# POSTECH-CVLab/PyTorch-StudioGAN

Measured on AMD Instinct MI355X. Metric: images/sec (G+D step) BigGAN ImageNet-128 bs256, higher is better.
Workload: dtype bf16

## Files before the change

### include/sgamd.h

```cpp
#ifndef SGAMD_H
#define SGAMD_H
#include <stdint.h>
#ifdef __cplusplus
extern "C" {
#endif

typedef void* sg_stream_t;

#define SG_DTYPE_F32 0
#define SG_DTYPE_BF16 1
#define SG_DTYPE_F64 2

#define SG_PIX_RELU 1
#define SG_PIX_UPSAMPLE 2
#define SG_PIX_QUAD 4
#define SG_PIX_TRANSPOSED 8
#define SG_EPI_OUT_F32 1
#define SG_EPI_ATOMIC 2
#define SG_EPI_POOL 4
#define SG_EPI_RELU 8
#define SG_EPI_RES_F32 16

const char* sg_last_error(void);
int sg_version(void);
int sg_prof_enable(int on);
int sg_prof_collect(double* out, int nkinds);

typedef struct {
  int dtype;
  int N, Hs, Ws, C, ldx;
  int Ho, Wo, Cout;
  int R, S, stride, pad_h, pad_w;
  int pix_flags, epi_flags;
  float alpha, beta;
  const void* x; const void* w;
  const float* bias; const void* res; const void* mask; void* out; const float* alpha_ptr;
  int ldo, ldr, ldm;
} sg_conv_fwd_desc;
int sg_conv2d_fwd(const sg_conv_fwd_desc* d, sg_stream_t stream);
int sg_set_f32_mode(int mode);
int sg_get_f32_mode(void);

typedef struct {
  sg_conv_fwd_desc main;
  const void* x2; const void* w2; const float* bias2;
  int C2, ldx2, x2_up;
  float* stats;
} sg_conv_skip_desc;
int sg_conv2d_fwd_skip_stat_rows(const sg_conv_skip_desc* d);
int sg_conv2d_fwd_skip(const sg_conv_skip_desc* d, sg_stream_t stream);
int sg_conv2d_fwd_skip_ok(const sg_conv_skip_desc* d);
long long sg_conv_rs_launches(void);

#define SG_Q_POOL 0
#define SG_Q_UP 1
typedef struct {
  int dtype, form;
  int N, Hl, Wl;
  int C, ldx, Cout;
  int pix_flags, epi_flags;
  float alpha, beta;
  const void* x; const void* wq;
  const float* bias; const void* res; const void* mask; void* out; const float* alpha_ptr;
  int ldo, ldr, ldm;
  const void* x2; const void* w2q; const float* bias2;
  int C2, ldx2;
  float* stats;
  int x2_norelu;
} sg_convq_desc;
int sg_conv2d_q_stat_rows(const sg_convq_desc* d);
int sg_conv2d_q(const sg_convq_desc* d, sg_stream_t stream);
int sg_conv2d_q_ok(const sg_convq_desc* d);
int sg_quad_pack(int dtype, int mode, const void* src, void* dst, int M, int Cs, sg_stream_t stream);
typedef struct { const void* src; void* dst; int M, Cs, mode, pad_; } sg_quad_item;
int sg_quad_pack_batch(int dtype, const sg_quad_item* items_dev, const sg_quad_item* items_host, int n, sg_stream_t stream);
typedef struct {
  int dtype, form;
  int N, Hl, Wl;
  int C, ldx, x_flags;
  int Cout, ldg;
  float alpha; const float* alpha_ptr;
  const void* x; const void* dy; float* dw; float* dbias;
  float* work; long long work_floats;
  int splits;
} sg_convq_wgrad_desc;
int sg_conv2d_q_wgrad_plan(const sg_convq_wgrad_desc* d, int* splits, long long* work_floats);
int sg_conv2d_q_wgrad(const sg_convq_wgrad_desc* d, sg_stream_t stream);
int sg_prof_collect_ex(double* out, int nkinds);
int sg_prof_collect_tags(double* out, int ntags);

typedef struct {
  int dtype;
  int N;
  int xHs, xWs, C, ldx, x_flags;
  int gHs, gWs, Cout, ldg, g_flags;
  int Ho, Wo;
  int R, S, stride, pad_h, pad_w;
  float alpha;
  const void* x; const void* dy; float* dw;
  const float* alpha_ptr;
  int splits;
  int no_tr;
  float* work; long long work_floats;
  float* dbias;
} sg_conv_wgrad_desc;
int sg_conv2d_wgrad(const sg_conv_wgrad_desc* d, sg_stream_t stream);
int sg_conv2d_wgrad_fuses_bias(const sg_conv_wgrad_desc* d);
int sg_conv2d_wgrad_plan(const sg_conv_wgrad_desc* d, int* splits, long long* work_floats);

typedef struct {
  int dtype, p_form, q_form;
  int I, J, K, batch;
  const void* p; long long p_bstride; int ldp;
  const void* q; long long q_bstride; int ldq;
  void* out; long long out_bstride; int ldo;
  const float* bias; const void* res; long long res_bstride; int ldr; float beta;
  float alpha; const float* alpha_ptr;
  int epi_flags; int splits; int no_tr;
} sg_gemm_desc;
int sg_gemm(const sg_gemm_desc* d, sg_stream_t stream);
typedef struct { const float* w; const float* y; const float* bias; float* out; int rows, K, ldy, ldo; } sg_linear_item;
int sg_linear_group(const sg_linear_item* items_dev, const sg_linear_item* items_host, int n, int B, sg_stream_t stream);

int sg_nchw_to_nhwc(int dtype, const float* src, void* dst, int N, int C, int H, int W, int ldo, sg_stream_t s);
int sg_nhwc_to_nchw(int dtype, const void* src, float* dst, int N, int C, int H, int W, int lds, int apply_tanh, sg_stream_t s);
int sg_nchw_grad_to_nhwc(int dtype, const float* dy, const float* y, void* dst, int N, int C, int H, int W, int ldo, int apply_tanh, sg_stream_t s);
int sg_avgpool2_fwd(int dtype, const void* x, void* y, int N, int H, int W, int C, sg_stream_t s);
int sg_avgpool2_bwd(int dtype, const void* dy, void* dx, int N, int H, int W, int C, sg_stream_t s);
int sg_maxpool2_fwd(int dtype, const void* x, int ldx, void* y, int ldy, uint8_t* idx, int N, int H, int W, int C, sg_stream_t s);
int sg_maxpool2_bwd(int dtype, const void* dy, int ldy, const uint8_t* idx, void* dx, int ldx, int N, int H, int W, int C, sg_stream_t s);
int sg_softmax_rows(int dtype, const float* s_in, void* p_out, long long rows, int cols, sg_stream_t st);
int sg_softmax_rows_bwd(int dtype, const void* p, const float* dp, void* ds, long long rows, int cols, sg_stream_t st);
int sg_convert(int src_dtype, int dst_dtype, const void* x, void* y, long long n, sg_stream_t s);
int sg_add_relu(int dtype, const void* a, const void* x, void* out, long long n, sg_stream_t s);
int sg_relu_mask(int dtype, const void* dy, const void* x, void* dx, long long n, sg_stream_t s);
int sg_axpby(int dtype, const void* x, void* y, long long n, float a, float b, sg_stream_t s);
int sg_dot(int dtype, const void* x, const void* y, long long n, float* out, float scale, const float* scale_ptr, sg_stream_t s);
int sg_colsum(int dtype, const void* x, int ldx, const void* mask, int ldm, long long rows, int C, float* out, float alpha, sg_stream_t s);

int sg_bn_partial_stats(int dtype, const void* x, int ldx, long long rows, int C, double* partial, sg_stream_t s);
int sg_bn_stats_from_tiles(const float* stats, int nrows, int C, double* partial, sg_stream_t s);
int sg_bn_finalize(const double* partial, double count, int C, float eps, float momentum, float* mean, float* invstd,
                   float* running_mean, float* running_var, sg_stream_t s);
typedef void* sg_comm_t;
int sg_comm_unique_id(void* out128);
int sg_comm_init_rank(const void* id128, int nranks, int rank, sg_comm_t* comm);
int sg_comm_size(sg_comm_t comm, int* nranks);
int sg_comm_destroy(sg_comm_t comm);
int sg_allreduce_flat(sg_comm_t comm, void* buf, long long count, int dtype, sg_stream_t s);
int sg_bn_stats_sync(int dtype, const void* x, int ldx, long long rows, int C, double* partial, sg_comm_t comm, float eps, float momentum,
                     float* mean, float* invstd, float* running_mean, float* running_var, sg_stream_t s);
int sg_reduce_scatter_flat(sg_comm_t comm, float* buf, long long per_rank, sg_stream_t s);
int sg_allgather_flat(sg_comm_t comm, float* buf, long long per_rank, sg_stream_t s);

// ... 194 lines not shown
```

### pytorch-studiogan_amd/_lib.py

```python
import ctypes as C
import os
import subprocess
import sys

import torch

_HERE = os.path.dirname(os.path.abspath(__file__))
LIB_PATH = os.path.join(_HERE, "libsgamd.so")
if os.environ.get("SG_LIBSGAMD"):
    LIB_PATH = os.path.abspath(os.environ["SG_LIBSGAMD"])
CSRC = os.path.join(_HERE, "csrc")

F32, BF16, F64 = 0, 1, 2
PIX_RELU, PIX_UPSAMPLE, PIX_QUAD, PIX_TRANSPOSED = 1, 2, 4, 8
Q_POOL, Q_UP = 0, 1
EPI_OUT_F32, EPI_ATOMIC, EPI_POOL, EPI_RELU, EPI_RES_F32 = 1, 2, 4, 8, 16

_vp, _i, _f, _ll = C.c_void_p, C.c_int, C.c_float, C.c_longlong


class ConvFwdDesc(C.Structure):
    _fields_ = [("dtype", _i), ("N", _i), ("Hs", _i), ("Ws", _i), ("C", _i), ("ldx", _i), ("Ho", _i), ("Wo", _i), ("Cout", _i),
                ("R", _i), ("S", _i), ("stride", _i), ("pad_h", _i), ("pad_w", _i), ("pix_flags", _i), ("epi_flags", _i),
                ("alpha", _f), ("beta", _f), ("x", _vp), ("w", _vp), ("bias", _vp), ("res", _vp), ("mask", _vp), ("out", _vp),
                ("alpha_ptr", _vp), ("ldo", _i), ("ldr", _i), ("ldm", _i)]


class ConvSkipDesc(C.Structure):
    _fields_ = [("main", ConvFwdDesc), ("x2", _vp), ("w2", _vp), ("bias2", _vp), ("C2", _i), ("ldx2", _i), ("x2_up", _i), ("stats", _vp)]


class ConvWgradDesc(C.Structure):
    _fields_ = [("dtype", _i), ("N", _i), ("xHs", _i), ("xWs", _i), ("C", _i), ("ldx", _i), ("x_flags", _i), ("gHs", _i), ("gWs", _i),
                ("Cout", _i), ("ldg", _i), ("g_flags", _i), ("Ho", _i), ("Wo", _i), ("R", _i), ("S", _i), ("stride", _i),
                ("pad_h", _i), ("pad_w", _i), ("alpha", _f), ("x", _vp), ("dy", _vp), ("dw", _vp), ("alpha_ptr", _vp),
                ("splits", _i), ("no_tr", _i), ("work", _vp), ("work_floats", _ll), ("dbias", _vp)]


class ConvQDesc(C.Structure):
    _fields_ = [("dtype", _i), ("form", _i), ("N", _i), ("Hl", _i), ("Wl", _i), ("C", _i), ("ldx", _i), ("Cout", _i),
                ("pix_flags", _i), ("epi_flags", _i), ("alpha", _f), ("beta", _f), ("x", _vp), ("wq", _vp), ("bias", _vp), ("res", _vp),
                ("mask", _vp), ("out", _vp), ("alpha_ptr", _vp), ("ldo", _i), ("ldr", _i), ("ldm", _i),
                ("x2", _vp), ("w2q", _vp), ("bias2", _vp), ("C2", _i), ("ldx2", _i), ("stats", _vp), ("x2_norelu", _i)]


class ConvQWgradDesc(C.Structure):
    _fields_ = [("dtype", _i), ("form", _i), ("N", _i), ("Hl", _i), ("Wl", _i), ("C", _i), ("ldx", _i), ("x_flags", _i), ("Cout", _i),
                ("ldg", _i), ("alpha", _f), ("alpha_ptr", _vp), ("x", _vp), ("dy", _vp), ("dw", _vp), ("dbias", _vp), ("work", _vp),
                ("work_floats", _ll), ("splits", _i)]


class QuadItem(C.Structure):
    _fields_ = [("src", _vp), ("dst", _vp), ("M", _i), ("Cs", _i), ("mode", _i), ("pad_", _i)]


class LinearItem(C.Structure):
    _fields_ = [("w", _vp), ("y", _vp), ("bias", _vp), ("out", _vp), ("rows", _i), ("K", _i), ("ldy", _i), ("ldo", _i)]


class GemmDesc(C.Structure):
    _fields_ = [("dtype", _i), ("p_form", _i), ("q_form", _i), ("I", _i), ("J", _i), ("K", _i), ("batch", _i),
                ("p", _vp), ("p_bstride", _ll), ("ldp", _i), ("q", _vp), ("q_bstride", _ll), ("ldq", _i),
                ("out", _vp), ("out_bstride", _ll), ("ldo", _i), ("bias", _vp), ("res", _vp), ("res_bstride", _ll), ("ldr", _i),
                ("beta", _f), ("alpha", _f), ("alpha_ptr", _vp), ("epi_flags", _i), ("splits", _i), ("no_tr", _i)]


class SnLayer(C.Structure):
    _fields_ = [("w", _vp), ("u", _vp), ("v", _vp), ("sigma", _vp), ("u_snap", _vp), ("v_snap", _vp), ("w_fwd", _vp), ("w_dgrad", _vp),
                ("w_f32", _vp), ("rows", _i), ("cols", _i), ("Cin", _i), ("RS", _i), ("do_power_iter", _i), ("apply_sn", _i),
                ("rows_pad", _i), ("work_off", _ll), ("trans", _i), ("dgrad_noflip", _i), ("Cin_pad", _i)]


class SnBwdLayer(C.Structure):
    _fields_ = [("dwt", _vp), ("w", _vp), ("u", _vp), ("v", _vp), ("sigma", _vp), ("dw", _vp), ("rows", _i), ("cols", _i),
                ("Cin", _i), ("RS", _i), ("natural", _i), ("apply_sn", _i), ("trans", _i), ("Cin_pad", _i)]


class AugDesc(C.Structure):
    _fields_ = [("N", _i), ("C", _i), ("H", _i), ("W", _i), ("ops", _i), ("cut_h", _i), ("cut_w", _i), ("max_t", _i), ("color", _vp), ("geom", _vp)]


AUG_BRIGHTNESS, AUG_SATURATION, AUG_CONTRAST, AUG_FLIP, AUG_TRANSLATE, AUG_TRANSLATE_REFLECT, AUG_CUTOUT = 1, 2, 4, 8, 16, 32, 64

_lib = None


def build(force=False, verbose=False):
    cmd = ["make", "-C", CSRC, "-j", str(max(2, os.cpu_count() or 2))]
    if force:
        subprocess.run(["make", "-C", CSRC, "clean"], check=True, stdout=subprocess.DEVNULL)
    res = subprocess.run(cmd, stdout=subprocess.PIPE, stderr=subprocess.STDOUT, text=True)
    if verbose or res.returncode != 0:
        sys.stderr.write(res.stdout)
    if res.returncode != 0:
        raise RuntimeError("building libsgamd.so failed")
    return LIB_PATH


_PROTOS = {
    "sg_prof_enable": [_i],
    "sg_prof_collect": [C.POINTER(C.c_double), _i],
    "sg_conv2d_fwd": [C.POINTER(ConvFwdDesc), _vp],
    "sg_conv2d_fwd_skip": [C.POINTER(ConvSkipDesc), _vp],
    "sg_conv2d_fwd_skip_ok": [C.POINTER(ConvSkipDesc)],
    "sg_conv_rs_launches": [],
    "sg_conv2d_q": [C.POINTER(ConvQDesc), _vp],
    "sg_conv2d_q_ok": [C.POINTER(ConvQDesc)],
    "sg_conv2d_q_stat_rows": [C.POINTER(ConvQDesc)],
    "sg_conv2d_fwd_skip_stat_rows": [C.POINTER(ConvSkipDesc)],
    "sg_bn_stats_from_tiles": [_vp, _i, _i, _vp, _vp],
    "sg_quad_pack": [_i, _i, _vp, _vp, _i, _i, _vp],
    "sg_quad_pack_batch": [_i, _vp, C.POINTER(QuadItem), _i, _vp],
    "sg_linear_group": [_vp, C.POINTER(LinearItem), _i, _i, _vp],
    "sg_conv2d_q_wgrad_plan": [C.POINTER(ConvQWgradDesc), C.POINTER(_i), C.POINTER(_ll)],
    "sg_conv2d_q_wgrad": [C.POINTER(ConvQWgradDesc), _vp],
    "sg_prof_collect_ex": [C.POINTER(C.c_double), _i],
    "sg_prof_collect_tags": [C.POINTER(C.c_double), _i],
    "sg_conv2d_wgrad": [C.POINTER(ConvWgradDesc), _vp],
    "sg_conv2d_wgrad_plan": [C.POINTER(ConvWgradDesc), C.POINTER(_i), C.POINTER(_ll)],
    "sg_conv2d_wgrad_fuses_bias": [C.POINTER(ConvWgradDesc)],
    "sg_gemm": [C.POINTER(GemmDesc), _vp],
    "sg_nchw_to_nhwc": [_i, _vp, _vp, _i, _i, _i, _i, _i, _vp],
    "sg_nhwc_to_nchw": [_i, _vp, _vp, _i, _i, _i, _i, _i, _i, _vp],
    "sg_nchw_grad_to_nhwc": [_i, _vp, _vp, _vp, _i, _i, _i, _i, _i, _i, _vp],
    "sg_avgpool2_fwd": [_i, _vp, _vp, _i, _i, _i, _i, _vp],
    "sg_avgpool2_bwd": [_i, _vp, _vp, _i, _i, _i, _i, _vp],
    "sg_maxpool2_fwd": [_i, _vp, _i, _vp, _i, _vp, _i, _i, _i, _i, _vp],
    "sg_maxpool2_bwd": [_i, _vp, _i, _vp, _vp, _i, _i, _i, _i, _i, _vp],
    "sg_softmax_rows": [_i, _vp, _vp, _ll, _i, _vp],
    "sg_softmax_rows_bwd": [_i, _vp, _vp, _vp, _ll, _i, _vp],
    "sg_axpby": [_i, _vp, _vp, _ll, _f, _f, _vp],
    "sg_convert": [_i, _i, _vp, _vp, _ll, _vp],
    "sg_add_relu": [_i, _vp, _vp, _vp, _ll, _vp],
    "sg_relu_mask": [_i, _vp, _vp, _vp, _ll, _vp],
    "sg_dot": [_i, _vp, _vp, _ll, _vp, _f, _vp, _vp],
    "sg_colsum": [_i, _vp, _i, _vp, _i, _ll, _i, _vp, _f, _vp],
    "sg_bn_partial_stats": [_i, _vp, _i, _ll, _i, _vp, _vp],
    "sg_bn_finalize": [_vp, C.c_double, _i, _f, _f, _vp, _vp, _vp, _vp, _vp],
    "sg_comm_unique_id": [_vp],
    "sg_comm_init_rank": [_vp, _i, _i, C.POINTER(_vp)],
    "sg_comm_size": [_vp, C.POINTER(_i)],
    "sg_comm_destroy": [_vp],
    "sg_allreduce_flat": [_vp, _vp, _ll, _i, _vp],
    "sg_bn_stats_sync": [_i, _vp, _i, _ll, _i, _vp, _vp, _f, _f, _vp, _vp, _vp, _vp, _vp],
    "sg_set_f32_mode": [_i],
    "sg_get_f32_mode": [],
    "sg_reduce_scatter_flat": [_vp, _vp, _ll, _vp],
    "sg_allgather_flat": [_vp, _vp, _ll, _vp],
    "sg_p2p_create": [_i, _i, _ll, C.POINTER(_vp), _vp],
    "sg_p2p_connect": [_vp, _vp],
    "sg_p2p_destroy": [_vp],
    "sg_p2p_timeouts": [_vp, C.POINTER(_i)],
    "sg_p2p_allreduce_f64": [_vp, _vp, _i, _vp],
    "sg_bn_finalize_p2p": [_vp, _vp, C.c_double, _i, _f, _f, _vp, _vp, _vp, _vp, _vp],
    "sg_bn_stats_sync_p2p": [_i, _vp, _i, _ll, _i, _vp, _vp, _f, _f, _vp, _vp, _vp, _vp, _vp],
    "sg_bn_from_running": [_vp, _vp, _i, _f, _vp, _vp, _vp],
    "sg_bn_apply": [_i, _vp, _vp, _i, _ll, _i, _vp, _vp, _vp, _vp, _i, _i, _vp],
    "sg_bn_bwd_reduce": [_i, _vp, _vp, _i, _ll, _i, _vp, _vp, _vp, _vp, _i, _i, _vp, _vp],
    "sg_bn_bwd_finalize": [_vp, _i, _i, _vp, _i, _vp, _vp, _vp, _vp],
    "sg_bn_bwd_apply": [_i, _vp, _vp, _vp, _i, _ll, _i, _vp, _vp, _vp, _vp, _i, _i, _vp, C.c_double, _i, _vp],
    "sg_bn_bwd_apply_res": [_i, _vp, _vp, _vp, _i, _ll, _i, _vp, _vp, _vp, _vp, _i, _i, _vp, C.c_double, _i, _vp, _vp],
    "sg_bn_bwd2_reduce": [_i, _vp, _vp, _vp, _i, _ll, _i, _vp, _vp, _vp, _vp, _i, _vp, _vp],
    "sg_bn_bwd2_finalize": [_vp, _i, _i, _vp, _vp],
    "sg_bn_bwd2_dgain": [_vp, _vp, C.c_double, _vp, _i, _i, _vp, _vp],
    "sg_bn_bwd2_apply": [_i, _vp, _vp, _vp, _vp, _vp, _i, _ll, _i, _vp, _vp, _vp, _vp, _i, _vp, C.c_double, _i, _vp],
    "sg_attn_fused_ok": [_i, _i, _i, _i, _i],
    "sg_attn_fwd_fused_ok": [_i, _i, _i, _i, _i],
    "sg_attn_fwd_flash_ok": [_i, _i, _i, _i, _i],
    "sg_attn_fwd_fused": [_vp, _vp, _vp, _vp, _vp, _vp, _vp, _i, _i, _i, _i, _i, _vp],
    "sg_attn_bwd_fused_ok": [_i, _i, _i, _i, _i],
    "sg_attn_bwd_fused": [_vp, _vp, _vp, _vp, _vp, _vp, _vp, _vp, _vp, _vp, _i, _i, _i, _i, _i, _vp],
    "sg_attn_probs_fwd": [_vp, _vp, _vp, _vp, _i, _i, _i, _i, _vp],
    "sg_attn_ds_bwd": [_vp, _vp, _vp, _vp, _vp, _vp, _i, _i, _i, _i, _i, _vp],
    "sg_attn_proj_ok": [_i, _i, _i, _i, _i, _i, _i],
    "sg_attn_proj_fwd": [_vp, _i, _vp, _vp, _vp, _vp, _vp, _vp, _vp, _vp, _i, _i, _i, _i, _i, _i, _i, _vp],
    "sg_attn_proj_bwd_data": [_vp, _vp, _vp, _vp, _vp, _vp, _vp, _vp, _vp, _vp, _i, _i, _i, _i, _i, _i, _vp],
    "sg_slice_up_fwd": [_i, _vp, _vp, _i, _i, _i, _i, _i, _i, _vp],
    "sg_slice_up_bwd": [_i, _vp, _vp, _i, _i, _i, _i, _i, _i, _vp],
    "sg_copy_channels": [_i, _vp, _i, _vp, _i, _ll, _i, _vp],
    "sg_interp_rows": [_vp, _vp, _vp, _vp, _i, _ll, _vp],
    "sg_gp_fwd": [_i, _vp, _i, _ll, _vp, _vp, _vp],
    "sg_gp_bwd": [_i, _vp, _vp, _vp, _vp, _i, _ll, _vp],
    "sg_masked_sum_hw": [_i, _vp, _vp, _vp, _i, _i, _i, _vp],
    "sg_sn_forward": [_i, _vp, C.POINTER(SnLayer), _i, _f, _vp, _ll, _vp],
    "sg_sn_backward": [_vp, C.POINTER(SnBwdLayer), _i, _vp, _ll, _vp],
    "sg_embedding_fwd": [_vp, _vp, _vp, _i, _i, _i, _vp],
    "sg_embedding_bwd": [_vp, _vp, _vp, _i, _i, _i, _vp],
# ... 142 lines not shown
```

### pytorch-studiogan_amd/backbones/big_resnet.py

```python
import torch
import torch.nn as nn

from .. import functional as F
from .. import ops
from ..bank import get_bank
from .heads import build_heads, apply_heads


def _dtype(mixed_precision):
    return torch.bfloat16 if mixed_precision else torch.float32


def _need_graph(module, *inputs):
    if not torch.is_grad_enabled():
        return False
    for t in inputs:
        if torch.is_tensor(t) and t.requires_grad:
            return True
    return any(p.requires_grad for p in module.parameters())


class GenBlock(nn.Module):
    def __init__(self, in_channels, out_channels, g_cond_mtd, affine_input_dim, MODULES):
        super().__init__()
# ... 69 lines not shown
        for index in range(self.num_blocks):
            blocks += [[GenBlock(in_channels=self.in_dims[index], out_channels=self.out_dims[index], g_cond_mtd=self.g_cond_mtd,
                                 affine_input_dim=self.affine_input_dim, MODULES=MODULES)]]
            if index + 1 in attn_g_loc and apply_attn:
                blocks += [[ops.SelfAttention(self.out_dims[index], is_generator=True, MODULES=MODULES)]]
        self.blocks = nn.ModuleList([nn.ModuleList(block) for block in blocks])

        self.bn4 = ops.batchnorm_2d(in_features=self.out_dims[-1])
        self.activation = MODULES.g_act_fn
        self.conv2d5 = MODULES.g_conv2d(in_channels=self.out_dims[-1], out_channels=3, kernel_size=3, stride=1, padding=1)
        self.tanh = nn.Tanh()
        self.conv2d5._sg_rows_pad = 8
        ops.init_weights(self.modules, g_init)
        ops.adopt(self, _dtype(mixed_precision))

    def forward(self, z, label, shared_label=None, eval=False):
        dtype = self.compute_dtype
        bank = get_bank(self, dtype)
        slot = bank.begin_forward(_need_graph(self, z, shared_label))
        affine_list = []
        if self.info_type != "N/A":
            if self.g_info_injection == "concat":
                z = self.info_mix_linear.forward_rt(z, slot)
            else:
                z, z_info = z[:, :self.z_dim], z[:, self.z_dim:]
                affine_list.append(self.info_proj_linear.forward_rt(z_info, slot))
        zs = torch.split(z, self.chunk_size, 1)
        z0 = zs[0]
        if self.g_cond_mtd != "W/O":
            if shared_label is None:
                shared_label = self.shared(label)
            affine_list.append(shared_label)
        if len(affine_list) == 0:
            affines = [item for item in zs[1:]]
        else:
            affines = [torch.cat(affine_list + [item], 1) for item in zs[1:]]

        pairs, counter = [], 0
        for blocklist in self.blocks:
            for block in blocklist:
                if not isinstance(block, ops.SelfAttention):
                    if isinstance(block.bn1, ops.ConditionalBatchNorm2d):
                        pairs += [(block.bn1, affines[counter]), (block.bn2, affines[counter])]
                    counter += 1
        F.cbn_prefetch(slot, pairs)

        act = self.linear0.forward_rt(z0, slot)
        act = F.NchwToNhwcFn.apply(act.view(-1, self.in_dims[0], self.bottom, self.bottom), dtype)
        act = ops.block_boundary(self, -1, act)
        counter = 0
        nxt = bank.boundaries(self.blocks) if bank.exchange is not None else None
        with ops.bump_batches_tracked(self):
            for bi, blocklist in enumerate(self.blocks):
                for block in blocklist:
                    if isinstance(block, ops.SelfAttention):
                        act = block.forward_nhwc(act, slot)
                    else:
                        act = block.forward_nhwc(act, affines[counter], slot)
                        counter += 1
                if nxt is not None:
                    act = bank.mark(act, nxt[bi])
                act = ops.block_boundary(self, bi, act)
            act = self.bn4.forward_nhwc(act, relu=True)
        act = self.conv2d5.forward_nhwc(act, slot)
        return F.NhwcToNchwFn.apply(act, True, 3)


class DiscOptBlock(nn.Module):
    def __init__(self, in_channels, out_channels, apply_d_sn, MODULES):
        super().__init__()
        self.apply_d_sn = apply_d_sn
        self.conv2d0 = MODULES.d_conv2d(in_channels=in_channels, out_channels=out_channels, kernel_size=1, stride=1, padding=0)
        self.conv2d1 = MODULES.d_conv2d(in_channels=in_channels, out_channels=out_channels, kernel_size=3, stride=1, padding=1)
        self.conv2d2 = MODULES.d_conv2d(in_channels=out_channels, out_channels=out_channels, kernel_size=3, stride=1, padding=1)
        if not apply_d_sn:
            self.bn0 = MODULES.d_bn(in_features=in_channels)
            self.bn1 = MODULES.d_bn(in_features=out_channels)
        self.activation = MODULES.d_act_fn
        self.average_pooling = nn.AvgPool2d(2)
        self.cpad = 8 if (apply_d_sn and in_channels < 8) else 0
        if self.cpad:
            self.conv2d1._sg_cin_pad = self.conv2d0._sg_cin_pad = self.cpad

    def forward_nhwc(self, x, slot):
        h = self.conv2d1.forward_nhwc(x, slot)
        if not self.apply_d_sn:
            h = self.bn1.forward_nhwc(h, relu=True)
            h = self.conv2d2.forward_nhwc(h, slot, out_pool=True)
        else:
            if self.cpad == 8 and h.dtype == torch.bfloat16 and not x.requires_grad:
                return ops.conv_skip_nhwc(self.conv2d2, self.conv2d0, h, x, slot, in_relu=True, out_pool=True, skip_relu=False)
            h = self.conv2d2.forward_nhwc(h, slot, in_relu=True, out_pool=True)
        x0 = F.AvgPool2Fn.apply(x)
        if not self.apply_d_sn:
            x0 = self.bn0.forward_nhwc(x0)
        return self.conv2d0.forward_nhwc(x0, slot, res=h)


class DiscBlock(nn.Module):
    def __init__(self, in_channels, out_channels, apply_d_sn, MODULES, downsample=True):
        super().__init__()
        self.apply_d_sn = apply_d_sn
        self.downsample = downsample
        self.activation = MODULES.d_act_fn
        self.ch_mismatch = in_channels != out_channels
        if self.ch_mismatch or downsample:
            self.conv2d0 = MODULES.d_conv2d(in_channels=in_channels, out_channels=out_channels, kernel_size=1, stride=1, padding=0)
            if not apply_d_sn:
                self.bn0 = MODULES.d_bn(in_features=in_channels)
        self.conv2d1 = MODULES.d_conv2d(in_channels=in_channels, out_channels=out_channels, kernel_size=3, stride=1, padding=1)
        self.conv2d2 = MODULES.d_conv2d(in_channels=out_channels, out_channels=out_channels, kernel_size=3, stride=1, padding=1)
        if not apply_d_sn:
            self.bn1 = MODULES.d_bn(in_features=in_channels)
            self.bn2 = MODULES.d_bn(in_features=out_channels)
        self.average_pooling = nn.AvgPool2d(2)

    def forward_nhwc(self, x, slot):
        if self.apply_d_sn:
            if self.downsample or self.ch_mismatch:
                link = F.GradLink()
                h = self.conv2d1.forward_nhwc(x, slot, in_relu=True, link=link)
                return ops.conv_skip_nhwc(self.conv2d2, self.conv2d0, h, x, slot, in_relu=True, out_pool=self.downsample, link=link)
            h = self.conv2d1.forward_nhwc(x, slot, in_relu=True)
            h = self.conv2d2.forward_nhwc(h, slot, in_relu=True, out_pool=False)
            return F.AddReluFn.apply(h, x)
        h = self.bn1.forward_nhwc(x, relu=True)
        h = self.conv2d1.forward_nhwc(h, slot)
        h = self.bn2.forward_nhwc(h, relu=True)
        h = self.conv2d2.forward_nhwc(h, slot, out_pool=self.downsample)
        if self.downsample or self.ch_mismatch:
            x0 = self.bn0.forward_nhwc(x)
            return self.conv2d0.forward_nhwc(x0, slot, out_pool=self.downsample, res=h)
        return F.AddFn.apply(h, x)


class Discriminator(nn.Module):
    def __init__(self, img_size, d_conv_dim, apply_d_sn, apply_attn, attn_d_loc, d_cond_mtd, aux_cls_type, d_embed_dim, normalize_d_embed,
                 num_classes, d_init, d_depth, mixed_precision, MODULES, MODEL):
        super().__init__()
        d_in_dims_collection = {
            "32": [3] + [d_conv_dim * 2, d_conv_dim * 2, d_conv_dim * 2],
            "64": [3] + [d_conv_dim, d_conv_dim * 2, d_conv_dim * 4, d_conv_dim * 8],
            "128": [3] + [d_conv_dim, d_conv_dim * 2, d_conv_dim * 4, d_conv_dim * 8, d_conv_dim * 16],
            "256": [3] + [d_conv_dim, d_conv_dim * 2, d_conv_dim * 4, d_conv_dim * 8, d_conv_dim * 8, d_conv_dim * 16],
            "512": [3] + [d_conv_dim, d_conv_dim, d_conv_dim * 2, d_conv_dim * 4, d_conv_dim * 8, d_conv_dim * 8, d_conv_dim * 16]
        }
        d_out_dims_collection = {
            "32": [d_conv_dim * 2, d_conv_dim * 2, d_conv_dim * 2, d_conv_dim * 2],
            "64": [d_conv_dim, d_conv_dim * 2, d_conv_dim * 4, d_conv_dim * 8, d_conv_dim * 16],
            "128": [d_conv_dim, d_conv_dim * 2, d_conv_dim * 4, d_conv_dim * 8, d_conv_dim * 16, d_conv_dim * 16],
            "256": [d_conv_dim, d_conv_dim * 2, d_conv_dim * 4, d_conv_dim * 8, d_conv_dim * 8, d_conv_dim * 16, d_conv_dim * 16],
            "512": [d_conv_dim, d_conv_dim, d_conv_dim * 2, d_conv_dim * 4, d_conv_dim * 8, d_conv_dim * 8, d_conv_dim * 16, d_conv_dim * 16]
        }
        d_down = {
            "32": [True, True, False, False],
            "64": [True, True, True, True, False],
            "128": [True, True, True, True, True, False],
            "256": [True, True, True, True, True, True, False],
            "512": [True, True, True, True, True, True, True, False]
        }
        self.d_cond_mtd = d_cond_mtd
        self.aux_cls_type = aux_cls_type
        self.normalize_d_embed = normalize_d_embed
        self.num_classes = num_classes
        self.mixed_precision = mixed_precision
        self.in_dims = d_in_dims_collection[str(img_size)]
        self.out_dims = d_out_dims_collection[str(img_size)]
        self.MODEL = MODEL
        down = d_down[str(img_size)]

        blocks = []
        for index in range(len(self.in_dims)):
            if index == 0:
                blocks += [[DiscOptBlock(in_channels=self.in_dims[index], out_channels=self.out_dims[index], apply_d_sn=apply_d_sn, MODULES=MODULES)]]
            else:
                blocks += [[DiscBlock(in_channels=self.in_dims[index], out_channels=self.out_dims[index], apply_d_sn=apply_d_sn,
                                      MODULES=MODULES, downsample=down[index])]]
            if index + 1 in attn_d_loc and apply_attn:
                blocks += [[ops.SelfAttention(self.out_dims[index], is_generator=False, MODULES=MODULES)]]
        self.blocks = nn.ModuleList([nn.ModuleList(block) for block in blocks])
        self.activation = MODULES.d_act_fn
        build_heads(self, MODULES, self.out_dims[-1], d_cond_mtd, aux_cls_type, d_embed_dim, num_classes, MODEL)
        if d_init:
            ops.init_weights(self.modules, d_init)
        ops.adopt(self, _dtype(mixed_precision))

    def forward(self, x, label, eval=False, adc_fake=False):
        dtype = self.compute_dtype
        bank = get_bank(self, dtype)
        slot = bank.begin_forward(_need_graph(self, x))
        h = ops.to_nhwc(x, dtype, self.blocks[0][0].cpad)
        nxt = bank.boundaries(self.blocks) if bank.exchange is not None else None
        for bi, blocklist in enumerate(self.blocks):
            for block in blocklist:
                h = block.forward_nhwc(h, slot)
            if nxt is not None:
                h = bank.mark(h, nxt[bi])
            h = ops.block_boundary(self, bi, h)
        hw = h.shape[1] * h.shape[2]
        h = F.ReluSumFn.apply(h)
        return apply_heads(self, h, label, slot, adc_fake, hw=hw)
```

### pytorch-studiogan_amd/csrc/common.h

```cpp
#pragma once
#include <hip/hip_runtime.h>
#include <stdint.h>

typedef uint16_t bf16_t;
typedef __attribute__((ext_vector_type(4))) uint32_t u32x4;
typedef __attribute__((ext_vector_type(2))) uint32_t u32x2;
typedef __attribute__((ext_vector_type(4))) float f32x4;
typedef __attribute__((ext_vector_type(16))) float f32x16;
typedef __attribute__((ext_vector_type(8))) __bf16 bf16x8_t;
typedef __attribute__((ext_vector_type(4))) short s16x4;
typedef __attribute__((ext_vector_type(8))) short s16x8;

#define SG_PRIO_UP() __builtin_amdgcn_s_setprio(1)
#define SG_PRIO_DOWN() __builtin_amdgcn_s_setprio(0)

#define SG_DTYPE_F32 0
#define SG_DTYPE_BF16 1

__device__ __forceinline__ float bf2f(bf16_t v) { return __uint_as_float(((uint32_t)v) << 16); }
__device__ __forceinline__ bf16_t f2bf(float f) {
  uint32_t u = __float_as_uint(f);
  if ((u & 0x7fffffffu) > 0x7f800000u) return (bf16_t)((u >> 16) | 0x40u);
  u += 0x7fffu + ((u >> 16) & 1u);
  return (bf16_t)(u >> 16);
}

typedef __bf16 sg_bf16x2_t __attribute__((ext_vector_type(2)));
typedef float sg_f32x2_t __attribute__((ext_vector_type(2)));
__device__ __forceinline__ uint32_t pack2bf(float a, float b) {
  sg_f32x2_t v = {a, b};
  return __builtin_bit_cast(uint32_t, __builtin_convertvector(v, sg_bf16x2_t));
}

template <typename T> __device__ __forceinline__ float to_f(T v);
template <> __device__ __forceinline__ float to_f<float>(float v) { return v; }
template <> __device__ __forceinline__ float to_f<bf16_t>(bf16_t v) { return bf2f(v); }
template <typename T> __device__ __forceinline__ T from_f(float v);
template <> __device__ __forceinline__ float from_f<float>(float v) { return v; }
template <> __device__ __forceinline__ bf16_t from_f<bf16_t>(float v) { return f2bf(v); }

template <typename T> struct ET;
template <> struct ET<float> { static constexpr int VEC = 4, BK = 16; };
template <> struct ET<bf16_t> { static constexpr int VEC = 8, BK = 32; };

__device__ __forceinline__ u32x4 zero16() { u32x4 z = {0u, 0u, 0u, 0u}; return z; }

template <typename T> __device__ __forceinline__ void unpack16(u32x4 v, float* o);
template <> __device__ __forceinline__ void unpack16<float>(u32x4 v, float* o) {
#pragma unroll
  for (int i = 0; i < 4; i++) o[i] = __uint_as_float(v[i]);
}
template <> __device__ __forceinline__ void unpack16<bf16_t>(u32x4 v, float* o) {
#pragma unroll
  for (int i = 0; i < 4; i++) { o[2 * i] = __uint_as_float(v[i] << 16); o[2 * i + 1] = __uint_as_float(v[i] & 0xffff0000u); }
}
template <typename T> __device__ __forceinline__ u32x4 pack16(const float* o);
template <> __device__ __forceinline__ u32x4 pack16<float>(const float* o) {
  u32x4 v;
#pragma unroll
  for (int i = 0; i < 4; i++) v[i] = __float_as_uint(o[i]);
  return v;
}
template <> __device__ __forceinline__ u32x4 pack16<bf16_t>(const float* o) {
  u32x4 v;
#pragma unroll
  for (int i = 0; i < 4; i++) v[i] = (uint32_t)f2bf(o[2 * i]) | ((uint32_t)f2bf(o[2 * i + 1]) << 16);
  return v;
}


template <typename T> __device__ __forceinline__ u32x4 relu16(u32x4 v);
template <> __device__ __forceinline__ u32x4 relu16<float>(u32x4 v) {
#pragma unroll
  for (int i = 0; i < 4; i++) v[i] = (v[i] & 0x80000000u) ? 0u : v[i];
  return v;
}
template <> __device__ __forceinline__ u32x4 relu16<bf16_t>(u32x4 v) {
  typedef short s16x2_t __attribute__((ext_vector_type(2)));
#pragma unroll
  for (int i = 0; i < 4; i++) {
    const uint32_t x = v[i];
    s16x2_t a = __builtin_bit_cast(s16x2_t, x);
    const s16x2_t z = {0, 0};
    a = __builtin_elementwise_max(a, z);
    v[i] = __builtin_bit_cast(uint32_t, a);
  }
  return v;
}

__device__ __forceinline__ float quad_sum(float v) {
  v += __builtin_bit_cast(float, __builtin_amdgcn_update_dpp(0, __builtin_bit_cast(int, v), 0xB1, 0xF, 0xF, true));
  v += __builtin_bit_cast(float, __builtin_amdgcn_update_dpp(0, __builtin_bit_cast(int, v), 0x4E, 0xF, 0xF, true));
  return v;
}

__device__ __forceinline__ float wave_sum(float v) {
#pragma unroll
  for (int o = 32; o > 0; o >>= 1) v += __shfl_xor(v, o, 64);
  return v;
}
__device__ __forceinline__ double wave_sum_d(double v) {
#pragma unroll
  for (int o = 32; o > 0; o >>= 1) v += __shfl_xor(v, o, 64);
  return v;
}
__device__ __forceinline__ float wave_max(float v) {
#pragma unroll
  for (int o = 32; o > 0; o >>= 1) v = fmaxf(v, __shfl_xor(v, o, 64));
  return v;
}

__device__ __forceinline__ float block_sum_256(float v, float* sm ) {
  v = wave_sum(v);
  int w = threadIdx.x >> 6;
// ... 46 lines not shown
```

### pytorch-studiogan_amd/csrc/conv.hip

```cpp
#include "conv_common.h"
#include "conv_v2.h"

int g_sg_f32_mode = 0;
extern "C" int sg_set_f32_mode(int mode) {
  SG_CHECK(mode == 0 || mode == 3, "sg_set_f32_mode: 0 (exact fp32 MFMA) or 3 (bf16x3 split)");
  g_sg_f32_mode = mode;
  return 0;
}
extern "C" int sg_get_f32_mode() { return g_sg_f32_mode; }

template <typename T, bool FAST>
static void conv_fwd_launch(const sg_conv_fwd_desc* d, const Epilogue<T>& e, int I, int J, int K, int pflags, hipStream_t st) {
  typedef StridedKC<T, FAST> LP;
  typedef ConvPixKC<T, FAST> LQ;
  LP lp;
  lp.base = (const T*)d->w; lp.bstride = 0; lp.ld = K; lp.rows = I; lp.K = K;
  lp.vec_ok = (K % ET<T>::VEC == 0) && aligned16(d->w);
  LQ lq;
  fill_geom<T>(lq.g, d->x, d->N, d->Hs, d->Ws, d->C, d->ldx, d->Ho, d->Wo, d->R, d->S, d->stride, d->pad_h, d->pad_w, pflags);
  lq.rows = J; lq.K = K;
  if constexpr (sizeof(T) == 4 && FAST) {
    if (g_sg_f32_mode == 3) {
      if (I <= 32) sg_launch_gemm<T, LP, LQ, 32, 256, 1, 4, true, 3>(lp, lq, e, I, J, K, 1, 1, st);
      else if (I % 128 != 0 && (I % 96 == 0 || (I < 128 && I > 64))) sg_launch_gemm<T, LP, LQ, 96, 256, 1, 4, true, 3>(lp, lq, e, I, J, K, 1, 1, st);
      else sg_launch_gemm<T, LP, LQ, 128, 128, 2, 2, true, 3>(lp, lq, e, I, J, K, 1, 1, st);
      return;
    }
  }
  if (I <= 32) sg_launch_gemm<T, LP, LQ, 32, 256, 1, 4>(lp, lq, e, I, J, K, 1, 1, st);
  else if (I % 128 != 0 && (I % 96 == 0 || (I < 128 && I > 64))) sg_launch_gemm<T, LP, LQ, 96, 256, 1, 4>(lp, lq, e, I, J, K, 1, 1, st);
  else sg_launch_gemm<T, LP, LQ, 128, 128, 2, 2>(lp, lq, e, I, J, K, 1, 1, st);
}

template <typename T> static bool conv_fwd_v2_try(const sg_conv_fwd_desc*, const Epilogue<T>&, int, int, int, int, hipStream_t) { return false; }
template <> bool conv_fwd_v2_try<bf16_t>(const sg_conv_fwd_desc* d, const Epilogue<bf16_t>& e, int I, int J, int K, int pflags, hipStream_t st) {
  const char* mode = getenv("SG_CONV_V2");
  const bool disabled = mode && mode[0] == '0';
  const bool force = mode && mode[0] == 'f';
  if (disabled || (pflags & SG_PIX_TRANSPOSED)) return false;
  if (d->stride != 1 && (d->stride != 2 || (pflags & (SG_PIX_UPSAMPLE | SG_PIX_QUAD)) || getenv("SG_CONV_V2_STRIDE2_OFF"))) return false;
  if (d->C % 8 || d->ldx % 8 || d->R * d->S > 25 || J < 256) return false;
  const long long xbytes = (((long long)d->N * d->Hs * d->Ws - 1) * d->ldx + d->C) * 2, wbytes = (long long)I * K * 2;
  if (xbytes >= (1ll << 31) || wbytes >= (1ll << 30)) return false;
  if (!aligned16(d->x) || !aligned16(d->w)) return false;
  if ((e.flags & (SG_EPI_ATOMIC | SG_EPI_OUT_F32)) || (e.ldo & 7) || !aligned16(e.out)) return false;
  if (e.mask && ((e.ldm & 7) || !aligned16(e.mask))) return false;
  if (e.res && ((e.flags & SG_EPI_RES_F32) || (e.ldr & 7) || !aligned16(e.res))) return false;
  const int tj = (J + 255) / 256;
  const int cands[3] = {192, 128, 96};
  int best = 0, best_tiles = 0;
  for (int c = 0; c < 3; c++) {
    if (I % cands[c]) continue;
    const int tiles = (I / cands[c]) * tj;
    if (tiles >= 512) { best = cands[c]; best_tiles = tiles; break; }
    if (tiles > best_tiles) { best = cands[c]; best_tiles = tiles; }
  }
  if (!best && I % 8 == 0 && I >= 32) {
    int best_pad = 0;
    for (int c = 0; c < 3; c++) {
      const int padded = ((I + cands[c] - 1) / cands[c]) * cands[c];
      if (2 * padded > 3 * I) continue;
      const int tiles = (padded / cands[c]) * tj;
      if (!best || padded < best_pad) { best = cands[c]; best_pad = padded; best_tiles = tiles; }
    }
  }
  int min_tiles = 160;
  if (const char* mt = getenv("SG_CONV_V2_MIN_TILES")) { const int v = atoi(mt); if (v > 0) min_tiles = v; }
  if (!best || (best_tiles < min_tiles && !force)) return false;
  ConvV2Params p;
  p.x = (const bf16_t*)d->x; p.w = (const bf16_t*)d->w;
  p.N = d->N; p.Hs = d->Hs; p.Ws = d->Ws; p.C = d->C; p.ldx = d->ldx;
  const int up = (pflags & SG_PIX_UPSAMPLE) ? 2 : 1;
  p.Hin = d->Hs * up; p.Win = d->Ws * up; p.Ho = d->Ho; p.Wo = d->Wo;
  p.R = d->R; p.S = d->S; p.pad_h = d->pad_h; p.pad_w = d->pad_w; p.flags = pflags; p.stride = d->stride;
  p.I = I; p.J = J; p.K = K; p.cpt = d->C / 8; p.ntap = d->R * d->S;
  p.wshift = ilog2_exact(d->Wo); p.hshift = ilog2_exact(d->Ho);
  p.xbytes = (unsigned)xbytes; p.wbytes = (unsigned)wbytes;
  int rc = 0;
  if (best == 192) rc = sg_launch_conv_v2<192, 4, 2, 256, 7>(p, e, st);
  else if (best == 128) rc = sg_launch_conv_v2<128, 4, 2, 256, 7>(p, e, st);
  else {
    if (J >= 512 * 256) rc = sg_launch_conv_v2<96, 8, 1, 512, 1>(p, e, st);
    else rc = sg_launch_conv_v2<96, 8, 1, 256, 1>(p, e, st);
  }
  return rc == 0;
}

template <typename T> static bool conv_fwd_v3_try(const sg_conv_fwd_desc*, const Epilogue<T>&, int, int, int, int, hipStream_t) { return false; }
template <> bool conv_fwd_v3_try<bf16_t>(const sg_conv_fwd_desc* d, const Epilogue<bf16_t>& e, int I, int J, int K, int pflags, hipStream_t st) {
  return sg_conv_fwd_v3_try(d, e, I, J, K, pflags, st);
}
template <typename T> static bool conv_fwd_v4_try(const sg_conv_fwd_desc*, const Epilogue<T>&, int, int, int, int, hipStream_t) { return false; }
template <> bool conv_fwd_v4_try<bf16_t>(const sg_conv_fwd_desc* d, const Epilogue<bf16_t>& e, int I, int J, int K, int pflags, hipStream_t st) {
  return sg_conv_fwd_v4_try(d, e, I, J, K, pflags, st);
}
template <typename T> static bool conv_fwd_rs_try(const sg_conv_fwd_desc*, const Epilogue<T>&, int, int, int, int, hipStream_t) { return false; }
template <> bool conv_fwd_rs_try<bf16_t>(const sg_conv_fwd_desc* d, const Epilogue<bf16_t>& e, int I, int J, int K, int pflags, hipStream_t st) {
  return sg_conv_fwd_rs_try(d, e, I, J, K, pflags, st);
}
template <typename T> static bool conv_fwd_sk_try(const sg_conv_fwd_desc*, const Epilogue<T>&, int, int, int, int, hipStream_t) { return false; }
template <> bool conv_fwd_sk_try<bf16_t>(const sg_conv_fwd_desc* d, const Epilogue<bf16_t>& e, int I, int J, int K, int pflags, hipStream_t st) {
  return sg_conv_fwd_sk_try(d, e, I, J, K, pflags, st);
}

template <typename T> static int conv_fwd_t(const sg_conv_fwd_desc* d, hipStream_t st) {
  const int K = d->R * d->S * d->C;
  const int I = d->Cout;
  const long long Jll = (long long)d->N * d->Ho * d->Wo;
  SG_CHECK(Jll < (1ll << 31), "sg_conv2d_fwd: too many output pixels");
  SG_CHECK((long long)d->N * d->Hs * d->Ws * d->ldx < (1ll << 31), "sg_conv2d_fwd: input tensor too large for 32-bit element offsets");
  const int J = (int)Jll;
  int pflags = d->pix_flags;
  if (d->epi_flags & SG_EPI_POOL) {
    SG_CHECK((d->Ho % 2 == 0) && (d->Wo % 2 == 0), "sg_conv2d_fwd: pooled output needs even Ho, Wo");
    pflags |= SG_PIX_QUAD;
  } else {
    pflags &= ~SG_PIX_QUAD;
  }
  const bool w_vec = (K % ET<T>::VEC == 0) && aligned16(d->w);
  const bool x_vec = (d->C % ET<T>::VEC == 0) && (d->ldx % ET<T>::VEC == 0) && aligned16(d->x);
  Epilogue<T> e;
  e.out = d->out; e.out_bstride = 0; e.ldo = d->ldo; e.bias = d->bias;
  e.res = d->res; e.res_bstride = 0; e.ldr = d->ldr; e.beta = d->beta;
  e.mask = (const T*)d->mask; e.mask_bstride = 0; e.ldm = d->ldm; e.split_stride = 0;
  e.alpha = d->alpha; e.alpha_ptr = d->alpha_ptr; e.flags = d->epi_flags; e.I = I; e.J = J;
  const int prof = sg_prof_begin(st, 2.0 * (double)I * (double)J * (double)K, 0);
  int eng = SG_ENG_CONV_GEMM;
  if (w_vec && x_vec && conv_fwd_sk_try<T>(d, e, I, J, K, pflags, st)) eng = SG_ENG_CONV_SK;
  else if (w_vec && x_vec && conv_fwd_rs_try<T>(d, e, I, J, K, pflags, st)) eng = SG_ENG_CONV_RS;
  else if (w_vec && x_vec && conv_fwd_v4_try<T>(d, e, I, J, K, pflags, st)) eng = SG_ENG_CONV_V4;
  else if (w_vec && x_vec && conv_fwd_v3_try<T>(d, e, I, J, K, pflags, st)) eng = SG_ENG_CONV_V3;
  else if (w_vec && x_vec && conv_fwd_v2_try<T>(d, e, I, J, K, pflags, st)) eng = SG_ENG_CONV_V2;
  else if (w_vec && x_vec) conv_fwd_launch<T, true>(d, e, I, J, K, pflags, st);
  else conv_fwd_launch<T, false>(d, e, I, J, K, pflags, st);
  {
    const double es = sizeof(T), jout = (d->epi_flags & SG_EPI_POOL) ? (double)J / 4.0 : (double)J;
    const double b = es * ((double)d->N * d->Hs * d->Ws * d->C + (double)I * K + jout * I * (1.0 + (d->mask ? 1.0 : 0.0) + (d->res ? 1.0 : 0.0)));
    sg_prof_tag(prof, eng, b);
  }
  sg_prof_end(st, prof);
  SG_LAUNCH_CHECK();
  return 0;
}

static int conv_fwd_skip(const sg_conv_skip_desc* sk, hipStream_t st, bool dry) {
  const sg_conv_fwd_desc* d = &sk->main;
  if (d->dtype != SG_DTYPE_BF16 || d->R != 3 || d->S != 3 || d->stride != 1 || (d->pix_flags & (SG_PIX_UPSAMPLE | SG_PIX_TRANSPOSED))) return 0;
  const int K = 9 * d->C, I = d->Cout;
  const long long Jll = (long long)d->N * d->Ho * d->Wo;
  if (Jll >= (1ll << 31) || (long long)d->N * d->Hs * d->Ws * d->ldx >= (1ll << 31)) return 0;
  const int J = (int)Jll;
  int pflags = d->pix_flags;
  if (d->epi_flags & SG_EPI_POOL) { if ((d->Ho & 1) || (d->Wo & 1)) return 0; pflags |= SG_PIX_QUAD; } else pflags &= ~SG_PIX_QUAD;
  Epilogue<bf16_t> e;
  e.out = d->out; e.out_bstride = 0; e.ldo = d->ldo; e.bias = d->bias;
  e.res = d->res; e.res_bstride = 0; e.ldr = d->ldr; e.beta = d->beta;
  e.mask = (const bf16_t*)d->mask; e.mask_bstride = 0; e.ldm = d->ldm; e.split_stride = 0;
  e.alpha = d->alpha; e.alpha_ptr = d->alpha_ptr; e.flags = d->epi_flags; e.I = I; e.J = J;
  if (dry) return sg_conv_fwd_v4_skip_try(d, sk, e, I, J, K, pflags, st, true) ? 1 : 0;
  const int prof = sg_prof_begin(st, 2.0 * (double)I * (double)J * ((double)K + (double)sk->C2), 0);
  const bool ok = sg_conv_fwd_v4_skip_try(d, sk, e, I, J, K, pflags, st, false);
  {
    const double jout = (d->epi_flags & SG_EPI_POOL) ? (double)J / 4.0 : (double)J;
    const double x2 = (double)d->N * (sk->x2_up ? (d->Ho / 2) * (d->Wo / 2) : d->Ho * d->Wo) * sk->C2;
    sg_prof_tag(prof, SG_ENG_CONV_V4_SKIP, 2.0 * ((double)d->N * d->Hs * d->Ws * d->C + x2 + (double)I * (K + sk->C2) + jout * I));
  }
  sg_prof_end(st, prof);
  return ok ? 1 : 0;
}
extern "C" int sg_conv2d_fwd_skip_stat_rows(const sg_conv_skip_desc* d) {
  if (!d) return 0;
  const long long J = (long long)d->main.N * d->main.Ho * d->main.Wo;
  return (int)((J + 255) / 256);
}
extern "C" int sg_conv2d_fwd_skip_ok(const sg_conv_skip_desc* d) {
  if (!d || !d->main.x || !d->main.w || !d->main.out || !d->x2 || !d->w2) return 0;
  return conv_fwd_skip(d, nullptr, true);
}
extern "C" int sg_conv2d_fwd_skip(const sg_conv_skip_desc* d, sg_stream_t stream) {
  SG_CHECK(d && d->main.x && d->main.w && d->main.out && d->x2 && d->w2, "sg_conv2d_fwd_skip: null pointer");
  SG_CHECK(conv_fwd_skip(d, (hipStream_t)stream, false) == 1, "sg_conv2d_fwd_skip: problem not eligible for the fused kernel (ask sg_conv2d_fwd_skip_ok first)");
  SG_LAUNCH_CHECK();
  return 0;
}

extern "C" int sg_conv2d_fwd(const sg_conv_fwd_desc* d, sg_stream_t stream) {
  SG_CHECK(d && d->x && d->w && d->out, "sg_conv2d_fwd: null pointer");
  SG_CHECK(d->N > 0 && d->C > 0 && d->Cout > 0 && d->R > 0 && d->S > 0 && d->stride > 0, "sg_conv2d_fwd: bad shape");
  SG_CHECK(!(d->epi_flags & SG_EPI_ATOMIC), "sg_conv2d_fwd: atomic epilogue not supported");
  if (d->dtype == SG_DTYPE_F32) return conv_fwd_t<float>(d, (hipStream_t)stream);
  if (d->dtype == SG_DTYPE_BF16) return conv_fwd_t<bf16_t>(d, (hipStream_t)stream);
  sg_set_error("sg_conv2d_fwd: bad dtype");
  return -1;
}
```

### pytorch-studiogan_amd/csrc/conv_q.hip

```cpp
#include "conv_common.h"
#include "conv_q.h"
#include "wgrad_q.h"
#include "wgrad_ql.h"

__device__ __host__ static inline int quad_pat(int pool_like, int a, int t) {
  const int P[2][2] = {{3, 4}, {1, 6}};
  const int U[2][2] = {{1, 6}, {3, 4}};
  return pool_like ? P[a][t] : U[a][t];
}
static inline bool quad_mode_pool_like(int mode) { return mode == 0 || mode == 3; }
static inline float quad_mode_scale(int mode) { return (mode == 0 || mode == 2) ? 0.25f : 1.f; }

template <typename T>
__global__ __launch_bounds__(256) void k_quad_pack(const T* src, T* dst, long long nvec, int cv, int pool_like, float scale) {
  constexpr int V = ET<T>::VEC;
  const long long i = (long long)blockIdx.x * 256 + threadIdx.x;
  if (i >= nvec) return;
  const long long m = i / cv;
  const int c = (int)(i - m * cv) * V;
  const int Cs = cv * V;
  const T* s0 = src + m * 9 * Cs + c;
  float w[9][V];
#pragma unroll
  for (int k = 0; k < 9; k++) unpack16<T>(*(const u32x4*)(s0 + (long long)k * Cs), w[k]);
// ... 41 lines not shown
  SG_LAUNCH_CHECK();
  return 0;
}

template <typename T>
__global__ __launch_bounds__(256) void k_quad_pack_batch(const sg_quad_item* items, int n) {
  constexpr int V = ET<T>::VEC;
  long long base = 0;
  int it = 0;
  long long blk = blockIdx.x;
  for (; it < n; it++) {
    const long long per = items[it].mode == 5 ? (long long)items[it].M * 4 : (long long)items[it].M * (items[it].Cs / V) * (items[it].mode == 4 ? 1 : 16);
    const long long nb = (per + 255) / 256;
    if (blk < base + nb) break;
    base += nb;
  }
  if (it >= n) return;
  const sg_quad_item q = items[it];
  const int cv = q.Cs / V;
  const long long i = (blk - base) * 256 + threadIdx.x;
  if (q.mode == 5) {
    if (i >= (long long)q.M * 4) return;
    float o[V];
    unpack16<T>(*(const u32x4*)((const T*)q.src + (i >> 2) * V), o);
#pragma unroll
    for (int e = 0; e < V; e++) o[e] *= 0.25f;
    *(u32x4*)((T*)q.dst + i * V) = pack16<T>(o);
    return;
  }
  if (q.mode == 4) {
    if (i >= (long long)q.M * cv) return;
    float o[V];
    unpack16<T>(*(const u32x4*)((const T*)q.src + i * V), o);
#pragma unroll
    for (int e = 0; e < V; e++) o[e] *= 0.25f;
    *(u32x4*)((T*)q.dst + i * V) = pack16<T>(o);
    return;
  }
  if (i >= (long long)q.M * cv * 16) return;
  const bool pool_like = q.mode == 0 || q.mode == 3;
  const float scale = (q.mode == 0 || q.mode == 2) ? 0.25f : 1.f;
  const int c = (int)(i % cv) * V;
  const long long mv = i / cv;
  const int vt = (int)(mv & 15);
  const long long m = mv >> 4;
  const int view = vt >> 2, t = vt & 3;
  const int pr = quad_pat(pool_like, view >> 1, t >> 1), pc = quad_pat(pool_like, view & 1, t & 1);
  const T* s0 = (const T*)q.src + m * 9 * q.Cs + c;
  float o[V];
#pragma unroll
  for (int e = 0; e < V; e++) o[e] = 0.f;
#pragma unroll
  for (int r = 0; r < 3; r++)
#pragma unroll
    for (int s = 0; s < 3; s++)
      if (((pr >> r) & 1) && ((pc >> s) & 1)) {
        float w[V];
        unpack16<T>(*(const u32x4*)(s0 + (long long)(r * 3 + s) * q.Cs), w);
#pragma unroll
        for (int e = 0; e < V; e++) o[e] += w[e];
      }
#pragma unroll
  for (int e = 0; e < V; e++) o[e] *= scale;
  *(u32x4*)((T*)q.dst + (m * 16 + vt) * q.Cs + c) = pack16<T>(o);
}
extern "C" int sg_quad_pack_batch(int dtype, const sg_quad_item* items_dev, const sg_quad_item* items_host, int n, sg_stream_t stream) {
  SG_CHECK(items_dev && items_host && n > 0 && n <= 64, "sg_quad_pack_batch: bad arguments");
  const int V = dtype == SG_DTYPE_BF16 ? 8 : 4;
  long long blocks = 0;
  for (int i = 0; i < n; i++) {
    const sg_quad_item& q = items_host[i];
    SG_CHECK(q.src && q.dst && q.M > 0 && q.Cs > 0 && q.Cs % V == 0 && q.mode >= 0 && q.mode <= 5 && (q.mode != 5 || (q.Cs == 8 && dtype == SG_DTYPE_BF16)) && aligned16(q.src) && aligned16(q.dst), "sg_quad_pack_batch: bad item");
    blocks += ((q.mode == 5 ? (long long)q.M * 4 : (long long)q.M * (q.Cs / V) * (q.mode == 4 ? 1 : 16)) + 255) / 256;
  }
  hipStream_t st = (hipStream_t)stream;
  if (dtype == SG_DTYPE_BF16) hipLaunchKernelGGL(k_quad_pack_batch<bf16_t>, dim3((unsigned)blocks), dim3(256), 0, st, items_dev, n);
  else if (dtype == SG_DTYPE_F32) hipLaunchKernelGGL(k_quad_pack_batch<float>, dim3((unsigned)blocks), dim3(256), 0, st, items_dev, n);
  else { sg_set_error("sg_quad_pack_batch: bad dtype"); return -1; }
  SG_LAUNCH_CHECK();
  return 0;
}

static bool convq_plan(const sg_convq_desc* d, ConvQParams& p, Epilogue<bf16_t>& e, int& NB) {
  if (d->dtype != SG_DTYPE_BF16 || (d->form != SG_Q_POOL && d->form != SG_Q_UP)) return false;
  const char* mode = getenv("SG_CONV_Q");
  if (mode && mode[0] == '0') return false;
  if (d->C < 32 || d->C % 32 || d->ldx % 8 || !aligned16(d->x) || !aligned16(d->wq)) return false;
  const int wlog = ilog2_exact(d->Wl), hlog = ilog2_exact(d->Hl);
  if (wlog < 2 || hlog < 1) return false;
  const long long J = (long long)d->N * d->Hl * d->Wl;
  const long long npix_x = d->form == SG_Q_POOL ? 4 * J : J;
  if (4 * J >= (1ll << 29)) return false;
  const long long xbytes = ((npix_x - 1) * d->ldx + d->C) * 2, wbytes = (long long)d->Cout * 16 * d->C * 2;
  if (xbytes >= (1ll << 31) || wbytes >= (1ll << 31)) return false;
  if ((d->epi_flags & ~SG_EPI_RELU) || (d->pix_flags & ~SG_PIX_RELU)) return false;
  if ((d->ldo & 7) || !aligned16(d->out)) return false;
  if (d->mask && ((d->ldm & 7) || !aligned16(d->mask))) return false;
  if (d->res && ((d->ldr & 7) || !aligned16(d->res))) return false;
  if (d->Cout % 96 == 0) NB = 3; else if (d->Cout % 64 == 0) NB = 2; else return false;
  p.x = (const bf16_t*)d->x; p.w = (const bf16_t*)d->wq;
  p.form = d->form; p.Wl = d->Wl; p.wlog = wlog; p.hlog = hlog;
  p.C = d->C; p.ldx = d->ldx; p.I = d->Cout; p.J = (int)J; p.K = 16 * d->C; p.nslice = d->C / 32;
  {
    const int nph = d->form == SG_Q_POOL ? 1 : 4;
    const long long tiles256 = (long long)(d->Cout / (32 * NB)) * ((J + 255) / 256) * nph;
    p.bj = tiles256 < 512 ? 128 : 256;
    if (const char* bj = getenv("SG_CONV_Q_BJ")) { if (bj[0] == '1') p.bj = 128; else if (bj[0] == '2') p.bj = 256; }
  }
  p.npx = ((p.bj + 2 * d->Wl + 16) + 15) & ~15;
  p.gj = wbytes > (2ll << 20) ? 8 : 1;
  if (const char* gj = getenv("SG_CONV_Q_GJ")) { const int v = atoi(gj); if (v >= 1 && v <= 64) p.gj = v; }
  p.flags = d->pix_flags;
  p.xbytes = (unsigned)xbytes; p.wbytes = (unsigned)wbytes;
  p.wgt_off = p.zero_off = p.bias_off = 0;
  p.x2 = nullptr; p.w2 = nullptr; p.bias2 = nullptr; p.C2 = p.ldx2 = p.nslice2 = 0; p.x2bytes = p.w2bytes = 0; p.c2x8 = p.skip_norelu = 0;
  if (d->x2) {
    const bool c8 = d->C2 == 8;
    if (d->form != SG_Q_POOL || !d->w2q || (!c8 && (d->C2 < 32 || d->C2 % 32)) || d->ldx2 % 8 || !aligned16(d->x2) || !aligned16(d->w2q)) return false;
    if (d->bias2 && !d->bias) return false;
    const int c2w = c8 ? 32 : d->C2;
    const long long x2bytes = ((4 * J - 1) * d->ldx2 + d->C2) * 2, w2bytes = (long long)d->Cout * c2w * 2;
    if (x2bytes >= (1ll << 31) || w2bytes >= (1ll << 31)) return false;
    p.x2 = (const bf16_t*)d->x2; p.w2 = (const bf16_t*)d->w2q; p.bias2 = d->bias2;
    p.C2 = c2w; p.ldx2 = d->ldx2; p.nslice2 = c2w / 32; p.x2bytes = (unsigned)x2bytes; p.w2bytes = (unsigned)w2bytes;
    p.c2x8 = c8 ? 1 : 0; p.skip_norelu = d->x2_norelu ? 1 : 0;
  }
  p.stats = d->stats;
  e.out = d->out; e.out_bstride = 0; e.ldo = d->ldo; e.bias = d->bias;
  e.res = d->res; e.res_bstride = 0; e.ldr = d->ldr; e.beta = d->beta;
  e.mask = (const bf16_t*)d->mask; e.mask_bstride = 0; e.ldm = d->ldm; e.split_stride = 0;
  e.alpha = d->alpha; e.alpha_ptr = d->alpha_ptr; e.flags = d->epi_flags; e.I = d->Cout; e.J = (int)J;
  return true;
}
extern "C" int sg_conv2d_q_ok(const sg_convq_desc* d) {
  if (!d || !d->x || !d->wq || !d->out) return 0;
  ConvQParams p; Epilogue<bf16_t> e; int NB;
  return convq_plan(d, p, e, NB) ? 1 : 0;
}
extern "C" int sg_conv2d_q_stat_rows(const sg_convq_desc* d) {
  if (!d || !d->x || !d->wq || !d->out) return 0;
  ConvQParams p; Epilogue<bf16_t> e; int NB;
  if (!convq_plan(d, p, e, NB)) return 0;
  const int sbj = p.bj > 256 ? 256 : p.bj;
  return ((p.J + sbj - 1) / sbj) * (d->form == SG_Q_POOL ? 1 : 4);
}
extern "C" int sg_conv2d_q(const sg_convq_desc* d, sg_stream_t stream) {
  SG_CHECK(d && d->x && d->wq && d->out, "sg_conv2d_q: null pointer");
  ConvQParams p; Epilogue<bf16_t> e; int NB = 0;
  SG_CHECK(convq_plan(d, p, e, NB), "sg_conv2d_q: problem not eligible for the quad kernel (ask sg_conv2d_q_ok first)");
  hipStream_t st = (hipStream_t)stream;
  const double c2 = d->x2 ? (double)d->C2 : 0.0;
  const int prof = sg_prof_begin_q(st, 2.0 * (double)d->Cout * 4.0 * (double)p.J * (9.0 * (double)d->C + c2), 0);
  sg_prof_set_executed(prof, 2.0 * (double)d->Cout * (double)p.J * (16.0 * (double)d->C + 4.0 * c2));
  const char* ev_db = getenv("SG_CONV_Q_DB");
  int db_mode = ev_db ? (ev_db[0] == '1' ? 1 : 0) : ((d->Wl == 4 && d->form == SG_Q_UP) ? 1 : 0);
  const int rc = NB == 3 ? sg_launch_conv_q<3>(p, e, db_mode, st) : sg_launch_conv_q<2>(p, e, db_mode, st);
  {
    const double J = (double)p.J, jin = d->form == SG_Q_POOL ? 4.0 * J : J, jout = d->form == SG_Q_POOL ? J : 4.0 * J;
    sg_prof_tag(prof, d->x2 ? SG_ENG_CONV_Q_SKIP : SG_ENG_CONV_Q,
                2.0 * (jin * d->C + (d->x2 ? 4.0 * J * d->C2 + (double)d->Cout * d->C2 : 0.0) + 16.0 * d->C * d->Cout + jout * d->Cout * (1.0 + (d->mask ? 1.0 : 0.0) + (d->res ? 1.0 : 0.0))));
  }
  sg_prof_end(st, prof);
  SG_CHECK(rc == 0, "sg_conv2d_q: launch failed");
  SG_LAUNCH_CHECK();
  return 0;
}

struct QPlan { bool ok; int NB, S, nci, nco, splits, nchunk; long long n, stride; };
static QPlan wgradq_plan(const sg_convq_wgrad_desc* d) {
  QPlan s; s.ok = false; s.NB = s.S = s.nci = s.nco = s.splits = s.nchunk = 0; s.n = s.stride = 0;
  const char* mode = getenv("SG_WGRAD_Q");
  if (mode && mode[0] == '0') return s;
  if (d->dtype != SG_DTYPE_BF16 || (d->form != SG_Q_POOL && d->form != SG_Q_UP)) return s;
  if (ilog2_exact(d->Wl) < 2 || ilog2_exact(d->Hl) < 0) return s;
  if (d->Wl == 4 && (d->Hl != 4 || d->N % 4)) return s;
  if (d->Wl < 64 && d->Wl > 4 && d->Hl % (64 / d->Wl)) return s;
  if (d->C % 32 || d->ldx % 8 || d->ldg % 8 || !aligned16(d->x) || !aligned16(d->dy)) return s;
  if (d->x_flags & ~SG_PIX_RELU) return s;
  if (d->Cout % 96 == 0) s.NB = 3; else if (d->Cout % 64 == 0) s.NB = 2; else return s;
  const long long K = (long long)d->N * d->Hl * d->Wl;
  if (K % 64 || 4 * K >= (1ll << 29)) return s;
  const long long xpix = d->form == SG_Q_POOL ? 4 * K : K, gpix = d->form == SG_Q_POOL ? K : 4 * K;
  if (xpix * d->ldx * 2 >= (1ll << 31) || gpix * d->ldg * 2 >= (1ll << 31)) return s;
  s.S = (d->C % 64 == 0) ? 2 : 1;
  s.nci = d->C / (32 * s.S); s.nco = d->Cout / (32 * s.NB); s.nchunk = (int)(K / 64);
  s.n = 16ll * d->C * d->Cout;
  s.stride = s.n + (d->dbias ? 4ll * d->Cout : 0);
  const int tiles = 4 * s.nci * s.nco;
  int sp = d->splits > 0 ? d->splits : (512 >= tiles ? 512 / tiles : 1);
  const int maxs = s.nchunk / 8 > 0 ? s.nchunk / 8 : 1;
  if (sp > maxs) sp = maxs;
  if (sp > 512) sp = 512;
  s.splits = sp;
  s.ok = true;
  return s;
}
extern "C" int sg_conv2d_q_wgrad_plan(const sg_convq_wgrad_desc* d, int* splits, long long* work_floats) {
  SG_CHECK(d && splits && work_floats, "sg_conv2d_q_wgrad_plan: null");
  const QPlan s = wgradq_plan(d);
  *splits = s.ok ? s.splits : 0;
  *work_floats = s.ok ? (long long)s.splits * s.stride : 0;
  return 0;
}

__global__ __launch_bounds__(256) void k_quad_reduce_fold(const float* partial, float* dw, int splits, long long stride, int M, int C, int pool_like, float scale,
                                                          float* dbias, long long bias_off, int nviews, int nmain) {
  __shared__ f32x4 sm[16][16];
  const int tid = threadIdx.x;
  if ((int)blockIdx.x >= nmain) {
    const int co = ((int)blockIdx.x - nmain) * 256 + tid;
    if (co < M) {
      float t = 0.f;
      for (int s = 0; s < splits; s++)
        for (int v = 0; v < nviews; v++) t += partial[(long long)s * stride + bias_off + (long long)v * M + co];
      dbias[co] += t;
    }
    return;
  }
  const int cb = C > 64 ? (C + 63) / 64 : 1;
  const int m = blockIdx.x / cb, c0 = (blockIdx.x - m * cb) * 64;
  const int vt = tid >> 4, c4 = tid & 15;
  const int c = c0 + 4 * c4;
  f32x4 a0 = {0.f, 0.f, 0.f, 0.f}, a1 = a0, a2 = a0, a3 = a0;
  if (c < C) {
    const float* src = partial + ((long long)m * 16 + vt) * C + c;
    int s = 0;
    for (; s + 3 < splits; s += 4) {
      const f32x4 v0 = *(const f32x4*)(src + (long long)s * stride), v1 = *(const f32x4*)(src + (long long)(s + 1) * stride);
      const f32x4 v2 = *(const f32x4*)(src + (long long)(s + 2) * stride), v3 = *(const f32x4*)(src + (long long)(s + 3) * stride);
      a0 += v0; a1 += v1; a2 += v2; a3 += v3;
    }
    for (; s < splits; s++) a0 += *(const f32x4*)(src + (long long)s * stride);
  }
  sm[vt][c4] = (a0 + a1) + (a2 + a3);
  __syncthreads();
  if (tid < 144 && c < C) {
    const int rs = tid >> 4, r = rs / 3, s3 = rs - 3 * r;
    f32x4 t = {0.f, 0.f, 0.f, 0.f};
#pragma unroll
    for (int view = 0; view < 4; view++)
#pragma unroll
      for (int q = 0; q < 4; q++) {
        const int pr = quad_pat(pool_like, view >> 1, q >> 1), pc = quad_pat(pool_like, view & 1, q & 1);
// ... 46 lines not shown
```

### pytorch-studiogan_amd/csrc/conv_sk.h

```cpp
#pragma once
#include "conv_v2.h"

struct ConvSkParams {
  const bf16_t* x; const bf16_t* w;
  int C, ldx, Hs, Ws;
  int Ho, Wo, wshift, hshift;
  int mode3;
  int flags;
  int I, J, K;
  unsigned xbytes;
  unsigned obytes, sbytes;
  int nrb;
};

template <int TI, int NP, int TJ, int KS, int NW, bool POOL>
__global__ __launch_bounds__(64 * NW) void sg_conv_sk_kernel(ConvSkParams p, Epilogue<bf16_t> epi) {
  constexpr int BI = TI * NP * 32;
  constexpr int NCH = 2 * KS;
  constexpr int WP = KS * 32 + 16;
  constexpr int CP = TI * 64 + 16;
  constexpr int ROWS = 32 * TJ;
  constexpr int CPR = TI * 4;
  extern __shared__ __attribute__((aligned(16))) char smem[];
  char* const wsm = smem;
  float* const sbias = (float*)(smem + BI * WP);
  const int tid = threadIdx.x, lane = tid & 63;
  const int wave = __builtin_amdgcn_readfirstlane(tid >> 6);
  char* const stg = smem + BI * WP + BI * 4 + wave * (ROWS * CP);
  const int i0 = blockIdx.y * BI;

  for (int idx = tid; idx < BI * NCH; idx += 64 * NW) {
    const int row = idx / NCH, c = idx - row * NCH;
    u32x4 v = {0u, 0u, 0u, 0u};
    if (i0 + row < p.I && c * 8 < p.K) v = *(const u32x4*)(p.w + (long long)(i0 + row) * p.K + c * 8);
    *(u32x4*)(wsm + row * WP + c * 16) = v;
  }
  for (int i = tid; i < BI; i += 64 * NW) sbias[i] = (epi.bias && i0 + i < epi.I) ? epi.bias[i0 + i] : 0.f;
  __syncthreads();

  const auto rsx = __builtin_amdgcn_make_buffer_rsrc((void*)p.x, 0, (int)p.xbytes, 0x00020000);
  const auto rso = __builtin_amdgcn_make_buffer_rsrc(epi.out, 0, (int)p.obytes, 0x00020000);
  const auto rss = __builtin_amdgcn_make_buffer_rsrc((void*)(epi.mask ? (const void*)epi.mask : epi.res), 0, (int)p.sbytes, 0x00020000);
  constexpr int NIT = ((POOL ? ROWS / 4 : ROWS) * CPR + 63) / 64;
  const int frow = lane & 31, fhi = lane >> 5;
  const unsigned ldx2 = 2u * (unsigned)p.ldx;
  const bool up = (p.flags & SG_PIX_UPSAMPLE) != 0, quad = (p.flags & SG_PIX_QUAD) != 0;
  typedef short s16x2_t __attribute__((ext_vector_type(2)));
  const short fl = (p.flags & SG_PIX_RELU) ? (short)0 : (short)-32768;
  const s16x2_t floor2 = {fl, fl};

  int ctr[KS], cts[KS];
  unsigned cdelta[KS];
  bool cok[KS];
#pragma unroll
  for (int ks = 0; ks < KS; ks++) {
    const int c = 2 * ks + fhi;
    const int tr3 = (c * 11) >> 5;
    const int ts3 = c - 3 * tr3;
    ctr[ks] = p.mode3 ? tr3 : 1;
    cts[ks] = p.mode3 ? ts3 : 1;
    cdelta[ks] = p.mode3 ? (unsigned)((tr3 - 1) * p.Ws + (ts3 - 1)) * ldx2 : (unsigned)c * 16u;
    cok[ks] = p.mode3 ? (c < 9) : (c * 8 < p.C);
  }

  auto fetch = [&](int rb, u32x4 (&q)[TJ][KS]) {
#pragma unroll
    for (int b = 0; b < TJ; b++) {
      const int row = rb * ROWS + b * 32 + frow;
      int n, ho, wo;
      if (quad) {
        const int qd = row >> 2, dy = (row >> 1) & 1, dx = row & 1;
        const int wq = qd & ((p.Wo >> 1) - 1);
        const int t = qd >> (p.wshift - 1);
        const int hq = t & ((p.Ho >> 1) - 1);
        n = t >> (p.hshift - 1);
        ho = 2 * hq + dy; wo = 2 * wq + dx;
      } else {
        wo = row & (p.Wo - 1); const int t = row >> p.wshift; ho = t & (p.Ho - 1); n = t >> p.hshift;
      }
      const bool rok = row < p.J;
      const int hs = up ? (ho >> 1) : ho, ws = up ? (wo >> 1) : wo;
      const unsigned pixoff = ((unsigned)(n * p.Hs + hs) * (unsigned)p.Ws + (unsigned)ws) * ldx2;
      if constexpr (KS == 6) {
#pragma unroll
        for (int ks = 0; ks < KS; ks++) {
          const bool ok = rok && cok[ks] && (unsigned)(ho + ctr[ks] - 1) < (unsigned)p.Ho && (unsigned)(wo + cts[ks] - 1) < (unsigned)p.Wo;
          unsigned off = pixoff + cdelta[ks];
          off = ok ? off : 0x80000000u;
          q[b][ks] = __builtin_bit_cast(u32x4, __builtin_amdgcn_raw_buffer_load_b128(rsx, (int)off, 0, 0));
        }
      } else {
        const unsigned base = rok ? pixoff + (unsigned)fhi * 16u : 0x80000000u;
#pragma unroll
        for (int ks = 0; ks < KS; ks++) {
          const unsigned off = ((2 * ks + fhi) * 8 < p.C) ? base + (unsigned)ks * 32u : 0x80000000u;
          q[b][ks] = __builtin_bit_cast(u32x4, __builtin_amdgcn_raw_buffer_load_b128(rsx, (int)off, 0, 0));
        }
      }
    }
  };

  float al = epi.alpha;
  if (epi.alpha_ptr) al *= *epi.alpha_ptr;
  constexpr bool pool = POOL;
  const bool relu_out = (epi.flags & SG_EPI_RELU) != 0;
  const bool pre_mask = epi.mask != nullptr, pre_res = epi.res != nullptr;
  const int Jout = pool ? (epi.J >> 2) : epi.J;
  const int ncr = ((epi.I - i0 < BI ? epi.I - i0 : BI) + 7) >> 3;
  constexpr int rows_out_full = ROWS;

  auto compute_store = [&](int rb, u32x4 (&q)[TJ][KS]) {
#pragma unroll
    for (int b = 0; b < TJ; b++)
#pragma unroll
      for (int ks = 0; ks < KS; ks++)
#pragma unroll
        for (int e = 0; e < 4; e++) {
          const uint32_t xw = q[b][ks][e];
          s16x2_t t = __builtin_bit_cast(s16x2_t, xw);
          t = __builtin_elementwise_max(t, floor2);
          q[b][ks][e] = __builtin_bit_cast(uint32_t, t);
        }
    const int r0 = rb * ROWS;
    constexpr int rows_out = pool ? rows_out_full / 4 : rows_out_full;
    const int jbase = pool ? (r0 >> 2) : r0;
#pragma unroll
    for (int ps = 0; ps < NP; ps++) {
      f32x16 acc[TI][TJ];
#pragma unroll
      for (int a = 0; a < TI; a++)
#pragma unroll
        for (int b = 0; b < TJ; b++)
#pragma unroll
          for (int r = 0; r < 16; r++) acc[a][b][r] = 0.f;
#pragma unroll
      for (int ks = 0; ks < KS; ks++) {
        bf16x8_t pf[TI], qf[TJ];
#pragma unroll
        for (int a = 0; a < TI; a++) {
          const u32x4 v = *(const u32x4*)(wsm + ((ps * TI + a) * 32 + frow) * WP + (2 * ks + fhi) * 16);
          pf[a] = __builtin_bit_cast(bf16x8_t, v);
        }
#pragma unroll
        for (int b = 0; b < TJ; b++) qf[b] = __builtin_bit_cast(bf16x8_t, q[b][ks]);
#pragma unroll
        for (int a = 0; a < TI; a++)
#pragma unroll
          for (int b = 0; b < TJ; b++)
            acc[a][b] = __builtin_amdgcn_mfma_f32_32x32x16_bf16(pf[a], qf[b], acc[a][b], 0, 0, 0);
      }
      const int ic0 = ps * TI * 32;
      const int ncp = ncr - ps * CPR;
      asm volatile("s_waitcnt lgkmcnt(0)" ::: "memory");
      if (pre_mask || pre_res) {
        const int ld = pre_mask ? epi.ldm : epi.ldr;
        u32x4 pre[NIT];
#pragma unroll
        for (int it = 0; it < NIT; it++) {
          const int idx = lane + 64 * it;
          const int r = idx / CPR, c = idx - r * CPR;
          const int jg = jbase + r;
          const bool ok = idx < rows_out * CPR && jg < Jout && c < ncp;
          const unsigned off = ok ? ((unsigned)jg * (unsigned)ld + (unsigned)(i0 + ic0 + c * 8)) * 2u : 0x80000000u;
          pre[it] = __builtin_bit_cast(u32x4, __builtin_amdgcn_raw_buffer_load_b128(rss, (int)off, 0, 0));
        }
#pragma unroll
        for (int it = 0; it < NIT; it++) {
          const int idx = lane + 64 * it;
          const int r = idx / CPR, c = idx - r * CPR;
          if (idx < rows_out * CPR) *(u32x4*)(stg + r * CP + c * 16) = pre[it];
        }
        asm volatile("s_waitcnt lgkmcnt(0)" ::: "memory");
      }
#pragma unroll
      for (int ta = 0; ta < TI; ta++)
#pragma unroll
        for (int tb = 0; tb < TJ; tb++) {
          const int jl = tb * 32 + (lane & 31);
#pragma unroll
          for (int g4 = 0; g4 < 4; g4++) {
            const int il = ta * 32 + 8 * g4 + 4 * (lane >> 5);
            float v[4] = {acc[ta][tb][4 * g4 + 0], acc[ta][tb][4 * g4 + 1], acc[ta][tb][4 * g4 + 2], acc[ta][tb][4 * g4 + 3]};
            if (pool) {
#pragma unroll
              for (int e = 0; e < 4; e++) v[e] = quad_sum(v[e]);
            }
            const int jo = pool ? (jl >> 2) : jl;
            const bool act = (!pool || (lane & 3) == 0) && (jbase + jo < Jout);
            if (act) {
              char* loc = stg + jo * CP + il * 2;
#pragma unroll
              for (int e = 0; e < 4; e++) v[e] *= al;
              {
                const f32x4 bv = *(const f32x4*)(sbias + ic0 + il);
#pragma unroll
                for (int e = 0; e < 4; e++) v[e] += bv[e];
              }
              if (pre_mask) {
                const u32x2 m = *(const u32x2*)loc;
#pragma unroll
                for (int e = 0; e < 4; e++) { const bf16_t h = (bf16_t)((m[e >> 1] >> (16 * (e & 1))) & 0xffffu); if (!(bf2f(h) > 0.f)) v[e] = 0.f; }
              }
              if (pre_res) {
                const u32x2 r = *(const u32x2*)loc;
#pragma unroll
                for (int e = 0; e < 4; e++) { const bf16_t h = (bf16_t)((r[e >> 1] >> (16 * (e & 1))) & 0xffffu); v[e] += epi.beta * bf2f(h); }
              }
              if (relu_out) {
#pragma unroll
                for (int e = 0; e < 4; e++) v[e] = fmaxf(v[e], 0.f);
              }
              u32x2 t;
              t[0] = pack2bf(v[0], v[1]);
              t[1] = pack2bf(v[2], v[3]);
              *(u32x2*)loc = t;
            }
          }
        }
      asm volatile("s_waitcnt lgkmcnt(0)" ::: "memory");
#pragma unroll
      for (int it = 0; it < NIT; it++) {
        const int idx = lane + 64 * it;
        const int r = idx / CPR, c = idx - r * CPR;
        const int jg = jbase + r;
        const bool ok = idx < rows_out * CPR && jg < Jout && c < ncp;
        const unsigned off = ok ? ((unsigned)jg * (unsigned)epi.ldo + (unsigned)(i0 + ic0 + c * 8)) * 2u : 0x80000000u;
        const int rr = idx < rows_out * CPR ? r : 0;
        const u32x4 v = *(const u32x4*)(stg + rr * CP + c * 16);
        __builtin_amdgcn_raw_buffer_store_b128(v, rso, (int)off, 0, 0);
      }
    }
  };

  const int stride = gridDim.x * NW;
  int rb = blockIdx.x * NW + wave;
  u32x4 qa[TJ][KS], qb[TJ][KS];
  if (rb >= p.nrb) return;
  fetch(rb, qa);
#pragma unroll
  for (int it = 0; it < NP * NIT; it++) {
    const u32x4 z = {0u, 0u, 0u, 0u};
    __builtin_amdgcn_raw_buffer_store_b128(z, rso, (int)(0x80000000u + 16u * it), 0, 0);
  }
  while (true) {
    fetch(rb + stride, qb);
    compute_store(rb, qa);
    rb += stride;
    if (rb >= p.nrb) break;
    fetch(rb + stride, qa);
    compute_store(rb, qb);
    rb += stride;
    if (rb >= p.nrb) break;
  }
}

template <int TI, int NP, int TJ, int KS, bool POOL>
static inline int sg_launch_conv_sk_tp(ConvSkParams p, const Epilogue<bf16_t>& e, hipStream_t st) {
  constexpr int BI = TI * NP * 32, WP = KS * 32 + 16, CP = TI * 64 + 16, ROWS = 32 * TJ;
  constexpr int lds4 = BI * WP + BI * 4 + 4 * ROWS * CP;
  constexpr int NW = (2 * lds4 <= 160 * 1024) ? 4 : 8;
  constexpr int lds = BI * WP + BI * 4 + NW * ROWS * CP;
  static_assert(lds <= 160 * 1024, "LDS");
  static bool attr_done = false;
  if (!attr_done) {
    if (hipFuncSetAttribute((const void*)sg_conv_sk_kernel<TI, NP, TJ, KS, NW, POOL>, hipFuncAttributeMaxDynamicSharedMemorySize, lds) != hipSuccess) return -1;
    attr_done = true;
  }
  p.nrb = (p.J + ROWS - 1) / ROWS;
  const int tilesI = (p.I + BI - 1) / BI;
  int gx = (p.nrb + NW - 1) / NW;
  const int cap = (256 * (8 / NW) + tilesI - 1) / tilesI;
  if (gx > cap) gx = cap;
  hipLaunchKernelGGL((sg_conv_sk_kernel<TI, NP, TJ, KS, NW, POOL>), dim3(gx, tilesI), dim3(64 * NW), lds, st, p, e);
  return 0;
}
template <int TI, int NP, int TJ, int KS>
static inline int sg_launch_conv_sk_t(const ConvSkParams& p, const Epilogue<bf16_t>& e, hipStream_t st) {
  return (e.flags & SG_EPI_POOL) ? sg_launch_conv_sk_tp<TI, NP, TJ, KS, true>(p, e, st) : sg_launch_conv_sk_tp<TI, NP, TJ, KS, false>(p, e, st);
}

static inline int sg_launch_conv_sk(const ConvSkParams& p, const Epilogue<bf16_t>& e, hipStream_t st) {
  const int ti = p.I <= 32 ? 1 : p.I <= 64 ? 2 : p.I <= 96 ? 3 : p.I <= 128 ? 4 : 6;
  const int ks = p.K <= 16 ? 1 : p.K <= 48 ? 3 : p.K <= 96 ? 6 : 12;
#define SG_SK_CASE(T_, TI_, NP_, KS_, TJ_) if (ti == T_ && ks == KS_) return sg_launch_conv_sk_t<TI_, NP_, TJ_, KS_>(p, e, st);
  SG_SK_CASE(1, 1, 1, 1, 2) SG_SK_CASE(1, 1, 1, 3, 2) SG_SK_CASE(1, 1, 1, 6, 2) SG_SK_CASE(1, 1, 1, 12, 1)
  SG_SK_CASE(2, 2, 1, 1, 2) SG_SK_CASE(2, 2, 1, 3, 2) SG_SK_CASE(2, 2, 1, 6, 1) SG_SK_CASE(2, 2, 1, 12, 1)
  SG_SK_CASE(3, 3, 1, 1, 1) SG_SK_CASE(3, 3, 1, 3, 1) SG_SK_CASE(3, 3, 1, 6, 1) SG_SK_CASE(3, 3, 1, 12, 1)
  SG_SK_CASE(4, 2, 2, 1, 2) SG_SK_CASE(4, 2, 2, 3, 2) SG_SK_CASE(4, 2, 2, 6, 1) SG_SK_CASE(4, 2, 2, 12, 1)
  SG_SK_CASE(6, 3, 2, 1, 1) SG_SK_CASE(6, 3, 2, 3, 1) SG_SK_CASE(6, 3, 2, 6, 1) SG_SK_CASE(6, 2, 3, 12, 1)
#undef SG_SK_CASE
  return -1;
}
```

### pytorch-studiogan_amd/csrc/conv_v2.h

```cpp
#pragma once
#include "gemm_core.h"

struct ConvV2Params {
  const bf16_t* x; const bf16_t* w;
  int N, Hs, Ws, C, ldx;
  int Hin, Win, Ho, Wo;
  int R, S, pad_h, pad_w;
  int stride;
  int flags;
  int I, J, K;
  int cpt;
  int ntap;
  unsigned xbytes, wbytes;
  int wshift, hshift;
};

typedef __attribute__((address_space(1))) const void* sg_gptr_t;
typedef __attribute__((address_space(3))) void* sg_lptr_t;

template <int BI, int BJ, int NW, int TI, int TJ, bool VMAP = false, bool NOSTORE = false>
__device__ __forceinline__ void sg_conv_epilogue(f32x16 (&acc)[TI][TJ], char* smem, const float* sbias, const Epilogue<bf16_t>& epi,
                                                 int i0, int j0, int wi0, int wj0, float al, bool active = true, int vlog = 0, int vadd = 0,
                                                 float* stats = nullptr, int stats_C = 0, int stats_row = 0) {
  auto grow = [&](int jg) -> long long {
    if (VMAP) return (long long)(((jg >> vlog) << (vlog + 2)) + ((jg & ((1 << vlog) - 1)) << 1) + vadd);
    return (long long)jg;
  };
  const int tid = threadIdx.x, lane = tid & 63;
  const bool pool = (epi.flags & SG_EPI_POOL) != 0;
  constexpr int CP = BI * 2 + 16;
  __syncthreads();
  const int rows_out = pool ? BJ / 4 : BJ;
  const int jbase = pool ? (j0 >> 2) : j0, Jout = pool ? (epi.J >> 2) : epi.J;
  constexpr int CPR = BI / 8;
  const bool pre_mask = epi.mask != nullptr, pre_res = epi.res != nullptr;
  const bool pre_both = pre_mask && pre_res;
  const int ncr = ((epi.I - i0 < BI ? epi.I - i0 : BI) + 7) >> 3;
  auto stage_tile = [&](const bf16_t* src, int ld) {
    for (int idx = tid; idx < rows_out * CPR; idx += 64 * NW) {
      const int r = idx / CPR, c = idx - r * CPR;
      const int jg = jbase + r;
      u32x4 t = {0u, 0u, 0u, 0u};
      if (jg < Jout && c < ncr) t = *(const u32x4*)(src + grow(jg) * ld + i0 + c * 8);
      *(u32x4*)(smem + r * CP + c * 16) = t;
    }
  };
  uint32_t mbits[TI * TJ];
#pragma unroll
  for (int q = 0; q < TI * TJ; q++) mbits[q] = 0u;
  if (pre_both) {
    stage_tile(epi.mask, epi.ldm);
    __syncthreads();
    if (active) {
#pragma unroll
      for (int ta = 0; ta < TI; ta++)
#pragma unroll
        for (int tb = 0; tb < TJ; tb++) {
          const int jl = wj0 + tb * 32 + (lane & 31);
          const int jo = pool ? (jl >> 2) : jl;
          uint32_t bits = 0u;
#pragma unroll
          for (int g4 = 0; g4 < 4; g4++) {
            const int il = wi0 + ta * 32 + 8 * g4 + 4 * (lane >> 5);
            const u32x2 m = *(const u32x2*)(smem + jo * CP + il * 2);
#pragma unroll
            for (int e = 0; e < 4; e++) { const bf16_t h = (bf16_t)((m[e >> 1] >> (16 * (e & 1))) & 0xffffu); if (bf2f(h) > 0.f) bits |= 1u << (4 * g4 + e); }
          }
          mbits[ta * TJ + tb] = bits;
        }
    }
    __syncthreads();
    stage_tile((const bf16_t*)epi.res, epi.ldr);
    __syncthreads();
  } else if (pre_mask || pre_res) {
    stage_tile(pre_mask ? epi.mask : (const bf16_t*)epi.res, pre_mask ? epi.ldm : epi.ldr);
    __syncthreads();
  }
  const bool relu_out = (epi.flags & SG_EPI_RELU) != 0;
  if (active) {
#pragma unroll
  for (int ta = 0; ta < TI; ta++)
#pragma unroll
    for (int tb = 0; tb < TJ; tb++) {
      const int jl = wj0 + tb * 32 + (lane & 31);
#pragma unroll
      for (int g4 = 0; g4 < 4; g4++) {
        const int il = wi0 + ta * 32 + 8 * g4 + 4 * (lane >> 5);
        float v[4] = {acc[ta][tb][4 * g4 + 0], acc[ta][tb][4 * g4 + 1], acc[ta][tb][4 * g4 + 2], acc[ta][tb][4 * g4 + 3]};
        if (pool) {
#pragma unroll
          for (int e = 0; e < 4; e++) v[e] = quad_sum(v[e]);
        }
        const int jo = pool ? (jl >> 2) : jl;
        const bool act = (!pool || (lane & 3) == 0) && (jbase + jo < Jout);
        if (act) {
          char* loc = smem + jo * CP + il * 2;
#pragma unroll
          for (int e = 0; e < 4; e++) v[e] *= al;
          if (epi.bias) {
            const f32x4 b = *(const f32x4*)(sbias + il);
#pragma unroll
            for (int e = 0; e < 4; e++) v[e] += b[e];
          }
          if (pre_both) {
            const uint32_t bits = mbits[ta * TJ + tb] >> (4 * g4);
#pragma unroll
            for (int e = 0; e < 4; e++) if (!((bits >> e) & 1u)) v[e] = 0.f;
          } else if (pre_mask) {
            const u32x2 m = *(const u32x2*)loc;
#pragma unroll
            for (int e = 0; e < 4; e++) { const bf16_t h = (bf16_t)((m[e >> 1] >> (16 * (e & 1))) & 0xffffu); if (!(bf2f(h) > 0.f)) v[e] = 0.f; }
          }
          if (pre_res) {
            const u32x2 r = *(const u32x2*)loc;
#pragma unroll
            for (int e = 0; e < 4; e++) { const bf16_t h = (bf16_t)((r[e >> 1] >> (16 * (e & 1))) & 0xffffu); v[e] += epi.beta * bf2f(h); }
          }
          if (relu_out) {
#pragma unroll
            for (int e = 0; e < 4; e++) v[e] = fmaxf(v[e], 0.f);
          }
          u32x2 t;
          t[0] = pack2bf(v[0], v[1]);
          t[1] = pack2bf(v[2], v[3]);
          *(u32x2*)loc = t;
        }
      }
    }
  }
  __syncthreads();
  if (stats) {
    constexpr int PWV = BI / 2 / NW, RG = 64 / PWV;
    const int wv = tid >> 6, pl = lane % PWV, rg = lane / PWV;
    int rows_valid = Jout - jbase;
    if (rows_valid > rows_out) rows_valid = rows_out;
    float s1a = 0.f, s2a = 0.f, s1b = 0.f, s2b = 0.f;
    const int c2 = wv * PWV + pl;
    if (rg < RG) {
      constexpr int NIT = (BJ + RG - 1) / RG;
      const char* base = smem + rg * CP + c2 * 4;
#pragma unroll 8
      for (int k = 0; k < NIT; k++) {
        const int r = rg + k * RG;
        uint32_t v = *(const uint32_t*)(base + (r < BJ ? k * (RG * CP) : 0));
        v = r < rows_valid ? v : 0u;
        const float a = __uint_as_float(v << 16), b = __uint_as_float(v & 0xffff0000u);
        s1a += a; s2a += a * a; s1b += b; s2b += b * b;
      }
    }
    float t1a = s1a, t2a = s2a, t1b = s1b, t2b = s2b;
#pragma unroll
    for (int k = 1; k < RG; k++) {
      t1a += __shfl(s1a, lane + k * PWV, 64); t2a += __shfl(s2a, lane + k * PWV, 64);
      t1b += __shfl(s1b, lane + k * PWV, 64); t2b += __shfl(s2b, lane + k * PWV, 64);
    }
    const int c = i0 + 2 * c2;
    if (rg == 0 && c < epi.I) {
      f32x4 o4 = {t1a, t2a, t1b, t2b};
      *(f32x4*)(stats + ((long long)stats_row * stats_C + c) * 2) = o4;
    }
  }
  {
    bf16_t* o = (bf16_t*)epi.out;
    for (int idx = tid; idx < rows_out * CPR; idx += 64 * NW) {
      const int r = idx / CPR, c = idx - r * CPR;
      const int jg = jbase + r;
      if (NOSTORE) {
        const u32x4 v = *(const u32x4*)(smem + r * CP + c * 16);
        if (v[0] == 0x12345678u && v[1] == 0x9abcdef0u) *(u32x4*)(o + grow(jg) * epi.ldo + i0 + c * 8) = v;
      } else if (jg < Jout && c < ncr) *(u32x4*)(o + grow(jg) * epi.ldo + i0 + c * 8) = *(const u32x4*)(smem + r * CP + c * 16);
    }
  }
}

template <int BI, int WJ, int WI, int BJ, int SCHED, bool RELU, bool UP>
__global__ __launch_bounds__(64 * WJ * WI) void sg_conv_v2_kernel(ConvV2Params p, Epilogue<bf16_t> epi, int tilesI, int tilesJ) {
  constexpr int NW = WJ * WI;
  constexpr int QB = BJ * 128, PB = BI * 128, BUF = QB + PB;
  constexpr int NQ = BJ / 8 / NW;
  constexpr int NPI = (BI / 8 + NW - 1) / NW;
  constexpr int TJ = BJ / WJ / 32, TI = BI / WI / 32;
  static_assert(NW == 8 || NW == 4, "4 or 8 waves");
  static_assert(BJ % (8 * NW) == 0, "pixel tile / DMA groups");
  static_assert(BJ % (WJ * 32) == 0 && BI % (WI * 32) == 0, "tile/wave mismatch");
  extern __shared__ __attribute__((aligned(16))) char smem[];

  const int tid = threadIdx.x, lane = tid & 63;
  const int wave = __builtin_amdgcn_readfirstlane(tid >> 6);
  const int nt = tilesI * tilesJ;
  int bid = blockIdx.x;
  {
    const int xcd = bid & 7, q = nt >> 3, r = nt & 7;
    bid = (xcd < r ? xcd * (q + 1) : r * (q + 1) + (xcd - r) * q) + (bid >> 3);
  }
  const int tI = bid % tilesI, tJ = bid / tilesI;
  const int i0 = tI * BI, j0 = tJ * BJ;
  float* sbias = (float*)(smem + 2 * BUF);
  if (epi.bias) {
    for (int i = tid; i < BI; i += 64 * NW) sbias[i] = (i0 + i < epi.I) ? epi.bias[i0 + i] : 0.f;
  }

  const auto rsx = __builtin_amdgcn_make_buffer_rsrc((void*)p.x, 0, (int)p.xbytes, 0x00020000);
  const auto rsw = __builtin_amdgcn_make_buffer_rsrc((void*)p.w, 0, (int)p.wbytes, 0x00020000);
  const int sub = lane >> 3;
  const int lc = (lane & 7) ^ ((4 * wave + (lane >> 4)) & 7);
  const unsigned ldx2 = 2u * (unsigned)p.ldx;
  unsigned qoff[NQ];
  unsigned qinv[NQ];
  bool qph[NQ], qpw[NQ];
#pragma unroll
// ... 219 lines not shown
```

### pytorch-studiogan_amd/csrc/gemm_core.h

```cpp
#pragma once
#include "common.h"

#define SG_KC_STRIDE 80

__host__ __device__ constexpr int sg_mc_stride(int B, int es) {
  int s = B * es;
  if (es == 2) {
    while ((s % 128) != 64) s += 16;
    return s;
  }
  return s + 16;
}

template <typename T> __device__ __forceinline__ void set_elem(u32x4& v, int e, T x);
template <> __device__ __forceinline__ void set_elem<float>(u32x4& v, int e, float x) { v[e] = __float_as_uint(x); }
template <> __device__ __forceinline__ void set_elem<bf16_t>(u32x4& v, int e, bf16_t x) {
  v[e >> 1] |= ((uint32_t)x) << (16 * (e & 1));
}

template <typename T, bool FAST = false> struct StridedKC {
  static constexpr bool KC = true;
  static constexpr int VEC = ET<T>::VEC, BK = ET<T>::BK;
  const T* base; long long bstride; int ld; int rows; int K; int vec_ok;
  struct Chunk { const T* p; int k; bool valid; };
// ... 123 lines not shown
    u32x4 v = zero16();
    if (FAST || g.vec_ok) {
      bool ok;
      const unsigned off = g.tap_off(ch.n, ch.ho, ch.wo, ch.r, ch.s, ok);
      ok = ok & ch.valid & (ch.r < g.R);
      const u32x4 t = *(const u32x4*)(g.x + (ok ? off + (unsigned)ch.c : 0u));
      v = ok ? t : v;
    } else if constexpr (!FAST) {
      if (!ch.valid || ch.r >= g.R) return v;
      int r = ch.r, s = ch.s, c = ch.c;
#pragma unroll
      for (int e = 0; e < VEC; e++) {
        if (r < g.R) {
          const T* p;
          if (g.tap(ch.n, ch.ho, ch.wo, r, s, p)) set_elem<T>(v, e, p[c]);
        }
        c++; if (c == g.C) { c = 0; s++; if (s == g.S) { s = 0; r++; } }
      }
    }
    if (g.flags & SG_PIX_RELU) v = relu16<T>(v);
    return v;
  }
  __device__ __forceinline__ void advance(Chunk& ch) const {
    ch.c += BK;
    while (ch.c >= g.C) { ch.c -= g.C; ch.s++; if (ch.s == g.S) { ch.s = 0; ch.r++; } }
  }
};

template <typename T, bool FAST = false> struct ConvPixMC {
  static constexpr bool KC = false;
  static constexpr int VEC = ET<T>::VEC, BK = ET<T>::BK;
  PixGeom<T> g; int rows; int K;
  struct Chunk { int r, s, c; int pix; bool valid; };
  __device__ __forceinline__ void set_batch(int) {}
  __device__ __forceinline__ void init(Chunk& ch, int row, int k) const {
    ch.valid = row < rows;
    int rs = row / g.C; ch.c = row - rs * g.C; ch.r = rs / g.S; ch.s = rs - ch.r * g.S;
    ch.pix = k;
  }
  __device__ __forceinline__ u32x4 load(const Chunk& ch) const {
    u32x4 v = zero16();
    int n, ho, wo;
    if (FAST || g.vec_ok) {
      const bool inb = ch.valid & (ch.pix < K);
      g.pix_decompose(inb ? ch.pix : 0, n, ho, wo);
      bool ok;
      const unsigned off = g.tap_off(n, ho, wo, ch.r, ch.s, ok);
      ok = ok & inb;
      const u32x4 t = *(const u32x4*)(g.x + (ok ? off + (unsigned)ch.c : 0u));
      v = ok ? t : v;
    } else if constexpr (!FAST) {
      if (!ch.valid || ch.pix >= K) return v;
      g.pix_decompose(ch.pix, n, ho, wo);
      int r = ch.r, s = ch.s, c = ch.c;
#pragma unroll
      for (int e = 0; e < VEC; e++) {
        if (r < g.R) {
          const T* p;
          if (g.tap(n, ho, wo, r, s, p)) set_elem<T>(v, e, p[c]);
        }
        c++; if (c == g.C) { c = 0; s++; if (s == g.S) { s = 0; r++; } }
      }
    }
    if (g.flags & SG_PIX_RELU) v = relu16<T>(v);
    return v;
  }
  __device__ __forceinline__ void advance(Chunk& ch) const { ch.pix += BK; }
};

#define SG_EPI_OUT_F32 1
#define SG_EPI_ATOMIC 2
#define SG_EPI_POOL 4
#define SG_EPI_RELU 8
#define SG_EPI_RES_F32 16

template <typename T> struct Epilogue {
  void* out; long long out_bstride; int ldo;
  const float* bias;
  const void* res; long long res_bstride; int ldr; float beta;
  const T* mask; long long mask_bstride; int ldm;
  float alpha; const float* alpha_ptr;
  int flags; int I; int J;
  long long split_stride;

  __device__ __forceinline__ void set_batch(int b) {
    if (flags & (SG_EPI_OUT_F32 | SG_EPI_ATOMIC)) out = (float*)out + (long long)b * out_bstride;
    else out = (T*)out + (long long)b * out_bstride;
    if (res) {
      if (flags & SG_EPI_RES_F32) res = (const float*)res + (long long)b * res_bstride;
      else res = (const T*)res + (long long)b * res_bstride;
    }
    if (mask) mask += (long long)b * mask_bstride;
  }

  __device__ __forceinline__ void store(int j, int i0, float v[4], float a) const {
    if (prep(j, i0, v, a)) write(j, i0, v);
  }
  __device__ __forceinline__ bool prep(int& j, int i0, float v[4], float a) const {
    const int lane = threadIdx.x & 63;
    if (flags & SG_EPI_POOL) {
#pragma unroll
      for (int e = 0; e < 4; e++) v[e] = quad_sum(v[e]);
      if (lane & 3) return false;
      j >>= 2;
    }
    const int Jout = (flags & SG_EPI_POOL) ? (J >> 2) : J;
    if (j >= Jout || i0 >= I) return false;
    const int ne = (I - i0) < 4 ? (I - i0) : 4;
#pragma unroll
    for (int e = 0; e < 4; e++) {
      float x = v[e] * a;
      if (bias && e < ne) x += bias[i0 + e];
      v[e] = x;
    }
    if (mask) {
      const T* m = mask + (long long)j * ldm + i0;
#pragma unroll
      for (int e = 0; e < 4; e++) if (e < ne) { if (!(to_f<T>(m[e]) > 0.f)) v[e] = 0.f; }
    }
    if (res) {
      if (flags & SG_EPI_RES_F32) {
        const float* r = (const float*)res + (long long)j * ldr + i0;
#pragma unroll
        for (int e = 0; e < 4; e++) if (e < ne) v[e] += beta * r[e];
      } else {
        const T* r = (const T*)res + (long long)j * ldr + i0;
#pragma unroll
        for (int e = 0; e < 4; e++) if (e < ne) v[e] += beta * to_f<T>(r[e]);
      }
    }
    if (flags & SG_EPI_RELU) {
#pragma unroll
      for (int e = 0; e < 4; e++) v[e] = fmaxf(v[e], 0.f);
    }
    return true;
  }
  __device__ __forceinline__ void write(int j, int i0, const float v[4]) const {
    const int ne = (I - i0) < 4 ? (I - i0) : 4;
    if (flags & SG_EPI_ATOMIC) {
      float* o = (float*)out + (long long)j * ldo + i0;
#pragma unroll
      for (int e = 0; e < 4; e++) if (e < ne) unsafeAtomicAdd(o + e, v[e]);
    } else if ((flags & SG_EPI_OUT_F32) || sizeof(T) == 4) {
      float* o = (float*)out + (long long)j * ldo + i0;
      if (ne == 4 && ((ldo & 3) == 0) && ((((uintptr_t)out) & 15) == 0)) {
        f32x4 t = {v[0], v[1], v[2], v[3]};
        *(f32x4*)o = t;
      } else {
#pragma unroll
        for (int e = 0; e < 4; e++) if (e < ne) o[e] = v[e];
      }
    } else {
      bf16_t* o = (bf16_t*)out + (long long)j * ldo + i0;
      if (ne == 4 && ((ldo & 3) == 0) && ((((uintptr_t)out) & 7) == 0)) {
        u32x2 t;
        t[0] = (uint32_t)f2bf(v[0]) | ((uint32_t)f2bf(v[1]) << 16);
        t[1] = (uint32_t)f2bf(v[2]) | ((uint32_t)f2bf(v[3]) << 16);
        *(u32x2*)o = t;
      } else {
#pragma unroll
        for (int e = 0; e < 4; e++) if (e < ne) o[e] = f2bf(v[e]);
      }
    }
  }
};

// ... 254 lines not shown
```

### pytorch-studiogan_amd/functional/_base.py

```python
import os

import torch
import torch.distributed as dist

from .. import _lib as L
from .. import comm as _comm
from ..bank import ensure_grad


def _first_order_only(name):
    if torch.is_grad_enabled():
        raise NotImplementedError(name + ": second-order gradients (create_graph=True) are implemented for the discriminator's "
                                         "conv / BN / pooling / self-attention / head path only (gradient penalties, R1)")


def _param_grad_wanted(*params):
    for p in params:
        if p is None or not torch.is_tensor(p) or not p.requires_grad:
            continue
        try:
            if torch._C._will_engine_execute_node(torch.autograd.graph.get_gradient_edge(p).node):
                return True
        except Exception:
            return True
    return False


def _c(t):
    return t if t.is_contiguous() else t.contiguous()


_ZERO_POOL = {}
_ZERO_POOL_BYTES = 8 << 20
_ZERO_POOL_ON = [os.environ.get("SG_ZERO_POOL", "1") != "0"]


def zeros_small(shape, dtype, device):
    if isinstance(shape, int):
        shape = (shape,)
    n = 1
    for d in shape:
        n *= int(d)
    nbytes = n * torch.empty((), dtype=dtype).element_size()
    if not _ZERO_POOL_ON[0] or nbytes == 0 or nbytes > (_ZERO_POOL_BYTES >> 1) or torch.device(device).type != "cuda":
        return torch.zeros(shape, dtype=dtype, device=device)
    key = torch.device(device)
    ent = _ZERO_POOL.get(key)
    step = (nbytes + 255) & ~255
    if ent is None or ent[1] + step > _ZERO_POOL_BYTES:
        ent = _ZERO_POOL[key] = [torch.zeros(_ZERO_POOL_BYTES, dtype=torch.uint8, device=device), 0]
    off = ent[1]
    ent[1] = off + step
    return ent[0][off:off + nbytes].view(dtype).view(shape)


def zeros_like_small(t):
    return zeros_small(tuple(t.shape), t.dtype, t.device)


_SEQ = [0]
_STATS_OFFER = [None]
_BN_FUSED_STATS = [os.environ.get("SG_BN_FUSED_STATS", "1") != "0"]
_CBN_MERGED = [os.environ.get("SG_CBN_MERGED", "1") != "0"]


def _tick():
    _SEQ[0] += 1


def _offer_stats(out, st, rows, C):
    _STATS_OFFER[0] = (_SEQ[0], out.data_ptr(), tuple(out.shape), st, rows, C, out._version)


def _take_stats(x):
    ent, _STATS_OFFER[0] = _STATS_OFFER[0], None
    if ent is None or ent[0] != _SEQ[0] - 1 or ent[1] != x.data_ptr() or ent[2] != tuple(x.shape) or ent[5] != x.shape[3] or ent[6] != x._version:
        return None
    return ent[3], ent[4]


class f32_mode:
    MODES = {"exact": 0, "bf16x3": 3}

    def __init__(self, mode):
        if mode not in self.MODES:
            raise ValueError(f"f32_mode: {mode!r} (one of {sorted(self.MODES)})")
        self.mode = self.MODES[mode]

    def __enter__(self):
        self.saved = L.lib().sg_get_f32_mode()
        L.call("sg_set_f32_mode", self.mode)
        return self

    def __exit__(self, *exc):
        L.call("sg_set_f32_mode", self.saved)
        return False


def conv2d_raw(x, w_ptr, Cin, Cout, R, S, stride=1, pad_h=0, pad_w=0, pix_flags=0, epi_flags=0, bias=None, res=None, mask=None,
               alpha=1.0, beta=1.0, alpha_ptr=None, out=None, ldx=None, transposed_out_hw=None, out_coff=0, x_coff=0, desc=None):
    N, Hs, Ws = x.shape[0], x.shape[1], x.shape[2]
    ldx = x.shape[3] if ldx is None else ldx
    up = 2 if (pix_flags & L.PIX_UPSAMPLE) else 1
    Hin, Win = Hs * up, Ws * up
    if pix_flags & L.PIX_TRANSPOSED:
        Ho, Wo = transposed_out_hw
    else:
        Ho = (Hin + 2 * pad_h - R) // stride + 1
        Wo = (Win + 2 * pad_w - S) // stride + 1
    pool = bool(epi_flags & L.EPI_POOL)
    Hy, Wy = (Ho // 2, Wo // 2) if pool else (Ho, Wo)
    if out is None:
        odt = torch.float32 if (epi_flags & L.EPI_OUT_F32) else x.dtype
        out = torch.empty((N, Hy, Wy, Cout), dtype=odt, device=x.device)
    d = desc if desc is not None else L.ConvFwdDesc()
    d.dtype = L.dt(x)
    d.N, d.Hs, d.Ws, d.C, d.ldx = N, Hs, Ws, Cin, ldx
    d.Ho, d.Wo, d.Cout = Ho, Wo, Cout
    d.R, d.S, d.stride, d.pad_h, d.pad_w = R, S, stride, pad_h, pad_w
    d.pix_flags, d.epi_flags = pix_flags, epi_flags
    d.alpha, d.beta = alpha, beta
    d.x, d.w = L.ptr(x) + x_coff * x.element_size(), w_ptr
    d.bias = L.ptr(bias)
    d.res = L.ptr(res)
    d.mask = L.ptr(mask)
    d.out = L.ptr(out) + out_coff * out.element_size()
    d.alpha_ptr = L.ptr(alpha_ptr)
    d.ldo = out.shape[-1]
    d.ldr = res.shape[-1] if res is not None else 0
    d.ldm = mask.shape[-1] if mask is not None else 0
    if desc is not None:
        return out
    L.call("sg_conv2d_fwd", d, L.stream())
    return out


def conv2d_skip_raw(x, w_ptr, Cin, Cout, x2, w2_ptr, C2, x2_up=False, pix_flags=0, epi_flags=0, bias=None, bias2=None, alpha=1.0, dry=False, stats=False):
    sk = L.ConvSkipDesc()
    out = conv2d_raw(x, w_ptr, Cin, Cout, 3, 3, 1, 1, 1, pix_flags, epi_flags, bias=bias, alpha=alpha, desc=sk.main)
    sk.x2, sk.w2, sk.bias2 = L.ptr(x2), w2_ptr, L.ptr(bias2)
    sk.C2, sk.ldx2, sk.x2_up = C2, x2.shape[3], 1 if x2_up else 0
    if L.lib().sg_conv2d_fwd_skip_ok(L.C.byref(sk)) != 1:
        return None
    if dry:
        return out
    if stats and not (epi_flags & L.EPI_POOL):
        rows = L.lib().sg_conv2d_fwd_skip_stat_rows(L.C.byref(sk))
        st = torch.empty((rows, Cout, 2), dtype=torch.float32, device=x.device)
        sk.stats = st.data_ptr()
        L.call("sg_conv2d_fwd_skip", sk, L.stream())
        _offer_stats(out, st, rows, Cout)
        return out
    L.call("sg_conv2d_fwd_skip", sk, L.stream())
    return out


def conv2d_wgrad_raw(x, dy, dw_ptr, Cin, Cout, R, S, Ho, Wo, stride=1, pad_h=0, pad_w=0, x_flags=0, g_flags=0, alpha=1.0,
                     alpha_ptr=None, splits=0, no_tr=0, ldg=None, dy_coff=0, dbias=None):
    d = L.ConvWgradDesc()
    d.dtype = L.dt(x)
    d.N = x.shape[0]
    d.xHs, d.xWs, d.C, d.ldx, d.x_flags = x.shape[1], x.shape[2], Cin, x.shape[3], x_flags
    d.gHs, d.gWs, d.Cout, d.ldg, d.g_flags = dy.shape[1], dy.shape[2], Cout, (dy.shape[3] if ldg is None else ldg), g_flags
    d.Ho, d.Wo = Ho, Wo
    d.R, d.S, d.stride, d.pad_h, d.pad_w = R, S, stride, pad_h, pad_w
    d.alpha = alpha
    d.x, d.dy, d.dw = L.ptr(x), L.ptr(dy) + dy_coff * dy.element_size(), dw_ptr
    d.alpha_ptr = L.ptr(alpha_ptr)
    d.splits, d.no_tr = splits, no_tr
    fused = False
    if dbias is not None:
        d.dbias = L.ptr(dbias)
        fused = L.lib().sg_conv2d_wgrad_fuses_bias(L.C.byref(d)) == 1
        if not fused:
            d.dbias = None
    sp, wf = L.C.c_int(0), L.C.c_longlong(0)
    L.call("sg_conv2d_wgrad_plan", d, L.C.byref(sp), L.C.byref(wf))
    work = None
    if wf.value > 0:
        work = torch.empty(wf.value, dtype=torch.float32, device=x.device)
        d.splits, d.work, d.work_floats = sp.value, work.data_ptr(), wf.value
    L.call("sg_conv2d_wgrad", d, L.stream())
    return fused


def quad_pack_raw(src_ptr, dst, mode, M, Cs):
    L.call("sg_quad_pack", L.dt(dst), mode, src_ptr, L.ptr(dst), M, Cs, L.stream())
    return dst


def conv2d_q_raw(x, wq_ptr, form, Cin, Cout, pix_flags=0, epi_flags=0, bias=None, res=None, mask=None, alpha=1.0, beta=1.0, dry=False,
                 x2=None, w2q_ptr=None, bias2=None, stats=False, x2_norelu=False):
    N = x.shape[0]
    if form == L.Q_POOL:
        if x.shape[1] % 2 or x.shape[2] % 2:
            return None
        Hl, Wl = x.shape[1] // 2, x.shape[2] // 2
        oshape = (N, Hl, Wl, Cout)
    else:
        Hl, Wl = x.shape[1], x.shape[2]
        oshape = (N, 2 * Hl, 2 * Wl, Cout)
    if x.dtype != torch.bfloat16:
        return None
    d = L.ConvQDesc()
    d.dtype, d.form = L.dt(x), form
    d.N, d.Hl, d.Wl, d.C, d.ldx, d.Cout = N, Hl, Wl, Cin, x.shape[3], Cout
    d.pix_flags, d.epi_flags, d.alpha, d.beta = pix_flags, epi_flags, alpha, beta
    out = torch.empty(oshape, dtype=x.dtype, device=x.device)
    d.x, d.wq, d.bias, d.res, d.mask, d.out = L.ptr(x), wq_ptr, L.ptr(bias), L.ptr(res), L.ptr(mask), L.ptr(out)
    d.ldo = Cout
    d.ldr = res.shape[-1] if res is not None else 0
    d.ldm = mask.shape[-1] if mask is not None else 0
    if x2 is not None:
        d.x2, d.w2q, d.bias2, d.C2, d.ldx2 = L.ptr(x2), w2q_ptr, L.ptr(bias2), x2.shape[3], x2.shape[3]
        d.x2_norelu = 1 if x2_norelu else 0
    if L.lib().sg_conv2d_q_ok(L.C.byref(d)) != 1:
        return None
    if not dry:
        st = None
        if stats:
            rows = L.lib().sg_conv2d_q_stat_rows(L.C.byref(d))
            st = torch.empty((rows, Cout, 2), dtype=torch.float32, device=x.device)
            d.stats = st.data_ptr()
        L.call("sg_conv2d_q", d, L.stream())
        if st is not None:
            _offer_stats(out, st, rows, Cout)
    return out


def conv2d_q_wgrad_raw(x, dy, dw_ptr, form, Cin, Cout, x_flags=0, alpha=1.0, dbias=None, splits=0):
    if x.dtype != torch.bfloat16:
        return False
    d = L.ConvQWgradDesc()
    d.dtype, d.form = L.dt(x), form
    lo = dy if form == L.Q_POOL else x
    d.N, d.Hl, d.Wl = lo.shape[0], lo.shape[1], lo.shape[2]
    d.C, d.ldx, d.x_flags, d.Cout, d.ldg = Cin, x.shape[3], x_flags, Cout, dy.shape[3]
    d.alpha = alpha
    d.x, d.dy, d.dw, d.dbias = L.ptr(x), L.ptr(dy), dw_ptr, L.ptr(dbias)
    d.splits = splits
    sp, wf = L.C.c_int(0), L.C.c_longlong(0)
    L.call("sg_conv2d_q_wgrad_plan", d, L.C.byref(sp), L.C.byref(wf))
    if sp.value == 0:
        return False
    work = torch.empty(wf.value, dtype=torch.float32, device=x.device)
    d.work, d.work_floats, d.splits = work.data_ptr(), wf.value, sp.value
    L.call("sg_conv2d_q_wgrad", d, L.stream())
    return True


def gemm_raw(dtype, p, p_form, ldp, q, q_form, ldq, out, ldo, I, J, K, batch=1, p_bs=0, q_bs=0, out_bs=0, bias=None, res=None,
             res_bs=0, ldr=0, beta=1.0, alpha=1.0, alpha_ptr=None, epi_flags=0, splits=1, no_tr=0):
    d = L.GemmDesc()
    d.dtype, d.p_form, d.q_form = dtype, p_form, q_form
    d.I, d.J, d.K, d.batch = I, J, K, batch
    d.p = p if isinstance(p, int) else L.ptr(p)
    d.q = q if isinstance(q, int) else L.ptr(q)
    d.out = out if isinstance(out, int) else L.ptr(out)
    d.p_bstride, d.ldp, d.q_bstride, d.ldq, d.out_bstride, d.ldo = p_bs, ldp, q_bs, ldq, out_bs, ldo
    d.bias = bias if (bias is None or isinstance(bias, int)) else L.ptr(bias)
    d.res = res if (res is None or isinstance(res, int)) else L.ptr(res)
    d.res_bstride, d.ldr, d.beta = res_bs, ldr, beta
    d.alpha = alpha
    d.alpha_ptr = L.ptr(alpha_ptr)
    d.epi_flags, d.splits, d.no_tr = epi_flags, splits, no_tr
    L.call("sg_gemm", d, L.stream())


_DGRAD_SPLITK = [os.environ.get("SG_DGRAD_SPLITK", "1") != "0"]


def gemm_dgrad_rows(w_ptr, dy, dx, B, K, O):
    S = 1
    tiles = ((K + 127) // 128) * ((B + 127) // 128)
    if _DGRAD_SPLITK[0] and tiles < 64:
        while S < 32 and tiles * S < 256 and O % (2 * S) == 0 and O // (2 * S) >= 96:
            S *= 2
    if S == 1:
        gemm_raw(L.F32, w_ptr, 1, K, dy, 0, dy.shape[1] if torch.is_tensor(dy) else O, dx, K, K, B, O)
        return dx
    ldq = dy.shape[1]
    ws = torch.empty((S, B, K), dtype=torch.float32, device=dx.device)
    gemm_raw(L.F32, w_ptr, 1, K, dy, 0, ldq, ws, K, K, B, O // S, batch=S, p_bs=(O // S) * K, q_bs=O // S, out_bs=B * K)
    torch.sum(ws, dim=0, out=dx)
    return dx


__all__ = ['L', 'zeros_small', 'zeros_like_small', '_BN_FUSED_STATS', '_CBN_MERGED', '_DGRAD_SPLITK', '_SEQ', '_STATS_OFFER', '_c', '_comm', '_first_order_only', '_offer_stats', '_param_grad_wanted', '_take_stats', '_tick', 'conv2d_q_raw', 'conv2d_q_wgrad_raw', 'conv2d_raw', 'conv2d_skip_raw', 'conv2d_wgrad_raw', 'dist', 'ensure_grad', 'f32_mode', 'gemm_dgrad_rows', 'gemm_raw', 'os', 'quad_pack_raw', 'torch']
```

### pytorch-studiogan_amd/functional/attention.py

```python
from ._base import *
from .layout import ConvertFn
from .conv import ConvCfg, ConvDgradFn, ConvFn, _conv_wgrad

class MaxPool2Fn(torch.autograd.Function):

    @staticmethod
    def forward(ctx, x):
        x = _c(x)
        B, H, W, Cc = x.shape
        y = torch.empty((B, (H // 2) * (W // 2), Cc), dtype=x.dtype, device=x.device)
        idx = torch.empty((B, (H // 2) * (W // 2), Cc), dtype=torch.uint8, device=x.device)
        L.call("sg_maxpool2_fwd", L.dt(x), L.ptr(x), Cc, L.ptr(y), Cc, L.ptr(idx), B, H, W, Cc, L.stream())
        ctx.save_for_backward(idx)
        ctx.dims = (B, H, W, Cc)
        return y

    @staticmethod
    def backward(ctx, dy):
        (idx,) = ctx.saved_tensors
        if torch.is_grad_enabled():
            return MaxPool2BwdFn.apply(dy, idx, ctx.dims)
        return _maxpool2_bwd(dy, idx, ctx.dims)


# ... 215 lines not shown
        gemm_raw(sd, phi, 1, Dp, dS, 0, HW4, dtheta, Dp, Dp, HW, HW4, batch=B, p_bs=HW4 * Dp, q_bs=HW * HW4, out_bs=HW * Dp)
        dphi = torch.empty((B, HW4, Dp), dtype=T, device=dev)
        gemm_raw(sd, theta, 1, Dp, dS, 1, HW4, dphi, Dp, Dp, HW4, HW, batch=B, p_bs=HW * Dp, q_bs=HW * HW4, out_bs=HW4 * Dp)
        return dtheta, dphi, dg


def attn_proj_on():
    return os.environ.get("SG_ATTN_PROJ", "1") != "0"


def attn_proj_ok(x, rts):
    rt_t, rt_p, rt_g = rts
    if x.dtype != torch.bfloat16 or x.dim() != 4 or rt_t.rows_pad != rt_p.rows_pad or any(r.RS != 1 or r.trans or r.cin_pad != x.shape[3] for r in rts):
        return False
    B, H, W, Cc = x.shape
    return L.lib().sg_attn_proj_ok(B, H, W, Cc, Cc, rt_t.rows_pad, rt_g.rows_pad) == 1


class AttnProjFn(torch.autograd.Function):

    @staticmethod
    def forward(ctx, x, w_theta, w_phi, w_g, rts, slot, link=None):
        x = _c(x)
        rt_t, rt_p, rt_g = rts
        bank = rt_t.bank()
        B, H, W, Cc = x.shape
        Dp, Cg = rt_t.rows_pad, rt_g.rows_pad
        ctx.link = link
        if link is not None and link.chain:
            link.pending += 1
        for _ in rts:
            _tick()
        HW4 = (H // 2) * (W // 2)
        theta = torch.empty((B, H, W, Dp), dtype=x.dtype, device=x.device)
        phi = torch.empty((B, HW4, Dp), dtype=x.dtype, device=x.device)
        g = torch.empty((B, HW4, Cg), dtype=x.dtype, device=x.device)
        iphi = torch.empty((B, HW4, Dp), dtype=torch.uint8, device=x.device)
        ig = torch.empty((B, HW4, Cg), dtype=torch.uint8, device=x.device)
        L.call("sg_attn_proj_fwd", L.ptr(x), Cc, bank.w_fwd(slot, rt_t), bank.w_fwd(slot, rt_p), bank.w_fwd(slot, rt_g), L.ptr(theta), L.ptr(phi), L.ptr(g),
               L.ptr(iphi), L.ptr(ig), B, H, W, Cc, Dp, Cg, 0, L.stream())
        ctx.save_for_backward(x, iphi, ig)
        ctx.rts, ctx.slot = rts, slot
        ctx.weights = (w_theta, w_phi, w_g)
        return theta, phi, g

    @staticmethod
    def backward(ctx, dtheta, dphi, dg):
        x, iphi, ig = ctx.saved_tensors
        rts, slot = ctx.rts, ctx.slot
        B, H, W, Cc = x.shape
        cfg = ConvCfg(1, 1)
        if torch.is_grad_enabled():
            if not ctx.needs_input_grad[0]:
                return (None,) * 7
            with torch.enable_grad():
                outs = (ConvFn.apply(x, ctx.weights[0], None, None, rts[0], slot, cfg, None),
                        MaxPool2Fn.apply(ConvFn.apply(x, ctx.weights[1], None, None, rts[1], slot, cfg, None)),
                        MaxPool2Fn.apply(ConvFn.apply(x, ctx.weights[2], None, None, rts[2], slot, cfg, None)))
                (dx,) = torch.autograd.grad(outs, [x], [dtheta, dphi, dg], create_graph=True)
            return (dx,) + (None,) * 6
        bank = rts[0].bank()
        Dp, Cg = rts[0].rows_pad, rts[2].rows_pad
        dtheta, dphi, dg = _c(dtheta), _c(dphi), _c(dg)
        dx = None
        skip_dx = ctx.link.take() if ctx.link is not None else None
        if ctx.needs_input_grad[0]:
            dx = torch.empty_like(x)
            L.call("sg_attn_proj_bwd_data", L.ptr(dtheta), L.ptr(dphi), L.ptr(dg), L.ptr(iphi), L.ptr(ig), bank.w_dgrad(slot, rts[0]), bank.w_dgrad(slot, rts[1]),
                   bank.w_dgrad(slot, rts[2]), L.ptr(skip_dx), L.ptr(dx), B, H, W, Cc, Dp, Cg, L.stream())
        elif skip_dx is not None:
            raise RuntimeError("GradLink: a residual gradient was handed over but the attention block's input needs no gradient")
        if ctx.link is not None and ctx.link.chain:
            ctx.link.pending -= 1
        for k, (dy, idx) in enumerate(((dtheta, None), (dphi, iphi), (dg, ig))):
            if ctx.needs_input_grad[1 + k]:
                full = dy if idx is None else _maxpool2_bwd(dy, idx, (B, H, W, dy.shape[-1]))
                _conv_wgrad(x, full, rts[k], slot, cfg)
        return (dx,) + (None,) * 6


class AttnOutFn(torch.autograd.Function):

    @staticmethod
    def forward(ctx, x, o, weight, sigma, rt, slot, link=None):
        bank = rt.bank()
        x, o = _c(x), _c(o)
        ctx.link = link
        y = conv2d_raw(o, bank.w_fwd(slot, rt), rt.Cin, rt.rows, 1, 1, res=x, alpha_ptr=sigma)
        ctx.save_for_backward(o, sigma)
        ctx.rt, ctx.slot = rt, slot
        ctx.sigma_param = sigma
        ctx.weight = weight
        return y

    @staticmethod
    def backward(ctx, dy):
        o, sigma = ctx.saved_tensors
        rt, slot = ctx.rt, ctx.slot
        if torch.is_grad_enabled():
            if _param_grad_wanted(ctx.weight, ctx.sigma_param):
                raise NotImplementedError("create_graph=True is supported for input gradients only (WGAN-GP / R1 path)")
            do = ScalePtrFn.apply(ConvDgradFn.apply(dy, o, ctx.weight, rt, slot, ConvCfg(1, 1)), ctx.sigma_param) if ctx.needs_input_grad[1] else None
            return (dy if ctx.needs_input_grad[0] else None), do, None, None, None, None, None
        bank = rt.bank()
        dy = _c(dy)
        N, H, W, Cc = dy.shape
        do = None
        if ctx.needs_input_grad[3]:
            t = conv2d_raw(o, bank.w_fwd(slot, rt), rt.Cin, rt.rows, 1, 1)
            g = ensure_grad(ctx.sigma_param)
            L.call("sg_dot", L.dt(dy), L.ptr(dy), L.ptr(t), dy.numel(), L.ptr(g), 1.0, None, L.stream())
        if ctx.needs_input_grad[1]:
            do = conv2d_raw(dy, bank.w_dgrad(slot, rt), rt.rows, rt.Cin, 1, 1, alpha_ptr=sigma)
        if ctx.needs_input_grad[2]:
            conv2d_wgrad_raw(o, dy, bank.dwt(slot, rt), rt.Cin, rt.rows, 1, 1, H, W, alpha_ptr=sigma)
        dx = dy
        if ctx.link is not None and ctx.link.pending > 0 and ctx.needs_input_grad[0]:
            ctx.link.dx, dx = dy, None
        return dx, do, None, None, None, None, None


__all__ = ['AttnCoreFn', 'AttnOutFn', 'AttnPooledFn', 'AttnProjFn', 'attn_proj_ok', 'attn_proj_on', 'BmmFn', 'MaxPool2BwdFn', 'MaxPool2Fn', 'ScalePtrFn', 'SoftmaxRowsBwdFn', 'SoftmaxRowsFn', '_attn_reference_graph', '_maxpool2_bwd']
```

### pytorch-studiogan_amd/functional/conv.py

```python
import ctypes

from ._base import *

class ConvCfg:
    __slots__ = ("R", "S", "stride", "pad_h", "pad_w", "in_relu", "in_upsample", "out_pool", "stats")

    def __init__(self, R, S, stride=1, pad_h=0, pad_w=0, in_relu=False, in_upsample=False, out_pool=False, stats=False):
        self.R, self.S, self.stride, self.pad_h, self.pad_w = R, S, stride, pad_h, pad_w
        self.in_relu, self.in_upsample, self.out_pool = in_relu, in_upsample, out_pool
        self.stats = stats


class GradLink:
    __slots__ = ("dx", "chain", "pending")

    def __init__(self, chain=False):
        self.dx = None
        self.chain = chain
        self.pending = 0

    def take(self):
        t, self.dx = self.dx, None
        return t


_GRAD_LINK = [os.environ.get("SG_GRAD_LINK", "1") != "0"]


_QUAD = [os.environ.get("SG_QUAD", "1") != "0"]


def _quad_form(rt, cfg, x):
    if not _QUAD[0] or x.dtype != torch.bfloat16 or cfg.R != 3 or cfg.S != 3 or cfg.stride != 1 or cfg.pad_h != 1 or cfg.pad_w != 1:
        return None
    if cfg.out_pool == cfg.in_upsample or rt.trans or rt.RS != 9:
        return None
    if rt.cin_pad % 32 or (rt.rows_pad % 64 and rt.rows_pad % 96):
        return None
    return L.Q_POOL if cfg.out_pool else L.Q_UP


def _conv_fwd(x, rt, slot, cfg, bias, res=None, stats=False):
    bank = rt.bank()
    Cin = x.shape[3]
    form = _quad_form(rt, cfg, x)
    if form is not None:
        y = conv2d_q_raw(x, bank.w_quad(slot, rt, form), form, Cin, rt.rows_pad, L.PIX_RELU if cfg.in_relu else 0, 0, bias=bias, res=res,
                         stats=stats and _BN_FUSED_STATS[0] and rt.rows_pad == rt.rows)
        if y is not None:
            return y
    pf = (L.PIX_RELU if cfg.in_relu else 0) | (L.PIX_UPSAMPLE if cfg.in_upsample else 0)
    ef = L.EPI_POOL if cfg.out_pool else 0
    return conv2d_raw(x, bank.w_fwd(slot, rt), Cin, rt.rows_pad, cfg.R, cfg.S, cfg.stride, cfg.pad_h, cfg.pad_w, pf, ef, bias=bias, res=res,
                      alpha=0.25 if cfg.out_pool else 1.0)


def _conv_wgrad(x, dy, rt, slot, cfg, dbias=None):
    bank = rt.bank()
    N, Hs, Ws, Cin = x.shape
    form = _quad_form(rt, cfg, x)
    if form is not None and conv2d_q_wgrad_raw(x, dy, bank.dwt(slot, rt), form, Cin, rt.rows_pad, L.PIX_RELU if cfg.in_relu else 0, dbias=dbias):
        return dbias is not None
    up = 2 if cfg.in_upsample else 1
    Ho = (Hs * up + 2 * cfg.pad_h - cfg.R) // cfg.stride + 1
    Wo = (Ws * up + 2 * cfg.pad_w - cfg.S) // cfg.stride + 1
    pool = cfg.out_pool
    xf = (L.PIX_RELU if cfg.in_relu else 0) | (L.PIX_UPSAMPLE if cfg.in_upsample else 0)
    return conv2d_wgrad_raw(x, dy, bank.dwt(slot, rt), Cin, rt.rows_pad, cfg.R, cfg.S, Ho, Wo, cfg.stride, cfg.pad_h, cfg.pad_w, xf,
                            L.PIX_UPSAMPLE if pool else 0, alpha=0.25 if pool else 1.0, dbias=dbias)


def _conv_dgrad(dy, x, rt, slot, cfg, res=None):
    bank = rt.bank()
    N, Hs, Ws, Cin = x.shape
    form = _quad_form(rt, cfg, x)
    if form is not None and dy.shape[3] == rt.rows_pad:
        dx = conv2d_q_raw(dy, bank.w_quad(slot, rt, 2 + form), 1 - form, rt.rows_pad, Cin, 0, 0, mask=x if cfg.in_relu else None, res=res)
        if dx is not None:
            return dx
    up = 2 if cfg.in_upsample else 1
    Hin, Win = Hs * up, Ws * up
    pool = cfg.out_pool
    if cfg.stride != 1:
        assert not (pool or cfg.in_upsample), "upsample / pooling fusion is stride-1 only"
        return conv2d_raw(dy, bank.w_dgrad(slot, rt), rt.rows_pad, Cin, cfg.R, cfg.S, cfg.stride, cfg.pad_h, cfg.pad_w, L.PIX_TRANSPOSED, 0,
                          mask=x if cfg.in_relu else None, res=res, transposed_out_hw=(Hin, Win), ldx=dy.shape[3])
    pf = L.PIX_UPSAMPLE if pool else 0
    ef = L.EPI_POOL if cfg.in_upsample else 0
    return conv2d_raw(dy, bank.w_dgrad(slot, rt), rt.rows_pad, Cin, cfg.R, cfg.S, 1, cfg.R - 1 - cfg.pad_h, cfg.S - 1 - cfg.pad_w, pf, ef,
                      mask=x if cfg.in_relu else None, res=res, alpha=0.25 if pool else 1.0, ldx=dy.shape[3])


class ConvDgradFn(torch.autograd.Function):

    @staticmethod
    def forward(ctx, dy, x, weight, rt, slot, cfg):
        dy = _c(dy)
        ctx.save_for_backward(dy, x)
        ctx.rt, ctx.slot, ctx.cfg = rt, slot, cfg
        return _conv_dgrad(dy, x, rt, slot, cfg)

    @staticmethod
    def backward(ctx, ddx):
        dy, x = ctx.saved_tensors
        rt, slot, cfg = ctx.rt, ctx.slot, ctx.cfg
        bank = rt.bank()
        t = _c(ddx)
        if cfg.in_relu:
            m = torch.empty_like(t)
            L.call("sg_relu_mask", L.dt(t), L.ptr(t), L.ptr(x), L.ptr(m), t.numel(), L.stream())
            t = m
        N, Hs, Ws, Cin = x.shape
        up = 2 if cfg.in_upsample else 1
        Ho = (Hs * up + 2 * cfg.pad_h - cfg.R) // cfg.stride + 1
        Wo = (Ws * up + 2 * cfg.pad_w - cfg.S) // cfg.stride + 1
        pool = cfg.out_pool
        g_dy = None
        if ctx.needs_input_grad[0]:
            g_dy = conv2d_raw(t, bank.w_fwd(slot, rt), Cin, rt.rows_pad, cfg.R, cfg.S, cfg.stride, cfg.pad_h, cfg.pad_w,
                              L.PIX_UPSAMPLE if cfg.in_upsample else 0, L.EPI_POOL if pool else 0, alpha=0.25 if pool else 1.0)
        if ctx.needs_input_grad[2]:
            conv2d_wgrad_raw(t, dy, bank.dwt(slot, rt), Cin, rt.rows_pad, cfg.R, cfg.S, Ho, Wo, cfg.stride, cfg.pad_h, cfg.pad_w,
                             L.PIX_UPSAMPLE if cfg.in_upsample else 0, L.PIX_UPSAMPLE if pool else 0, alpha=0.25 if pool else 1.0)
        return g_dy, None, None, None, None, None


class ConvFn(torch.autograd.Function):

    @staticmethod
    def forward(ctx, x, weight, bias, res, rt, slot, cfg, link=None):
        bank = rt.bank()
        x = _c(x)
        N, Hs, Ws, Cin = x.shape
        assert Cin == rt.cin_pad, f"conv input channels {Cin} != {rt.cin_pad}"
        ctx.link = link
        if link is not None and link.chain:
            link.pending += 1
        if res is not None:
            res = _c(res)
        bias_k = bias
        if bias is not None and rt.rows_pad != rt.rows:
            bias_k = zeros_small(rt.rows_pad, torch.float32, x.device)
            bias_k[:rt.rows].copy_(bias.detach())
        _tick()
        y = _conv_fwd(x, rt, slot, cfg, bias_k, res, stats=cfg.stats)
        ctx.save_for_backward(x)
        ctx.rt, ctx.slot, ctx.cfg = rt, slot, cfg
        ctx.bias = bias
        ctx.weight = weight
        ctx.has_res = res is not None
        return y

    @staticmethod
    def backward(ctx, dy):
        (x,) = ctx.saved_tensors
        rt, slot, cfg = ctx.rt, ctx.slot, ctx.cfg
        bank = rt.bank()
        if torch.is_grad_enabled():
            if _param_grad_wanted(ctx.weight, ctx.bias):
                raise NotImplementedError("create_graph=True is supported for input gradients only (WGAN-GP path)")
            dx = ConvDgradFn.apply(dy, x, ctx.weight, rt, slot, cfg) if ctx.needs_input_grad[0] else None
            return dx, None, None, (dy if ctx.has_res else None), None, None, None, None
        dy = _c(dy)
        N, Hs, Ws, Cin = x.shape
        up = 2 if cfg.in_upsample else 1
        Hin, Win = Hs * up, Ws * up
        Ho = (Hin + 2 * cfg.pad_h - cfg.R) // cfg.stride + 1
        Wo = (Win + 2 * cfg.pad_w - cfg.S) // cfg.stride + 1
        pool = cfg.out_pool
        scale = 0.25 if pool else 1.0
        dx = None
        skip_dx = ctx.link.take() if ctx.link is not None else None
        if ctx.needs_input_grad[0]:
            dx = _conv_dgrad(dy, x, rt, slot, cfg, res=skip_dx)
        elif skip_dx is not None:
            raise RuntimeError("GradLink: a skip gradient was handed over but this convolution's input needs no gradient")
        if ctx.link is not None and ctx.link.chain:
            ctx.link.pending -= 1
            if ctx.link.pending > 0 and dx is not None:
                ctx.link.dx, dx = dx, None
        want_db = ctx.bias is not None and ctx.needs_input_grad[2]
        db_done = False
        if ctx.needs_input_grad[1]:
            g = ensure_grad(ctx.bias) if (want_db and rt.rows_pad == rt.rows) else None
            db_done = _conv_wgrad(x, dy, rt, slot, cfg, dbias=g)
        if want_db and not db_done:
            g = ensure_grad(ctx.bias)
            rows = dy.shape[0] * dy.shape[1] * dy.shape[2]
            L.call("sg_colsum", L.dt(dy), L.ptr(dy), dy.shape[3], None, 0, rows, rt.rows, L.ptr(g), 1.0, L.stream())
        dres = dy if ctx.has_res else None
        return dx, None, None, dres, None, None, None, None


class ConvSkipFn(torch.autograd.Function):

    @staticmethod
    def forward(ctx, h, x, w2, b2, w0, b0, rt2, rt0, slot, cfg2, cfg0, link=None):
        bank = rt2.bank()
        ctx.link = link
        h, x = _c(h), _c(x)
        _tick()
        assert cfg2.R == 3 and cfg0.R == 1 and cfg2.out_pool == cfg0.out_pool and not cfg2.in_upsample and (cfg0.in_relu == cfg2.in_relu or not cfg0.in_relu)
        pf = L.PIX_RELU if cfg2.in_relu else 0
        same_relu = cfg0.in_relu == cfg2.in_relu
        ef = L.EPI_POOL if cfg2.out_pool else 0
        al = 0.25 if cfg2.out_pool else 1.0
        y = None
        plain = rt2.rows_pad == rt2.rows and rt0.rows_pad == rt0.rows and b2 is not None and b0 is not None
        if plain and same_relu and h.dtype == torch.bfloat16 and _SKIP_FUSION[0] and (h.shape[1] >= 16 or _SKIP_FUSION[0] == "all") and _quad_form(rt2, cfg2, h) is None:
            y = conv2d_skip_raw(h, bank.w_fwd(slot, rt2), h.shape[3], rt2.rows, x, bank.w_fwd(slot, rt0), x.shape[3], cfg0.in_upsample, pf, ef,
                                bias=b2, bias2=b0, alpha=al, stats=cfg2.stats and _BN_FUSED_STATS[0])
        if y is None and plain and _quad_form(rt2, cfg2, h) == L.Q_POOL and _SKIP_FUSION[0] and (rt0.cin_pad % 32 == 0 or rt0.cin_pad == 8) and not cfg0.in_upsample:
            y = conv2d_q_raw(h, bank.w_quad(slot, rt2, L.Q_POOL), L.Q_POOL, h.shape[3], rt2.rows, pf, 0, bias=b2,
                             x2=x, w2q_ptr=bank.w_quad(slot, rt0, 5 if rt0.cin_pad == 8 else 4), bias2=b0, x2_norelu=not same_relu)
        if y is None:
            hh = _conv_fwd(h, rt2, slot, cfg2, b2)
            pf0 = (L.PIX_RELU if cfg0.in_relu else 0) | (L.PIX_UPSAMPLE if cfg0.in_upsample else 0)
            y = conv2d_raw(x, bank.w_fwd(slot, rt0), x.shape[3], rt0.rows_pad, 1, 1, 1, 0, 0, pf0, ef, bias=b0, res=hh, alpha=al)
        ctx.save_for_backward(h, x)
        ctx.rt2, ctx.rt0, ctx.slot, ctx.cfg2, ctx.cfg0 = rt2, rt0, slot, cfg2, cfg0
        ctx.w2, ctx.b2, ctx.w0, ctx.b0 = w2, b2, w0, b0
        return y

    @staticmethod
    def backward(ctx, dy):
        h, x = ctx.saved_tensors
        rt2, rt0, slot, cfg2, cfg0 = ctx.rt2, ctx.rt0, ctx.slot, ctx.cfg2, ctx.cfg0
        if torch.is_grad_enabled():
            if _param_grad_wanted(ctx.w2, ctx.b2, ctx.w0, ctx.b0):
                raise NotImplementedError("create_graph=True is supported for input gradients only (WGAN-GP path)")
            dh = ConvDgradFn.apply(dy, h, ctx.w2, rt2, slot, cfg2) if ctx.needs_input_grad[0] else None
            dx = ConvDgradFn.apply(dy, x, ctx.w0, rt0, slot, cfg0) if ctx.needs_input_grad[1] else None
            return (dh, dx) + (None,) * 10
        dy = _c(dy)
        bank = rt2.bank()
        outs = []
        want2 = ctx.b2 is not None and ctx.needs_input_grad[3]
        want0 = ctx.b0 is not None and ctx.needs_input_grad[5]
        shared_db = None
        if want2 and want0 and ctx.needs_input_grad[2] and ctx.needs_input_grad[4] and rt2.rows_pad == rt2.rows and rt0.rows == rt2.rows:
            shared_db = zeros_small(rt2.rows, torch.float32, dy.device)
        for inp, rt, cfg, w_i, b_i, wp, bp in ((h, rt2, cfg2, 2, 3, ctx.w2, ctx.b2), (x, rt0, cfg0, 4, 5, ctx.w0, ctx.b0)):
            k = 0 if inp is h else 1
            N, Hs, Ws, Cin = inp.shape
            up = 2 if cfg.in_upsample else 1
            Ho, Wo = Hs * up, Ws * up
            pool = cfg.out_pool
            outs.append(_conv_dgrad(dy, inp, rt, slot, cfg) if ctx.needs_input_grad[k] else None)
            want_db = bp is not None and ctx.needs_input_grad[b_i]
            db_done = False
            if ctx.needs_input_grad[w_i]:
                xf = (L.PIX_RELU if cfg.in_relu else 0) | (L.PIX_UPSAMPLE if cfg.in_upsample else 0)
                g = ensure_grad(bp) if (want_db and rt.rows_pad == rt.rows) else None
                if k == 0 and shared_db is not None:
                    g = shared_db
                elif k == 1 and shared_db is not None:
                    g = None
                db_done = _conv_wgrad(inp, dy, rt, slot, cfg, dbias=g)
                if k == 0 and shared_db is not None:
                    if db_done:
                        for bq in (ctx.b2, ctx.b0):
                            L.call("sg_axpby", L.F32, L.ptr(shared_db), L.ptr(ensure_grad(bq)), rt2.rows, 1.0, 1.0, L.stream())
                        continue
                    shared_db = None
                elif k == 1 and shared_db is not None:
                    continue
            if want_db and not db_done:
                g = ensure_grad(bp)
                L.call("sg_colsum", L.dt(dy), L.ptr(dy), dy.shape[3], None, 0, dy.shape[0] * dy.shape[1] * dy.shape[2], rt.rows, L.ptr(g), 1.0, L.stream())
        if ctx.link is not None and outs[1] is not None and _GRAD_LINK[0]:
            ctx.link.dx = outs[1]
            outs[1] = None
        return (outs[0], outs[1]) + (None,) * 10


_SKIP_FUSION = [{"0": False, "all": "all"}.get(os.environ.get("SG_SKIP_FUSION", "1"), True)]


class SliceUpFn(torch.autograd.Function):

    @staticmethod
    def forward(ctx, x, C, up, link=None):
        x = _c(x)
        N, Hs, Ws, ld = x.shape
        ctx.dims = (N, Hs, Ws, ld, C, up)
        ctx.link = link
        if C == ld and up == 1:
            return x.view_as(x)
        y = torch.empty((N, Hs * up, Ws * up, C), dtype=x.dtype, device=x.device)
        L.call("sg_slice_up_fwd", L.dt(x), L.ptr(x), L.ptr(y), N, Hs, Ws, ld, C, up, L.stream())
        return y

    @staticmethod
    def backward(ctx, dy):
        _first_order_only("SliceUpFn")
        N, Hs, Ws, ld, C, up = ctx.dims
        dy = _c(dy)
        if C == ld and up == 1:
            dx = dy
        else:
            dx = torch.empty((N, Hs, Ws, ld), dtype=dy.dtype, device=dy.device)
            L.call("sg_slice_up_bwd", L.dt(dy), L.ptr(dy), L.ptr(dx), N, Hs, Ws, ld, C, up, L.stream())
        if ctx.link is not None and _GRAD_LINK[0]:
            ctx.link.dx, dx = dx, None
        return dx, None, None, None


class CatConvFn(torch.autograd.Function):

    @staticmethod
    def forward(ctx, x, weight, bias, rt, slot):
        bank = rt.bank()
        x = _c(x)
        N, H, W, Cin = x.shape
        Cc = rt.rows
        out = torch.empty((N, H, W, Cin + Cc), dtype=x.dtype, device=x.device)
        L.call("sg_copy_channels", L.dt(x), L.ptr(x), Cin, L.ptr(out), Cin + Cc, N * H * W, Cin, L.stream())
        conv2d_raw(x, bank.w_fwd(slot, rt), Cin, Cc, 1, 1, bias=bias, out=out, out_coff=Cin)
        ctx.save_for_backward(x)
        ctx.rt, ctx.slot, ctx.bias = rt, slot, bias
        ctx.weight = weight
        return out

    @staticmethod
    def backward(ctx, dy):
        (x,) = ctx.saved_tensors
        rt, slot = ctx.rt, ctx.slot
        if torch.is_grad_enabled():
            if _param_grad_wanted(ctx.weight, ctx.bias):
                raise NotImplementedError("create_graph=True is supported for input gradients only (WGAN-GP / R1 path)")
            return (CatConvDgradFn.apply(dy, ctx.weight, rt, slot, x.shape[3]) if ctx.needs_input_grad[0] else None), None, None, None, None
        bank = rt.bank()
        dy = _c(dy)
        N, H, W, Cin = x.shape
        Cc = rt.rows
        ld = Cin + Cc
        dx = None
        if ctx.needs_input_grad[0]:
            dx = conv2d_raw(dy, bank.w_dgrad(slot, rt), Cc, Cin, 1, 1, res=dy, ldx=ld, x_coff=Cin)
        if ctx.needs_input_grad[1]:
            conv2d_wgrad_raw(x, dy, bank.dwt(slot, rt), Cin, Cc, 1, 1, H, W, ldg=ld, dy_coff=Cin)
        if ctx.bias is not None and ctx.needs_input_grad[2]:
            g = ensure_grad(ctx.bias)
            L.call("sg_colsum", L.dt(dy), L.ptr(dy) + Cin * dy.element_size(), ld, None, 0, N * H * W, Cc, L.ptr(g), 1.0, L.stream())
        return dx, None, None, None, None


class CatConvDgradFn(torch.autograd.Function):

    @staticmethod
    def forward(ctx, dy, weight, rt, slot, Cin):
        dy = _c(dy)
        ctx.save_for_backward(dy)
        ctx.rt, ctx.slot, ctx.Cin = rt, slot, Cin
        Cc = rt.rows
        return conv2d_raw(dy, rt.bank().w_dgrad(slot, rt), Cc, Cin, 1, 1, res=dy, ldx=Cin + Cc, x_coff=Cin)
# ... 325 lines not shown
```

### pytorch-studiogan_amd/ops.py

```python
import torch
import torch.nn as nn
from torch.nn import init
import torch.nn.functional as F_

from . import functional as F
from .bank import get_bank

COMPUTE_DTYPE = torch.float32


def to_nhwc(x, dtype, cpad=0):
    if x.dim() != 4:
        raise RuntimeError("expected a 4-D NCHW tensor")
    if x.dtype == torch.uint8:
        return F.u8_to_nhwc(x, dtype, max(cpad, 3))
    if cpad > x.shape[1]:
        return F.NchwToNhwcFn.apply(x.float(), dtype, cpad)
    if x.dtype == dtype and x.is_contiguous(memory_format=torch.channels_last) and not (x.shape[1] > 1 and x.is_contiguous() and x.shape[2] * x.shape[3] > 1):
        return x.permute(0, 2, 3, 1)
    if x.dtype == torch.float32 and x.is_contiguous():
        return F.NchwToNhwcFn.apply(x, dtype)
    y = x.permute(0, 2, 3, 1).contiguous()
    if y.dtype != dtype:
        y = F.ConvertFn.apply(y, dtype)
    return y


def to_nchw(y):
    return y.permute(0, 3, 1, 2)


BLOCK_HOOKS = [False]


def block_boundary(net, bi, act):
    if not BLOCK_HOOKS[0]:
        return act
    tf = net.__dict__.get("_sg_teacher")
    return act if tf is None else tf(bi, act)


def _root_and_bank(m):
    root = m.__dict__.get("_sg_root")
    root = root() if root is not None else None
    if root is None:
        root = m
    dtype = getattr(root, "compute_dtype", None) or getattr(m, "compute_dtype", None) or COMPUTE_DTYPE
    return root, get_bank(root, dtype)


def _standalone_slot(m, x):
    root, bank = _root_and_bank(m)
    if root is m:
        need_graph = torch.is_grad_enabled() and (x.requires_grad or any(p.requires_grad for p in m.parameters()))
        return bank.begin_forward(need_graph)
    return bank.current


class _WeightLayerMixin:
    _sg_weight_layer = True

    def _sg_setup(self, kind, rows, cols, cin, rs, sn, eps=1e-6):
        self._sg_kind, self._sg_rows, self._sg_cols, self._sg_cin, self._sg_rs = kind, rows, cols, cin, rs
        self._sg_sn = bool(sn)
        self._sg_eps = eps
        if sn:
            w = self.weight
            del self._parameters["weight"]
            self.register_parameter("weight_orig", w)
            with torch.no_grad():
                mat = w.reshape(rows, cols)
                u = F_.normalize(w.new_empty(rows).normal_(0, 1), dim=0, eps=eps)
                v = F_.normalize(w.new_empty(cols).normal_(0, 1), dim=0, eps=eps)
            self.register_buffer("weight_u", u)
            self.register_buffer("weight_v", v)

    @property
    def master_weight(self):
        return self.weight_orig if self._sg_sn else self.weight

    def __getattr__(self, name):
        if name == "weight" and "weight_orig" in self.__dict__.get("_parameters", {}):
            return self._parameters["weight_orig"].data
        return super().__getattr__(name)


class Conv2d(_WeightLayerMixin, nn.Conv2d):
    def __init__(self, in_channels, out_channels, kernel_size, stride=1, padding=0, dilation=1, groups=1, bias=True, sn=False,
                 cout_pad=0):
        nn.Conv2d.__init__(self, in_channels, out_channels, kernel_size, stride, padding, dilation, groups, bias)
        if self.dilation != (1, 1) or self.groups != 1:
            raise NotImplementedError("dilation/groups are not on the StudioGAN hot path")
        if self.kernel_size[0] != self.kernel_size[1] and self.stride != (1, 1):
            raise NotImplementedError
        kh, kw = self.kernel_size
        self._sg_rows_pad = cout_pad
        self._sg_dgrad_noflip = self.stride[0] != 1
        self._sg_setup("conv", out_channels, in_channels * kh * kw, in_channels, kh * kw, sn)

    def forward_nhwc(self, x, slot=None, in_relu=False, in_upsample=False, out_pool=False, res=None, link=None, stats=False):
        rt = self._sg_rt
        slot = slot if slot is not None else rt.bank().current
        kh, kw = self.kernel_size
        cfg = F.ConvCfg(kh, kw, self.stride[0], self.padding[0], self.padding[1], in_relu, in_upsample, out_pool, stats and self.training)
        return F.ConvFn.apply(x, self.master_weight, self.bias, res, rt, slot, cfg, link)

    def forward(self, x):
        slot = _standalone_slot(self, x)
        _, bank = _root_and_bank(self)
        y = self.forward_nhwc(to_nhwc(x, bank.dtype, getattr(self, "_sg_cin_pad", 0)), slot)
        if self._sg_rows_pad and self._sg_rows_pad != self.out_channels:
            y = y[..., :self.out_channels]
        return to_nchw(y)


def conv_skip_nhwc(conv_main, conv_skip, h, x, slot=None, in_relu=False, out_pool=False, skip_upsample=False, link=None, stats=False, skip_relu=None):
    rt2, rt0 = conv_main._sg_rt, conv_skip._sg_rt
    slot = slot if slot is not None else rt2.bank().current
    cfg2 = F.ConvCfg(3, 3, 1, 1, 1, in_relu, False, out_pool, stats)
    cfg0 = F.ConvCfg(1, 1, 1, 0, 0, in_relu if skip_relu is None else skip_relu, skip_upsample, out_pool)
    return F.ConvSkipFn.apply(h, x, conv_main.master_weight, conv_main.bias, conv_skip.master_weight, conv_skip.bias, rt2, rt0, slot, cfg2, cfg0, link)


class ConvTranspose2d(_WeightLayerMixin, nn.ConvTranspose2d):

    def __init__(self, in_channels, out_channels, kernel_size, stride=2, padding=0, dilation=1, groups=1, bias=True, sn=False):
        nn.ConvTranspose2d.__init__(self, in_channels, out_channels, kernel_size, stride, padding, 0, groups, bias, dilation)
        if self.dilation != (1, 1) or self.groups != 1 or self.output_padding != (0, 0):
            raise NotImplementedError
        kh, kw = self.kernel_size
        self._sg_trans = True
        self._sg_dgrad_noflip = True
        self._sg_setup("conv", out_channels, in_channels * kh * kw, in_channels, kh * kw, sn)

    def forward_nhwc(self, x, slot=None):
        rt = self._sg_rt
        slot = slot if slot is not None else rt.bank().current
        kh, kw = self.kernel_size
        cfg = F.ConvCfg(kh, kw, self.stride[0], self.padding[0], self.padding[1])
        return F.ConvTransposeFn.apply(x, self.master_weight, self.bias, rt, slot, cfg)

    def forward(self, x, output_size=None):
        slot = _standalone_slot(self, x)
        _, bank = _root_and_bank(self)
        return to_nchw(self.forward_nhwc(to_nhwc(x, bank.dtype), slot))


class Linear(_WeightLayerMixin, nn.Linear):
    def __init__(self, in_features, out_features, bias=True, sn=False):
        nn.Linear.__init__(self, in_features, out_features, bias)
        self._sg_setup("linear", out_features, in_features, in_features, 1, sn)

    def forward_rt(self, x, slot=None, const_bias=None):
        rt = self._sg_rt
        slot = slot if slot is not None else rt.bank().current
        return F.LinearFn.apply(x, self.master_weight, self.bias, rt, slot, const_bias)

    def forward(self, x):
        slot = _standalone_slot(self, x)
        shp = x.shape
        y = self.forward_rt(x.reshape(-1, shp[-1]), slot)
        return y.reshape(*shp[:-1], self.out_features)


class Embedding(_WeightLayerMixin, nn.Embedding):
    def __init__(self, num_embeddings, embedding_dim, sn=False):
        nn.Embedding.__init__(self, num_embeddings, embedding_dim)
        self._sg_setup("embedding", num_embeddings, embedding_dim, embedding_dim, 1, sn)

    def forward(self, idx):
        if not self._sg_sn:
            return F.EmbeddingFn.apply(self.weight, idx.reshape(-1)).reshape(*idx.shape, self.embedding_dim)
        slot = _standalone_slot(self, idx)
        rt = self._sg_rt
        return F.SNEmbeddingFn.apply(self.weight_orig, idx.reshape(-1), rt, slot).reshape(*idx.shape, self.embedding_dim)


_NBT_BULK = [False]


class bump_batches_tracked:

    def __init__(self, root):
        self.on = False
        bns = root.__dict__.get("_sg_bn_list")
        if bns is None:
            bns = [m for m in root.modules() if isinstance(m, BatchNorm2d)]
            root.__dict__["_sg_bn_list"] = bns
        if not bns or _NBT_BULK[0]:
            return
        for m in bns:
            if not (m.training and m.track_running_stats and m.running_mean is not None and m.num_batches_tracked is not None):
                return
        from .bank import get_buffer_arena
        ar = get_buffer_arena(root)
        if ar.inumel != len(bns) or any(b is not m.num_batches_tracked for b, m in zip(ar.ibufs, bns)):
            return
        with torch.no_grad():
            ar.idata.add_(1)
        self.on = True

    def __enter__(self):
        if self.on:
            _NBT_BULK[0] = True
        return self

    def __exit__(self, *a):
        if self.on:
            _NBT_BULK[0] = False


class BatchNorm2d(nn.BatchNorm2d):
    sync_group = None

    def _cfg(self, relu):
        batch_stats = self.training or (self.running_mean is None)
        track = self.training and self.track_running_stats and self.running_mean is not None
        mom = 0.0 if self.momentum is None else self.momentum
        return F.BNCfg(batch_stats, track, self.eps, mom, relu, self.sync_group)

    def forward_nhwc(self, x, gain=None, bias=None, relu=False, link=None, packed=False):
        cfg = self._cfg(relu)
        cfg.packed = packed
        if cfg.track and self.num_batches_tracked is not None and not _NBT_BULK[0]:
            self.num_batches_tracked.add_(1)
        if gain is None and self.affine:
            gain, bias = self.weight, self.bias
        return F.BNFn.apply(x, gain, bias, self.running_mean, self.running_var, cfg, link)

    def forward(self, x):
        dtype = getattr(self, "compute_dtype", None) or (x.dtype if x.dtype in (torch.float32, torch.bfloat16) else COMPUTE_DTYPE)
        return to_nchw(self.forward_nhwc(to_nhwc(x, dtype)))


class ConditionalBatchNorm2d(nn.Module):

    def __init__(self, in_features, out_features, MODULES):
        super().__init__()
        self.in_features = in_features
        self.bn = batchnorm_2d(out_features, eps=1e-4, momentum=0.1, affine=False)
        self.gain = MODULES.g_linear(in_features=in_features, out_features=out_features, bias=False)
        self.bias = MODULES.g_linear(in_features=in_features, out_features=out_features, bias=False)
        self.register_buffer("_ones", torch.ones(out_features), persistent=False)
        self.register_buffer("_ones2", torch.cat([torch.ones(out_features), torch.zeros(out_features)]), persistent=False)

    def forward_nhwc(self, x, y, slot=None, relu=False, link=None):
        pre = slot.__dict__.get("cbn_rows") if slot is not None else None
        if pre:
            gb = pre.pop(id(self), None)
            if gb is not None:
                return self.bn.forward_nhwc(x, gb, None, relu, link, packed=True)
        if F._CBN_MERGED[0] and self.gain.bias is None and self.bias.bias is None:
            rt_g, rt_b = self.gain._sg_rt, self.bias._sg_rt
            slot = slot if slot is not None else rt_g.bank().current
            gb = F.CbnAffineFn.apply(y, self.gain.master_weight, self.bias.master_weight, rt_g, rt_b, slot, self._ones2)
            return self.bn.forward_nhwc(x, gb, None, relu, link, packed=True)
        gain = self.gain.forward_rt(y, slot, const_bias=self._ones)
        bias = self.bias.forward_rt(y, slot)
        return self.bn.forward_nhwc(x, gain, bias, relu, link)

    def forward(self, x, y):
        _, bank = _root_and_bank(self.gain)
        if self.gain.__dict__.get("_sg_root") is None:
            raise RuntimeError("ConditionalBatchNorm2d must live inside a studiogan_amd backbone (its two linears share the network's bank)")
        return to_nchw(self.forward_nhwc(to_nhwc(x, bank.dtype), y))


class SelfAttention(nn.Module):

    def __init__(self, in_channels, is_generator, MODULES):
        super().__init__()
        self.in_channels = in_channels
        conv = MODULES.g_conv2d if is_generator else MODULES.d_conv2d
        c8, c2 = in_channels // 8, in_channels // 2
        pad8 = (c8 + 7) // 8 * 8
        self.conv1x1_theta = conv(in_channels=in_channels, out_channels=c8, kernel_size=1, stride=1, padding=0, bias=False)
        self.conv1x1_phi = conv(in_channels=in_channels, out_channels=c8, kernel_size=1, stride=1, padding=0, bias=False)
        self.conv1x1_g = conv(in_channels=in_channels, out_channels=c2, kernel_size=1, stride=1, padding=0, bias=False)
        self.conv1x1_attn = conv(in_channels=c2, out_channels=in_channels, kernel_size=1, stride=1, padding=0, bias=False)
        for m in (self.conv1x1_theta, self.conv1x1_phi):
            m._sg_rows_pad = pad8
        self.sigma = nn.Parameter(torch.zeros(1), requires_grad=True)

    def forward_nhwc(self, x, slot=None):
        link = F.GradLink(chain=True) if (F._GRAD_LINK[0] and torch.is_grad_enabled() and x.requires_grad) else None
        rt = self.conv1x1_attn._sg_rt
        slot = slot if slot is not None else rt.bank().current
        convs = (self.conv1x1_theta, self.conv1x1_phi, self.conv1x1_g)
        rts = tuple(m._sg_rt for m in convs)
        if F.attn_proj_on() and all(m.bias is None for m in convs) and F.attn_proj_ok(x, rts):
            theta, phi_p, g_p = F.AttnProjFn.apply(x, convs[0].master_weight, convs[1].master_weight, convs[2].master_weight, rts, slot, link)
            o = F.AttnPooledFn.apply(theta, phi_p, g_p)
        else:
            theta = self.conv1x1_theta.forward_nhwc(x, slot, link=link)
            phi = self.conv1x1_phi.forward_nhwc(x, slot, link=link)
            g = self.conv1x1_g.forward_nhwc(x, slot, link=link)
            o = F.AttnCoreFn.apply(theta, phi, g)
        return F.AttnOutFn.apply(x, o, self.conv1x1_attn.master_weight, self.sigma, rt, slot, link)

    def forward(self, x):
        _, bank = _root_and_bank(self.conv1x1_theta)
        return to_nchw(self.forward_nhwc(to_nhwc(x, bank.dtype)))


class LeCamEMA(object):

    def __init__(self, init=7777, decay=0.9, start_iter=0):
        self.G_loss = init
        self.D_loss_real = init
        self.D_loss_fake = init
        self.D_real = init
        self.D_fake = init
        self.decay = decay
        self.start_itr = start_iter

    def update(self, cur, mode, itr):
        decay = 0.0 if itr < self.start_itr else self.decay
        if mode not in ("G_loss", "D_loss_real", "D_loss_fake", "D_real", "D_fake"):
            raise ValueError(mode)
        setattr(self, mode, getattr(self, mode) * decay + cur * (1 - decay))


def conv2d(in_channels, out_channels, kernel_size, stride=1, padding=0, dilation=1, groups=1, bias=True):
    return Conv2d(in_channels, out_channels, kernel_size, stride, padding, dilation, groups, bias, sn=False)


def snconv2d(in_channels, out_channels, kernel_size, stride=1, padding=0, dilation=1, groups=1, bias=True):
    return Conv2d(in_channels, out_channels, kernel_size, stride, padding, dilation, groups, bias, sn=True)


def deconv2d(in_channels, out_channels, kernel_size, stride=2, padding=0, dilation=1, groups=1, bias=True):
    return ConvTranspose2d(in_channels, out_channels, kernel_size, stride, padding, dilation, groups, bias, sn=False)


def sndeconv2d(in_channels, out_channels, kernel_size, stride=2, padding=0, dilation=1, groups=1, bias=True):
    return ConvTranspose2d(in_channels, out_channels, kernel_size, stride, padding, dilation, groups, bias, sn=True)


def linear(in_features, out_features, bias=True):
    return Linear(in_features, out_features, bias, sn=False)


def snlinear(in_features, out_features, bias=True):
    return Linear(in_features, out_features, bias, sn=True)


def embedding(num_embeddings, embedding_dim):
    return Embedding(num_embeddings, embedding_dim, sn=False)


def sn_embedding(num_embeddings, embedding_dim):
    return Embedding(num_embeddings, embedding_dim, sn=True)


def batchnorm_2d(in_features, eps=1e-4, momentum=0.1, affine=True):
    return BatchNorm2d(in_features, eps=eps, momentum=momentum, affine=affine, track_running_stats=True)


def init_weights(modules, initialize):
    for module in modules():
        if isinstance(module, (nn.Conv2d, nn.ConvTranspose2d, nn.Linear)):
            w = module.master_weight if hasattr(module, "master_weight") else module.weight
            if initialize == "ortho":
                init.orthogonal_(w)
            elif initialize == "N02":
                init.normal_(w, 0, 0.02)
            elif initialize in ["glorot", "xavier"]:
                init.xavier_uniform_(w)
            else:
                continue
            if module.bias is not None:
                module.bias.data.fill_(0.)
        elif isinstance(module, nn.Embedding):
            w = module.master_weight if hasattr(module, "master_weight") else module.weight
            if initialize == "ortho":
                init.orthogonal_(w)
            elif initialize == "N02":
                init.normal_(w, 0, 0.02)
            elif initialize in ["glorot", "xavier"]:
                init.xavier_uniform_(w)

# ... 32 lines not shown
```

Baseline: 2062.

## Emit 1-bit sign planes in D forward and use them as ReLU masks in dgrad

```diff
diff --git a/include/sgamd.h b/include/sgamd.h
--- a/include/sgamd.h
+++ b/include/sgamd.h
@@ -38,6 +38,8 @@
   int ldo, ldr, ldm;
 } sg_conv_fwd_desc;
 int sg_conv2d_fwd(const sg_conv_fwd_desc* d, sg_stream_t stream);
+int sg_conv2d_fwd_planes(const sg_conv_fwd_desc* d, const void* mask_plane, void* out_plane, sg_stream_t stream);
+int sg_sign_plane_ok(int dtype, int C);
 int sg_set_f32_mode(int mode);
 int sg_get_f32_mode(void);
 
@@ -49,6 +51,7 @@
 } sg_conv_skip_desc;
 int sg_conv2d_fwd_skip_stat_rows(const sg_conv_skip_desc* d);
 int sg_conv2d_fwd_skip(const sg_conv_skip_desc* d, sg_stream_t stream);
+int sg_conv2d_fwd_skip_planes(const sg_conv_skip_desc* d, void* out_plane, sg_stream_t stream);
 int sg_conv2d_fwd_skip_ok(const sg_conv_skip_desc* d);
 long long sg_conv_rs_launches(void);
 
@@ -70,6 +73,7 @@
 } sg_convq_desc;
 int sg_conv2d_q_stat_rows(const sg_convq_desc* d);
 int sg_conv2d_q(const sg_convq_desc* d, sg_stream_t stream);
+int sg_conv2d_q_planes(const sg_convq_desc* d, const void* mask_plane, void* out_plane, sg_stream_t stream);
 int sg_conv2d_q_ok(const sg_convq_desc* d);
 int sg_quad_pack(int dtype, int mode, const void* src, void* dst, int M, int Cs, sg_stream_t stream);
 typedef struct { const void* src; void* dst; int M, Cs, mode, pad_; } sg_quad_item;
diff --git a/pytorch-studiogan_amd/_lib.py b/pytorch-studiogan_amd/_lib.py
--- a/pytorch-studiogan_amd/_lib.py
+++ b/pytorch-studiogan_amd/_lib.py
@@ -103,6 +103,10 @@
     "sg_conv2d_fwd": [C.POINTER(ConvFwdDesc), _vp],
     "sg_conv2d_fwd_skip": [C.POINTER(ConvSkipDesc), _vp],
     "sg_conv2d_fwd_skip_ok": [C.POINTER(ConvSkipDesc)],
+    "sg_sign_plane_ok": [_i, _i],
+    "sg_conv2d_fwd_planes": [C.POINTER(ConvFwdDesc), _vp, _vp, _vp],
+    "sg_conv2d_fwd_skip_planes": [C.POINTER(ConvSkipDesc), _vp, _vp],
+    "sg_conv2d_q_planes": [C.POINTER(ConvQDesc), _vp, _vp, _vp],
     "sg_conv_rs_launches": [],
     "sg_conv2d_q": [C.POINTER(ConvQDesc), _vp],
     "sg_conv2d_q_ok": [C.POINTER(ConvQDesc)],
diff --git a/pytorch-studiogan_amd/backbones/big_resnet.py b/pytorch-studiogan_amd/backbones/big_resnet.py
--- a/pytorch-studiogan_amd/backbones/big_resnet.py
+++ b/pytorch-studiogan_amd/backbones/big_resnet.py
@@ -175,14 +175,16 @@
         if self.cpad:
             self.conv2d1._sg_cin_pad = self.conv2d0._sg_cin_pad = self.cpad
 
-    def forward_nhwc(self, x, slot):
-        h = self.conv2d1.forward_nhwc(x, slot)
+    def forward_nhwc(self, x, slot, out_plane=None):
+        fused = self.apply_d_sn and self.cpad == 8 and x.dtype == torch.bfloat16 and not x.requires_grad
+        hp = F.SignPlane() if (fused and torch.is_grad_enabled()) else None
+        h = self.conv2d1.forward_nhwc(x, slot, out_plane=hp)
         if not self.apply_d_sn:
             h = self.bn1.forward_nhwc(h, relu=True)
             h = self.conv2d2.forward_nhwc(h, slot, out_pool=True)
         else:
-            if self.cpad == 8 and h.dtype == torch.bfloat16 and not x.requires_grad:
-                return ops.conv_skip_nhwc(self.conv2d2, self.conv2d0, h, x, slot, in_relu=True, out_pool=True, skip_relu=False)
+            if fused:
+                return ops.conv_skip_nhwc(self.conv2d2, self.conv2d0, h, x, slot, in_relu=True, out_pool=True, skip_relu=False, h_plane=hp, out_plane=out_plane)
             h = self.conv2d2.forward_nhwc(h, slot, in_relu=True, out_pool=True)
         x0 = F.AvgPool2Fn.apply(x)
         if not self.apply_d_sn:
@@ -208,12 +210,14 @@
             self.bn2 = MODULES.d_bn(in_features=out_channels)
         self.average_pooling = nn.AvgPool2d(2)
 
-    def forward_nhwc(self, x, slot):
+    def forward_nhwc(self, x, slot, x_plane=None, out_plane=None):
         if self.apply_d_sn:
             if self.downsample or self.ch_mismatch:
                 link = F.GradLink()
-                h = self.conv2d1.forward_nhwc(x, slot, in_relu=True, link=link)
-                return ops.conv_skip_nhwc(self.conv2d2, self.conv2d0, h, x, slot, in_relu=True, out_pool=self.downsample, link=link)
+                hp = F.SignPlane() if torch.is_grad_enabled() else None
+                h = self.conv2d1.forward_nhwc(x, slot, in_relu=True, link=link, x_plane=x_plane, out_plane=hp)
+                return ops.conv_skip_nhwc(self.conv2d2, self.conv2d0, h, x, slot, in_relu=True, out_pool=self.downsample, link=link,
+                                          h_plane=hp, x_plane=x_plane, out_plane=out_plane)
             h = self.conv2d1.forward_nhwc(x, slot, in_relu=True)
             h = self.conv2d2.forward_nhwc(h, slot, in_relu=True, out_pool=False)
             return F.AddReluFn.apply(h, x)
@@ -284,9 +288,19 @@
         slot = bank.begin_forward(_need_graph(self, x))
         h = ops.to_nhwc(x, dtype, self.blocks[0][0].cpad)
         nxt = bank.boundaries(self.blocks) if bank.exchange is not None else None
+        flat = [block for blocklist in self.blocks for block in blocklist]
+        planes = torch.is_grad_enabled()
+        k, xp = 0, None
         for bi, blocklist in enumerate(self.blocks):
             for block in blocklist:
-                h = block.forward_nhwc(h, slot)
+                k += 1
+                nb = flat[k] if k < len(flat) else None
+                op = F.SignPlane() if (planes and isinstance(nb, DiscBlock) and nb.apply_d_sn and (nb.downsample or nb.ch_mismatch)) else None
+                if isinstance(block, DiscBlock):
+                    h = block.forward_nhwc(h, slot, x_plane=xp, out_plane=op)
+                else:
+                    h = block.forward_nhwc(h, slot, out_plane=op)
+                xp = op
             if nxt is not None:
                 h = bank.mark(h, nxt[bi])
             h = ops.block_boundary(self, bi, h)
diff --git a/pytorch-studiogan_amd/csrc/common.h b/pytorch-studiogan_amd/csrc/common.h
--- a/pytorch-studiogan_amd/csrc/common.h
+++ b/pytorch-studiogan_amd/csrc/common.h
@@ -30,6 +30,14 @@
 __device__ __forceinline__ uint32_t pack2bf(float a, float b) {
   sg_f32x2_t v = {a, b};
   return __builtin_bit_cast(uint32_t, __builtin_convertvector(v, sg_bf16x2_t));
+}
+
+__device__ __forceinline__ uint32_t sign_nibble(u32x2 t) {
+  uint32_t b = 0u;
+#pragma unroll
+  for (int e = 0; e < 4; e++)
+    if (bf2f((bf16_t)((t[e >> 1] >> (16 * (e & 1))) & 0xffffu)) > 0.f) b |= 1u << e;
+  return b;
 }
 
 template <typename T> __device__ __forceinline__ float to_f(T v);
diff --git a/pytorch-studiogan_amd/csrc/conv.hip b/pytorch-studiogan_amd/csrc/conv.hip
--- a/pytorch-studiogan_amd/csrc/conv.hip
+++ b/pytorch-studiogan_amd/csrc/conv.hip
@@ -8,6 +8,24 @@
   return 0;
 }
 extern "C" int sg_get_f32_mode() { return g_sg_f32_mode; }
+
+__global__ __launch_bounds__(256) void k_sign_plane(const bf16_t* __restrict__ x, int ld, int C, long long rows, uint32_t* __restrict__ plane) {
+  const int pw = C >> 5;
+  const long long idx = (long long)blockIdx.x * 256 + threadIdx.x;
+  if (idx >= rows * pw) return;
+  const long long r = idx / pw;
+  const int w = (int)(idx - r * pw);
+  const bf16_t* src = x + r * ld + w * 32;
+  uint32_t bits = 0u;
+#pragma unroll
+  for (int c = 0; c < 4; c++) {
+    const u32x4 v = *(const u32x4*)(src + c * 8);
+    const u32x2 lo = {v[0], v[1]}, hi = {v[2], v[3]};
+    bits |= (sign_nibble(lo) | (sign_nibble(hi) << 4)) << (8 * c);
+  }
+  plane[idx] = bits;
+}
+extern "C" int sg_sign_plane_ok(int dtype, int C) { return (dtype == SG_DTYPE_BF16 && C >= 32 && C % 32 == 0) ? 1 : 0; }
 
 template <typename T, bool FAST>
 static void conv_fwd_launch(const sg_conv_fwd_desc* d, const Epilogue<T>& e, int I, int J, int K, int pflags, hipStream_t st) {
@@ -103,7 +121,7 @@
   return sg_conv_fwd_sk_try(d, e, I, J, K, pflags, st);
 }
 
-template <typename T> static int conv_fwd_t(const sg_conv_fwd_desc* d, hipStream_t st) {
+template <typename T> static int conv_fwd_t(const sg_conv_fwd_desc* d, const void* mask_plane, void* out_plane, hipStream_t st) {
   const int K = d->R * d->S * d->C;
   const int I = d->Cout;
   const long long Jll = (long long)d->N * d->Ho * d->Wo;
@@ -124,6 +142,12 @@
   e.res = d->res; e.res_bstride = 0; e.ldr = d->ldr; e.beta = d->beta;
   e.mask = (const T*)d->mask; e.mask_bstride = 0; e.ldm = d->ldm; e.split_stride = 0;
   e.alpha = d->alpha; e.alpha_ptr = d->alpha_ptr; e.flags = d->epi_flags; e.I = I; e.J = J;
+  if (mask_plane || out_plane) {
+    SG_CHECK(sg_sign_plane_ok(d->dtype, I) == 1 && !(d->epi_flags & SG_EPI_OUT_F32), "sg_conv2d_fwd: sign planes need bf16 tensors with Cout % 32 == 0 (ask sg_sign_plane_ok first)");
+    SG_CHECK(!mask_plane || d->mask, "sg_conv2d_fwd: mask_plane is given next to mask, not instead of it");
+    SG_CHECK(!out_plane || ((d->ldo & 7) == 0 && aligned16(d->out)), "sg_conv2d_fwd: out_plane needs 16-byte aligned output rows");
+    e.mplane = (const uint32_t*)mask_plane; e.oplane = (uint32_t*)out_plane;
+  }
   const int prof = sg_prof_begin(st, 2.0 * (double)I * (double)J * (double)K, 0);
   int eng = SG_ENG_CONV_GEMM;
   if (w_vec && x_vec && conv_fwd_sk_try<T>(d, e, I, J, K, pflags, st)) eng = SG_ENG_CONV_SK;
@@ -133,9 +157,16 @@
   else if (w_vec && x_vec && conv_fwd_v2_try<T>(d, e, I, J, K, pflags, st)) eng = SG_ENG_CONV_V2;
   else if (w_vec && x_vec) conv_fwd_launch<T, true>(d, e, I, J, K, pflags, st);
   else conv_fwd_launch<T, false>(d, e, I, J, K, pflags, st);
+  const bool planes = (eng == SG_ENG_CONV_SK && I > 64 && I <= 96) || eng == SG_ENG_CONV_V4 || eng == SG_ENG_CONV_V3 || eng == SG_ENG_CONV_V2;
+  const long long rows_out = (d->epi_flags & SG_EPI_POOL) ? (long long)J / 4 : (long long)J;
+  if (e.oplane && !(planes && !e.mask)) {
+    if constexpr (sizeof(T) == 2)
+      hipLaunchKernelGGL(k_sign_plane, dim3((unsigned)((rows_out * (I >> 5) + 255) / 256)), dim3(256), 0, st, (const bf16_t*)d->out, d->ldo, I, rows_out, e.oplane);
+  }
   {
-    const double es = sizeof(T), jout = (d->epi_flags & SG_EPI_POOL) ? (double)J / 4.0 : (double)J;
-    const double b = es * ((double)d->N * d->Hs * d->Ws * d->C + (double)I * K + jout * I * (1.0 + (d->mask ? 1.0 : 0.0) + (d->res ? 1.0 : 0.0)));
+    const double es = sizeof(T), jout = (double)rows_out;
+    const double mk = d->mask ? ((e.mplane && planes) ? 1.0 / 16.0 : 1.0) : 0.0, op = e.oplane ? 1.0 / 16.0 : 0.0;
+    const double b = es * ((double)d->N * d->Hs * d->Ws * d->C + (double)I * K + jout * I * (1.0 + mk + op + (d->res ? 1.0 : 0.0)));
     sg_prof_tag(prof, eng, b);
   }
   sg_prof_end(st, prof);
@@ -143,7 +174,7 @@
   return 0;
 }
 
-static int conv_fwd_skip(const sg_conv_skip_desc* sk, hipStream_t st, bool dry) {
+static int conv_fwd_skip(const sg_conv_skip_desc* sk, hipStream_t st, bool dry, void* out_plane = nullptr) {
   const sg_conv_fwd_desc* d = &sk->main;
   if (d->dtype != SG_DTYPE_BF16 || d->R != 3 || d->S != 3 || d->stride != 1 || (d->pix_flags & (SG_PIX_UPSAMPLE | SG_PIX_TRANSPOSED))) return 0;
   const int K = 9 * d->C, I = d->Cout;
@@ -157,6 +188,8 @@
   e.res = d->res; e.res_bstride = 0; e.ldr = d->ldr; e.beta = d->beta;
   e.mask = (const bf16_t*)d->mask; e.mask_bstride = 0; e.ldm = d->ldm; e.split_stride = 0;
   e.alpha = d->alpha; e.alpha_ptr = d->alpha_ptr; e.flags = d->epi_flags; e.I = I; e.J = J;
+  if (out_plane && (I % 32 || d->mask)) return 0;
+  e.oplane = (uint32_t*)out_plane;
   if (dry) return sg_conv_fwd_v4_skip_try(d, sk, e, I, J, K, pflags, st, true) ? 1 : 0;
   const int prof = sg_prof_begin(st, 2.0 * (double)I * (double)J * ((double)K + (double)sk->C2), 0);
   const bool ok = sg_conv_fwd_v4_skip_try(d, sk, e, I, J, K, pflags, st, false);
@@ -177,19 +210,21 @@
   if (!d || !d->main.x || !d->main.w || !d->main.out || !d->x2 || !d->w2) return 0;
   return conv_fwd_skip(d, nullptr, true);
 }
-extern "C" int sg_conv2d_fwd_skip(const sg_conv_skip_desc* d, sg_stream_t stream) {
+extern "C" int sg_conv2d_fwd_skip(const sg_conv_skip_desc* d, sg_stream_t stream) { return sg_conv2d_fwd_skip_planes(d, nullptr, stream); }
+extern "C" int sg_conv2d_fwd_skip_planes(const sg_conv_skip_desc* d, void* out_plane, sg_stream_t stream) {
   SG_CHECK(d && d->main.x && d->main.w && d->main.out && d->x2 && d->w2, "sg_conv2d_fwd_skip: null pointer");
-  SG_CHECK(conv_fwd_skip(d, (hipStream_t)stream, false) == 1, "sg_conv2d_fwd_skip: problem not eligible for the fused kernel (ask sg_conv2d_fwd_skip_ok first)");
+  SG_CHECK(conv_fwd_skip(d, (hipStream_t)stream, false, out_plane) == 1, "sg_conv2d_fwd_skip: problem not eligible for the fused kernel (ask sg_conv2d_fwd_skip_ok first)");
   SG_LAUNCH_CHECK();
   return 0;
 }
 
-extern "C" int sg_conv2d_fwd(const sg_conv_fwd_desc* d, sg_stream_t stream) {
+extern "C" int sg_conv2d_fwd(const sg_conv_fwd_desc* d, sg_stream_t stream) { return sg_conv2d_fwd_planes(d, nullptr, nullptr, stream); }
+extern "C" int sg_conv2d_fwd_planes(const sg_conv_fwd_desc* d, const void* mask_plane, void* out_plane, sg_stream_t stream) {
   SG_CHECK(d && d->x && d->w && d->out, "sg_conv2d_fwd: null pointer");
   SG_CHECK(d->N > 0 && d->C > 0 && d->Cout > 0 && d->R > 0 && d->S > 0 && d->stride > 0, "sg_conv2d_fwd: bad shape");
   SG_CHECK(!(d->epi_flags & SG_EPI_ATOMIC), "sg_conv2d_fwd: atomic epilogue not supported");
-  if (d->dtype == SG_DTYPE_F32) return conv_fwd_t<float>(d, (hipStream_t)stream);
-  if (d->dtype == SG_DTYPE_BF16) return conv_fwd_t<bf16_t>(d, (hipStream_t)stream);
+  if (d->dtype == SG_DTYPE_F32) return conv_fwd_t<float>(d, mask_plane, out_plane, (hipStream_t)stream);
+  if (d->dtype == SG_DTYPE_BF16) return conv_fwd_t<bf16_t>(d, mask_plane, out_plane, (hipStream_t)stream);
   sg_set_error("sg_conv2d_fwd: bad dtype");
   return -1;
 }
diff --git a/pytorch-studiogan_amd/csrc/conv_q.hip b/pytorch-studiogan_amd/csrc/conv_q.hip
--- a/pytorch-studiogan_amd/csrc/conv_q.hip
+++ b/pytorch-studiogan_amd/csrc/conv_q.hip
@@ -147,6 +147,7 @@
 }
 
 static bool convq_plan(const sg_convq_desc* d, ConvQParams& p, Epilogue<bf16_t>& e, int& NB) {
+  e.mplane = nullptr; e.oplane = nullptr;
   if (d->dtype != SG_DTYPE_BF16 || (d->form != SG_Q_POOL && d->form != SG_Q_UP)) return false;
   const char* mode = getenv("SG_CONV_Q");
   if (mode && mode[0] == '0') return false;
@@ -209,10 +210,13 @@
   const int sbj = p.bj > 256 ? 256 : p.bj;
   return ((p.J + sbj - 1) / sbj) * (d->form == SG_Q_POOL ? 1 : 4);
 }
-extern "C" int sg_conv2d_q(const sg_convq_desc* d, sg_stream_t stream) {
+extern "C" int sg_conv2d_q(const sg_convq_desc* d, sg_stream_t stream) { return sg_conv2d_q_planes(d, nullptr, nullptr, stream); }
+extern "C" int sg_conv2d_q_planes(const sg_convq_desc* d, const void* mask_plane, void* out_plane, sg_stream_t stream) {
   SG_CHECK(d && d->x && d->wq && d->out, "sg_conv2d_q: null pointer");
   ConvQParams p; Epilogue<bf16_t> e; int NB = 0;
   SG_CHECK(convq_plan(d, p, e, NB), "sg_conv2d_q: problem not eligible for the quad kernel (ask sg_conv2d_q_ok first)");
+  SG_CHECK((!mask_plane || d->mask) && !(out_plane && d->mask), "sg_conv2d_q_planes: mask_plane goes next to mask; out_plane not in a masked launch");
+  e.mplane = (const uint32_t*)mask_plane; e.oplane = (uint32_t*)out_plane;
   hipStream_t st = (hipStream_t)stream;
   const double c2 = d->x2 ? (double)d->C2 : 0.0;
   const int prof = sg_prof_begin_q(st, 2.0 * (double)d->Cout * 4.0 * (double)p.J * (9.0 * (double)d->C + c2), 0);
@@ -221,9 +225,10 @@
   int db_mode = ev_db ? (ev_db[0] == '1' ? 1 : 0) : ((d->Wl == 4 && d->form == SG_Q_UP) ? 1 : 0);
   const int rc = NB == 3 ? sg_launch_conv_q<3>(p, e, db_mode, st) : sg_launch_conv_q<2>(p, e, db_mode, st);
   {
+    const double mk = d->mask ? (mask_plane ? 1.0 / 16.0 : 1.0) : 0.0, op = out_plane ? 1.0 / 16.0 : 0.0;
     const double J = (double)p.J, jin = d->form == SG_Q_POOL ? 4.0 * J : J, jout = d->form == SG_Q_POOL ? J : 4.0 * J;
     sg_prof_tag(prof, d->x2 ? SG_ENG_CONV_Q_SKIP : SG_ENG_CONV_Q,
-                2.0 * (jin * d->C + (d->x2 ? 4.0 * J * d->C2 + (double)d->Cout * d->C2 : 0.0) + 16.0 * d->C * d->Cout + jout * d->Cout * (1.0 + (d->mask ? 1.0 : 0.0) + (d->res ? 1.0 : 0.0))));
+                2.0 * (jin * d->C + (d->x2 ? 4.0 * J * d->C2 + (double)d->Cout * d->C2 : 0.0) + 16.0 * d->C * d->Cout + jout * d->Cout * (1.0 + mk + op + (d->res ? 1.0 : 0.0))));
   }
   sg_prof_end(st, prof);
   SG_CHECK(rc == 0, "sg_conv2d_q: launch failed");
diff --git a/pytorch-studiogan_amd/csrc/conv_sk.h b/pytorch-studiogan_amd/csrc/conv_sk.h
--- a/pytorch-studiogan_amd/csrc/conv_sk.h
+++ b/pytorch-studiogan_amd/csrc/conv_sk.h
@@ -41,6 +41,9 @@
   const auto rsx = __builtin_amdgcn_make_buffer_rsrc((void*)p.x, 0, (int)p.xbytes, 0x00020000);
   const auto rso = __builtin_amdgcn_make_buffer_rsrc(epi.out, 0, (int)p.obytes, 0x00020000);
   const auto rss = __builtin_amdgcn_make_buffer_rsrc((void*)(epi.mask ? (const void*)epi.mask : epi.res), 0, (int)p.sbytes, 0x00020000);
+  constexpr bool PL = TI == 3 && NP == 1 && TJ == 1;
+  const bool by_plane = PL && epi.mplane != nullptr;
+  const int pw = epi.I >> 5, nib = 4 * (lane >> 5);
   constexpr int NIT = ((POOL ? ROWS / 4 : ROWS) * CPR + 63) / 64;
   const int frow = lane & 31, fhi = lane >> 5;
   const unsigned ldx2 = 2u * (unsigned)p.ldx;
@@ -104,7 +107,7 @@
   if (epi.alpha_ptr) al *= *epi.alpha_ptr;
   constexpr bool pool = POOL;
   const bool relu_out = (epi.flags & SG_EPI_RELU) != 0;
-  const bool pre_mask = epi.mask != nullptr, pre_res = epi.res != nullptr;
+  const bool pre_mask = epi.mask != nullptr && !by_plane, pre_res = epi.res != nullptr;
   const int Jout = pool ? (epi.J >> 2) : epi.J;
   const int ncr = ((epi.I - i0 < BI ? epi.I - i0 : BI) + 7) >> 3;
   constexpr int rows_out_full = ROWS;
@@ -172,6 +175,20 @@
         }
         asm volatile("s_waitcnt lgkmcnt(0)" ::: "memory");
       }
+      uint32_t mbits[TI * TJ];
+#pragma unroll
+      for (int q4 = 0; q4 < TI * TJ; q4++) mbits[q4] = 0u;
+      const bool emit = PL && epi.oplane != nullptr && epi.mask == nullptr;
+      if (by_plane) {
+#pragma unroll
+        for (int ta = 0; ta < TI; ta++)
+#pragma unroll
+          for (int tb = 0; tb < TJ; tb++) {
+            const int jl = tb * 32 + (lane & 31);
+            const int jg = jbase + (pool ? (jl >> 2) : jl), ig = i0 + ic0 + ta * 32;
+            if (jg < Jout && ig < epi.I) mbits[ta * TJ + tb] = epi.mplane[(unsigned)jg * (unsigned)pw + (unsigned)(ig >> 5)];
+          }
+      }
 #pragma unroll
       for (int ta = 0; ta < TI; ta++)
 #pragma unroll
@@ -196,7 +213,11 @@
 #pragma unroll
                 for (int e = 0; e < 4; e++) v[e] += bv[e];
               }
-              if (pre_mask) {
+              if (by_plane) {
+                const uint32_t bits = mbits[ta * TJ + tb] >> (8 * g4 + nib);
+#pragma unroll
+                for (int e = 0; e < 4; e++) if (!((bits >> e) & 1u)) v[e] = 0.f;
+              } else if (pre_mask) {
                 const u32x2 m = *(const u32x2*)loc;
 #pragma unroll
                 for (int e = 0; e < 4; e++) { const bf16_t h = (bf16_t)((m[e >> 1] >> (16 * (e & 1))) & 0xffffu); if (!(bf2f(h) > 0.f)) v[e] = 0.f; }
@@ -214,6 +235,7 @@
               t[0] = pack2bf(v[0], v[1]);
               t[1] = pack2bf(v[2], v[3]);
               *(u32x2*)loc = t;
+              if (emit) mbits[ta * TJ + tb] |= sign_nibble(t) << (8 * g4 + nib);
             }
           }
         }
@@ -228,6 +250,17 @@
         const int rr = idx < rows_out * CPR ? r : 0;
         const u32x4 v = *(const u32x4*)(stg + rr * CP + c * 16);
         __builtin_amdgcn_raw_buffer_store_b128(v, rso, (int)off, 0, 0);
+      }
+      if (emit) {
+#pragma unroll
+        for (int ta = 0; ta < TI; ta++)
+#pragma unroll
+          for (int tb = 0; tb < TJ; tb++) {
+            const int jl = tb * 32 + (lane & 31);
+            const int jg = jbase + (pool ? (jl >> 2) : jl), ig = i0 + ic0 + ta * 32;
+            const uint32_t w = mbits[ta * TJ + tb] | __shfl_xor(mbits[ta * TJ + tb], 32, 64);
+            if (lane < 32 && (!pool || (lane & 3) == 0) && jg < Jout && ig < epi.I) epi.oplane[(unsigned)jg * (unsigned)pw + (unsigned)(ig >> 5)] = w;
+          }
       }
     }
   };
diff --git a/pytorch-studiogan_amd/csrc/conv_v2.h b/pytorch-studiogan_amd/csrc/conv_v2.h
--- a/pytorch-studiogan_amd/csrc/conv_v2.h
+++ b/pytorch-studiogan_amd/csrc/conv_v2.h
@@ -33,8 +33,11 @@
   const int rows_out = pool ? BJ / 4 : BJ;
   const int jbase = pool ? (j0 >> 2) : j0, Jout = pool ? (epi.J >> 2) : epi.J;
   constexpr int CPR = BI / 8;
-  const bool pre_mask = epi.mask != nullptr, pre_res = epi.res != nullptr;
+  const bool by_plane = epi.mplane != nullptr;
+  const bool pre_mask = epi.mask != nullptr && !by_plane, pre_res = epi.res != nullptr;
   const bool pre_both = pre_mask && pre_res;
+  const int pw = epi.I >> 5;
+  const int nib = 4 * (lane >> 5);
   const int ncr = ((epi.I - i0 < BI ? epi.I - i0 : BI) + 7) >> 3;
   auto stage_tile = [&](const bf16_t* src, int ld) {
     for (int idx = tid; idx < rows_out * CPR; idx += 64 * NW) {
@@ -48,6 +51,17 @@
   uint32_t mbits[TI * TJ];
 #pragma unroll
   for (int q = 0; q < TI * TJ; q++) mbits[q] = 0u;
+  const bool emit = epi.oplane != nullptr && epi.mask == nullptr;
+  if (by_plane && active) {
+#pragma unroll
+    for (int ta = 0; ta < TI; ta++)
+#pragma unroll
+      for (int tb = 0; tb < TJ; tb++) {
+        const int jl = wj0 + tb * 32 + (lane & 31);
+        const int jg = jbase + (pool ? (jl >> 2) : jl), ig = i0 + wi0 + ta * 32;
+        if (jg < Jout && ig < epi.I) mbits[ta * TJ + tb] = epi.mplane[(unsigned)grow(jg) * (unsigned)pw + (unsigned)(ig >> 5)];
+      }
+  }
   if (pre_both) {
     stage_tile(epi.mask, epi.ldm);
     __syncthreads();
@@ -64,7 +78,7 @@
             const int il = wi0 + ta * 32 + 8 * g4 + 4 * (lane >> 5);
             const u32x2 m = *(const u32x2*)(smem + jo * CP + il * 2);
 #pragma unroll
-            for (int e = 0; e < 4; e++) { const bf16_t h = (bf16_t)((m[e >> 1] >> (16 * (e & 1))) & 0xffffu); if (bf2f(h) > 0.f) bits |= 1u << (4 * g4 + e); }
+            for (int e = 0; e < 4; e++) { const bf16_t h = (bf16_t)((m[e >> 1] >> (16 * (e & 1))) & 0xffffu); if (bf2f(h) > 0.f) bits |= 1u << (8 * g4 + nib + e); }
           }
           mbits[ta * TJ + tb] = bits;
         }
@@ -102,8 +116,8 @@
 #pragma unroll
             for (int e = 0; e < 4; e++) v[e] += b[e];
           }
-          if (pre_both) {
-            const uint32_t bits = mbits[ta * TJ + tb] >> (4 * g4);
+          if (pre_both || by_plane) {
+            const uint32_t bits = mbits[ta * TJ + tb] >> (8 * g4 + nib);
 #pragma unroll
             for (int e = 0; e < 4; e++) if (!((bits >> e) & 1u)) v[e] = 0.f;
           } else if (pre_mask) {
@@ -124,8 +138,20 @@
           t[0] = pack2bf(v[0], v[1]);
           t[1] = pack2bf(v[2], v[3]);
           *(u32x2*)loc = t;
-        }
-      }
+          if (emit) mbits[ta * TJ + tb] |= sign_nibble(t) << (8 * g4 + nib);
+        }
+      }
+    }
+    if (emit) {
+#pragma unroll
+      for (int ta = 0; ta < TI; ta++)
+#pragma unroll
+        for (int tb = 0; tb < TJ; tb++) {
+          const int jl = wj0 + tb * 32 + (lane & 31);
+          const int jg = jbase + (pool ? (jl >> 2) : jl), ig = i0 + wi0 + ta * 32;
+          const uint32_t w = mbits[ta * TJ + tb] | __shfl_xor(mbits[ta * TJ + tb], 32, 64);
+          if (lane < 32 && (!pool || (lane & 3) == 0) && jg < Jout && ig < epi.I) epi.oplane[(unsigned)grow(jg) * (unsigned)pw + (unsigned)(ig >> 5)] = w;
+        }
     }
   }
   __syncthreads();
diff --git a/pytorch-studiogan_amd/csrc/gemm_core.h b/pytorch-studiogan_amd/csrc/gemm_core.h
--- a/pytorch-studiogan_amd/csrc/gemm_core.h
+++ b/pytorch-studiogan_amd/csrc/gemm_core.h
@@ -229,6 +229,7 @@
   float alpha; const float* alpha_ptr;
   int flags; int I; int J;
   long long split_stride;
+  const uint32_t* mplane = nullptr; uint32_t* oplane = nullptr;
 
   __device__ __forceinline__ void set_batch(int b) {
     if (flags & (SG_EPI_OUT_F32 | SG_EPI_ATOMIC)) out = (float*)out + (long long)b * out_bstride;
diff --git a/pytorch-studiogan_amd/functional/_base.py b/pytorch-studiogan_amd/functional/_base.py
--- a/pytorch-studiogan_amd/functional/_base.py
+++ b/pytorch-studiogan_amd/functional/_base.py
@@ -79,6 +79,29 @@
     return ent[3], ent[4]
 
 
+def sign_plane_on():
+    return os.environ.get("SG_SIGN_PLANE", "1") != "0"
+
+
+class SignPlane:
+    __slots__ = ("plane", "key")
+
+    def __init__(self):
+        self.plane = None
+        self.key = None
+
+    def new(self, out):
+        C = out.shape[-1]
+        if not sign_plane_on() or not out.is_contiguous() or L.lib().sg_sign_plane_ok(L.dt(out), C) != 1:
+            return None
+        self.plane = torch.empty(out.shape[:-1] + (C // 32,), dtype=torch.int32, device=out.device)
+        self.key = (out.data_ptr(), tuple(out.shape), out._version)
+        return self.plane
+
+    def of(self, x):
+        return self.plane if self.key == (x.data_ptr(), tuple(x.shape), x._version) else None
+
+
 class f32_mode:
     MODES = {"exact": 0, "bf16x3": 3}
 
@@ -98,7 +121,8 @@
 
 
 def conv2d_raw(x, w_ptr, Cin, Cout, R, S, stride=1, pad_h=0, pad_w=0, pix_flags=0, epi_flags=0, bias=None, res=None, mask=None,
-               alpha=1.0, beta=1.0, alpha_ptr=None, out=None, ldx=None, transposed_out_hw=None, out_coff=0, x_coff=0, desc=None):
+               alpha=1.0, beta=1.0, alpha_ptr=None, out=None, ldx=None, transposed_out_hw=None, out_coff=0, x_coff=0, desc=None,
+               mask_plane=None, out_plane=None):
     N, Hs, Ws = x.shape[0], x.shape[1], x.shape[2]
     ldx = x.shape[3] if ldx is None else ldx
     up = 2 if (pix_flags & L.PIX_UPSAMPLE) else 1
@@ -110,9 +134,12 @@
         Wo = (Win + 2 * pad_w - S) // stride + 1
     pool = bool(epi_flags & L.EPI_POOL)
     Hy, Wy = (Ho // 2, Wo // 2) if pool else (Ho, Wo)
+    opl = None
     if out is None:
         odt = torch.float32 if (epi_flags & L.EPI_OUT_F32) else x.dtype
         out = torch.empty((N, Hy, Wy, Cout), dtype=odt, device=x.device)
+        if out_plane is not None and desc is None:
+            opl = out_plane.new(out)
     d = desc if desc is not None else L.ConvFwdDesc()
     d.dtype = L.dt(x)
     d.N, d.Hs, d.Ws, d.C, d.ldx = N, Hs, Ws, Cin, ldx
@@ -131,11 +158,15 @@
     d.ldm = mask.shape[-1] if mask is not None else 0
     if desc is not None:
         return out
-    L.call("sg_conv2d_fwd", d, L.stream())
+    if opl is not None or (mask_plane is not None and mask is not None):
+        L.call("sg_conv2d_fwd_planes", d, L.ptr(mask_plane) if mask is not None else None, L.ptr(opl), L.stream())
+    else:
+        L.call("sg_conv2d_fwd", d, L.stream())
     return out
 
 
-def conv2d_skip_raw(x, w_ptr, Cin, Cout, x2, w2_ptr, C2, x2_up=False, pix_flags=0, epi_flags=0, bias=None, bias2=None, alpha=1.0, dry=False, stats=False):
+def conv2d_skip_raw(x, w_ptr, Cin, Cout, x2, w2_ptr, C2, x2_up=False, pix_flags=0, epi_flags=0, bias=None, bias2=None, alpha=1.0, dry=False, stats=False,
+                    out_plane=None):
     sk = L.ConvSkipDesc()
     out = conv2d_raw(x, w_ptr, Cin, Cout, 3, 3, 1, 1, 1, pix_flags, epi_flags, bias=bias, alpha=alpha, desc=sk.main)
     sk.x2, sk.w2, sk.bias2 = L.ptr(x2), w2_ptr, L.ptr(bias2)
@@ -143,6 +174,10 @@
     if L.lib().sg_conv2d_fwd_skip_ok(L.C.byref(sk)) != 1:
         return None
     if dry:
+        return out
+    opl = out_plane.new(out) if out_plane is not None else None
+    if opl is not None:
+        L.call("sg_conv2d_fwd_skip_planes", sk, L.ptr(opl), L.stream())
         return out
     if stats and not (epi_flags & L.EPI_POOL):
         rows = L.lib().sg_conv2d_fwd_skip_stat_rows(L.C.byref(sk))
@@ -190,7 +225,7 @@
 
 
 def conv2d_q_raw(x, wq_ptr, form, Cin, Cout, pix_flags=0, epi_flags=0, bias=None, res=None, mask=None, alpha=1.0, beta=1.0, dry=False,
-                 x2=None, w2q_ptr=None, bias2=None, stats=False, x2_norelu=False):
+                 x2=None, w2q_ptr=None, bias2=None, stats=False, x2_norelu=False, mask_plane=None, out_plane=None):
     N = x.shape[0]
     if form == L.Q_POOL:
         if x.shape[1] % 2 or x.shape[2] % 2:
@@ -217,12 +252,16 @@
     if L.lib().sg_conv2d_q_ok(L.C.byref(d)) != 1:
         return None
     if not dry:
+        opl = out_plane.new(out) if (out_plane is not None and mask is None) else None
         st = None
         if stats:
             rows = L.lib().sg_conv2d_q_stat_rows(L.C.byref(d))
             st = torch.empty((rows, Cout, 2), dtype=torch.float32, device=x.device)
             d.stats = st.data_ptr()
-        L.call("sg_conv2d_q", d, L.stream())
+        if opl is not None or (mask_plane is not None and mask is not None):
+            L.call("sg_conv2d_q_planes", d, L.ptr(mask_plane) if mask is not None else None, L.ptr(opl), L.stream())
+        else:
+            L.call("sg_conv2d_q", d, L.stream())
         if st is not None:
             _offer_stats(out, st, rows, Cout)
     return out
@@ -286,4 +325,4 @@
     return dx
 
 
-__all__ = ['L', 'zeros_small', 'zeros_like_small', '_BN_FUSED_STATS', '_CBN_MERGED', '_DGRAD_SPLITK', '_SEQ', '_STATS_OFFER', '_c', '_comm', '_first_order_only', '_offer_stats', '_param_grad_wanted', '_take_stats', '_tick', 'conv2d_q_raw', 'conv2d_q_wgrad_raw', 'conv2d_raw', 'conv2d_skip_raw', 'conv2d_wgrad_raw', 'dist', 'ensure_grad', 'f32_mode', 'gemm_dgrad_rows', 'gemm_raw', 'os', 'quad_pack_raw', 'torch']
+__all__ = ['L', 'SignPlane', 'sign_plane_on', 'zeros_small', 'zeros_like_small', '_BN_FUSED_STATS', '_CBN_MERGED', '_DGRAD_SPLITK', '_SEQ', '_STATS_OFFER', '_c', '_comm', '_first_order_only', '_offer_stats', '_param_grad_wanted', '_take_stats', '_tick', 'conv2d_q_raw', 'conv2d_q_wgrad_raw', 'conv2d_raw', 'conv2d_skip_raw', 'conv2d_wgrad_raw', 'dist', 'ensure_grad', 'f32_mode', 'gemm_dgrad_rows', 'gemm_raw', 'os', 'quad_pack_raw', 'torch']
diff --git a/pytorch-studiogan_amd/functional/attention.py b/pytorch-studiogan_amd/functional/attention.py
--- a/pytorch-studiogan_amd/functional/attention.py
+++ b/pytorch-studiogan_amd/functional/attention.py
@@ -321,11 +321,11 @@
 class AttnOutFn(torch.autograd.Function):
 
     @staticmethod
-    def forward(ctx, x, o, weight, sigma, rt, slot, link=None):
+    def forward(ctx, x, o, weight, sigma, rt, slot, link=None, out_plane=None):
         bank = rt.bank()
         x, o = _c(x), _c(o)
         ctx.link = link
-        y = conv2d_raw(o, bank.w_fwd(slot, rt), rt.Cin, rt.rows, 1, 1, res=x, alpha_ptr=sigma)
+        y = conv2d_raw(o, bank.w_fwd(slot, rt), rt.Cin, rt.rows, 1, 1, res=x, alpha_ptr=sigma, out_plane=out_plane)
         ctx.save_for_backward(o, sigma)
         ctx.rt, ctx.slot = rt, slot
         ctx.sigma_param = sigma
@@ -340,7 +340,7 @@
             if _param_grad_wanted(ctx.weight, ctx.sigma_param):
                 raise NotImplementedError("create_graph=True is supported for input gradients only (WGAN-GP / R1 path)")
             do = ScalePtrFn.apply(ConvDgradFn.apply(dy, o, ctx.weight, rt, slot, ConvCfg(1, 1)), ctx.sigma_param) if ctx.needs_input_grad[1] else None
-            return (dy if ctx.needs_input_grad[0] else None), do, None, None, None, None, None
+            return (dy if ctx.needs_input_grad[0] else None), do, None, None, None, None, None, None
         bank = rt.bank()
         dy = _c(dy)
         N, H, W, Cc = dy.shape
@@ -356,7 +356,7 @@
         dx = dy
         if ctx.link is not None and ctx.link.pending > 0 and ctx.needs_input_grad[0]:
             ctx.link.dx, dx = dy, None
-        return dx, do, None, None, None, None, None
+        return dx, do, None, None, None, None, None, None
 
 
 __all__ = ['AttnCoreFn', 'AttnOutFn', 'AttnPooledFn', 'AttnProjFn', 'attn_proj_ok', 'attn_proj_on', 'BmmFn', 'MaxPool2BwdFn', 'MaxPool2Fn', 'ScalePtrFn', 'SoftmaxRowsBwdFn', 'SoftmaxRowsFn', '_attn_reference_graph', '_maxpool2_bwd']
diff --git a/pytorch-studiogan_amd/functional/conv.py b/pytorch-studiogan_amd/functional/conv.py
--- a/pytorch-studiogan_amd/functional/conv.py
+++ b/pytorch-studiogan_amd/functional/conv.py
@@ -40,19 +40,19 @@
     return L.Q_POOL if cfg.out_pool else L.Q_UP
 
 
-def _conv_fwd(x, rt, slot, cfg, bias, res=None, stats=False):
+def _conv_fwd(x, rt, slot, cfg, bias, res=None, stats=False, out_plane=None):
     bank = rt.bank()
     Cin = x.shape[3]
     form = _quad_form(rt, cfg, x)
     if form is not None:
         y = conv2d_q_raw(x, bank.w_quad(slot, rt, form), form, Cin, rt.rows_pad, L.PIX_RELU if cfg.in_relu else 0, 0, bias=bias, res=res,
-                         stats=stats and _BN_FUSED_STATS[0] and rt.rows_pad == rt.rows)
+                         stats=stats and _BN_FUSED_STATS[0] and rt.rows_pad == rt.rows, out_plane=out_plane)
         if y is not None:
             return y
     pf = (L.PIX_RELU if cfg.in_relu else 0) | (L.PIX_UPSAMPLE if cfg.in_upsample else 0)
     ef = L.EPI_POOL if cfg.out_pool else 0
     return conv2d_raw(x, bank.w_fwd(slot, rt), Cin, rt.rows_pad, cfg.R, cfg.S, cfg.stride, cfg.pad_h, cfg.pad_w, pf, ef, bias=bias, res=res,
-                      alpha=0.25 if cfg.out_pool else 1.0)
+                      alpha=0.25 if cfg.out_pool else 1.0, out_plane=out_plane)
 
 
 def _conv_wgrad(x, dy, rt, slot, cfg, dbias=None):
@@ -70,12 +70,12 @@
                             L.PIX_UPSAMPLE if pool else 0, alpha=0.25 if pool else 1.0, dbias=dbias)
 
 
-def _conv_dgrad(dy, x, rt, slot, cfg, res=None):
+def _conv_dgrad(dy, x, rt, slot, cfg, res=None, x_plane=None):
     bank = rt.bank()
     N, Hs, Ws, Cin = x.shape
     form = _quad_form(rt, cfg, x)
     if form is not None and dy.shape[3] == rt.rows_pad:
-        dx = conv2d_q_raw(dy, bank.w_quad(slot, rt, 2 + form), 1 - form, rt.rows_pad, Cin, 0, 0, mask=x if cfg.in_relu else None, res=res)
+        dx = conv2d_q_raw(dy, bank.w_quad(slot, rt, 2 + form), 1 - form, rt.rows_pad, Cin, 0, 0, mask=x if cfg.in_relu else None, res=res, mask_plane=x_plane)
         if dx is not None:
             return dx
     up = 2 if cfg.in_upsample else 1
@@ -88,7 +88,7 @@
     pf = L.PIX_UPSAMPLE if pool else 0
     ef = L.EPI_POOL if cfg.in_upsample else 0
     return conv2d_raw(dy, bank.w_dgrad(slot, rt), rt.rows_pad, Cin, cfg.R, cfg.S, 1, cfg.R - 1 - cfg.pad_h, cfg.S - 1 - cfg.pad_w, pf, ef,
-                      mask=x if cfg.in_relu else None, res=res, alpha=0.25 if pool else 1.0, ldx=dy.shape[3])
+                      mask=x if cfg.in_relu else None, res=res, alpha=0.25 if pool else 1.0, ldx=dy.shape[3], mask_plane=x_plane)
 
 
 class ConvDgradFn(torch.autograd.Function):
@@ -128,7 +128,7 @@
 class ConvFn(torch.autograd.Function):
 
     @staticmethod
-    def forward(ctx, x, weight, bias, res, rt, slot, cfg, link=None):
+    def forward(ctx, x, weight, bias, res, rt, slot, cfg, link=None, x_plane=None, out_plane=None):
         bank = rt.bank()
         x = _c(x)
         N, Hs, Ws, Cin = x.shape
@@ -143,7 +143,8 @@
             bias_k = zeros_small(rt.rows_pad, torch.float32, x.device)
             bias_k[:rt.rows].copy_(bias.detach())
         _tick()
-        y = _conv_fwd(x, rt, slot, cfg, bias_k, res, stats=cfg.stats)
+        y = _conv_fwd(x, rt, slot, cfg, bias_k, res, stats=cfg.stats, out_plane=out_plane)
+        ctx.x_plane = x_plane.of(x) if (x_plane is not None and cfg.in_relu) else None
         ctx.save_for_backward(x)
         ctx.rt, ctx.slot, ctx.cfg = rt, slot, cfg
         ctx.bias = bias
@@ -160,7 +161,7 @@
             if _param_grad_wanted(ctx.weight, ctx.bias):
                 raise NotImplementedError("create_graph=True is supported for input gradients only (WGAN-GP path)")
             dx = ConvDgradFn.apply(dy, x, ctx.weight, rt, slot, cfg) if ctx.needs_input_grad[0] else None
-            return dx, None, None, (dy if ctx.has_res else None), None, None, None, None
+            return dx, None, None, (dy if ctx.has_res else None), None, None, None, None, None, None
         dy = _c(dy)
         N, Hs, Ws, Cin = x.shape
         up = 2 if cfg.in_upsample else 1
@@ -172,7 +173,7 @@
         dx = None
         skip_dx = ctx.link.take() if ctx.link is not None else None
         if ctx.needs_input_grad[0]:
-            dx = _conv_dgrad(dy, x, rt, slot, cfg, res=skip_dx)
+            dx = _conv_dgrad(dy, x, rt, slot, cfg, res=skip_dx, **({} if ctx.x_plane is None else {"x_plane": ctx.x_plane}))
         elif skip_dx is not None:
             raise RuntimeError("GradLink: a skip gradient was handed over but this convolution's input needs no gradient")
         if ctx.link is not None and ctx.link.chain:
@@ -189,16 +190,17 @@
             rows = dy.shape[0] * dy.shape[1] * dy.shape[2]
             L.call("sg_colsum", L.dt(dy), L.ptr(dy), dy.shape[3], None, 0, rows, rt.rows, L.ptr(g), 1.0, L.stream())
         dres = dy if ctx.has_res else None
-        return dx, None, None, dres, None, None, None, None
+        return dx, None, None, dres, None, None, None, None, None, None
 
 
 class ConvSkipFn(torch.autograd.Function):
 
     @staticmethod
-    def forward(ctx, h, x, w2, b2, w0, b0, rt2, rt0, slot, cfg2, cfg0, link=None):
+    def forward(ctx, h, x, w2, b2, w0, b0, rt2, rt0, slot, cfg2, cfg0, link=None, h_plane=None, x_plane=None, out_plane=None):
         bank = rt2.bank()
         ctx.link = link
         h, x = _c(h), _c(x)
+        ctx.planes = (h_plane.of(h) if (h_plane is not None and cfg2.in_relu) else None, x_plane.of(x) if (x_plane is not None and cfg0.in_relu) else None)
         _tick()
         assert cfg2.R == 3 and cfg0.R == 1 and cfg2.out_pool == cfg0.out_pool and not cfg2.in_upsample and (cfg0.in_relu == cfg2.in_relu or not cfg0.in_relu)
         pf = L.PIX_RELU if cfg2.in_relu else 0
@@ -209,14 +211,14 @@
         plain = rt2.rows_pad == rt2.rows and rt0.rows_pad == rt0.rows and b2 is not None and b0 is not None
         if plain and same_relu and h.dtype == torch.bfloat16 and _SKIP_FUSION[0] and (h.shape[1] >= 16 or _SKIP_FUSION[0] == "all") and _quad_form(rt2, cfg2, h) is None:
             y = conv2d_skip_raw(h, bank.w_fwd(slot, rt2), h.shape[3], rt2.rows, x, bank.w_fwd(slot, rt0), x.shape[3], cfg0.in_upsample, pf, ef,
-                                bias=b2, bias2=b0, alpha=al, stats=cfg2.stats and _BN_FUSED_STATS[0])
+                                bias=b2, bias2=b0, alpha=al, stats=cfg2.stats and _BN_FUSED_STATS[0], out_plane=out_plane)
         if y is None and plain and _quad_form(rt2, cfg2, h) == L.Q_POOL and _SKIP_FUSION[0] and (rt0.cin_pad % 32 == 0 or rt0.cin_pad == 8) and not cfg0.in_upsample:
             y = conv2d_q_raw(h, bank.w_quad(slot, rt2, L.Q_POOL), L.Q_POOL, h.shape[3], rt2.rows, pf, 0, bias=b2,
-                             x2=x, w2q_ptr=bank.w_quad(slot, rt0, 5 if rt0.cin_pad == 8 else 4), bias2=b0, x2_norelu=not same_relu)
+                             x2=x, w2q_ptr=bank.w_quad(slot, rt0, 5 if rt0.cin_pad == 8 else 4), bias2=b0, x2_norelu=not same_relu, out_plane=out_plane)
         if y is None:
             hh = _conv_fwd(h, rt2, slot, cfg2, b2)
             pf0 = (L.PIX_RELU if cfg0.in_relu else 0) | (L.PIX_UPSAMPLE if cfg0.in_upsample else 0)
-            y = conv2d_raw(x, bank.w_fwd(slot, rt0), x.shape[3], rt0.rows_pad, 1, 1, 1, 0, 0, pf0, ef, bias=b0, res=hh, alpha=al)
+            y = conv2d_raw(x, bank.w_fwd(slot, rt0), x.shape[3], rt0.rows_pad, 1, 1, 1, 0, 0, pf0, ef, bias=b0, res=hh, alpha=al, out_plane=out_plane)
         ctx.save_for_backward(h, x)
         ctx.rt2, ctx.rt0, ctx.slot, ctx.cfg2, ctx.cfg0 = rt2, rt0, slot, cfg2, cfg0
         ctx.w2, ctx.b2, ctx.w0, ctx.b0 = w2, b2, w0, b0
@@ -231,7 +233,7 @@
                 raise NotImplementedError("create_graph=True is supported for input gradients only (WGAN-GP path)")
             dh = ConvDgradFn.apply(dy, h, ctx.w2, rt2, slot, cfg2) if ctx.needs_input_grad[0] else None
             dx = ConvDgradFn.apply(dy, x, ctx.w0, rt0, slot, cfg0) if ctx.needs_input_grad[1] else None
-            return (dh, dx) + (None,) * 10
+            return (dh, dx) + (None,) * 13
         dy = _c(dy)
         bank = rt2.bank()
         outs = []
@@ -246,7 +248,7 @@
             up = 2 if cfg.in_upsample else 1
             Ho, Wo = Hs * up, Ws * up
             pool = cfg.out_pool
-            outs.append(_conv_dgrad(dy, inp, rt, slot, cfg) if ctx.needs_input_grad[k] else None)
+            outs.append(_conv_dgrad(dy, inp, rt, slot, cfg, **({} if ctx.planes[k] is None else {"x_plane": ctx.planes[k]})) if ctx.needs_input_grad[k] else None)
             want_db = bp is not None and ctx.needs_input_grad[b_i]
             db_done = False
             if ctx.needs_input_grad[w_i]:
@@ -271,7 +273,7 @@
         if ctx.link is not None and outs[1] is not None and _GRAD_LINK[0]:
             ctx.link.dx = outs[1]
             outs[1] = None
-        return (outs[0], outs[1]) + (None,) * 10
+        return (outs[0], outs[1]) + (None,) * 13
 
 
 _SKIP_FUSION = [{"0": False, "all": "all"}.get(os.environ.get("SG_SKIP_FUSION", "1"), True)]
diff --git a/pytorch-studiogan_amd/ops.py b/pytorch-studiogan_amd/ops.py
--- a/pytorch-studiogan_amd/ops.py
+++ b/pytorch-studiogan_amd/ops.py
@@ -98,12 +98,12 @@
         self._sg_dgrad_noflip = self.stride[0] != 1
         self._sg_setup("conv", out_channels, in_channels * kh * kw, in_channels, kh * kw, sn)
 
-    def forward_nhwc(self, x, slot=None, in_relu=False, in_upsample=False, out_pool=False, res=None, link=None, stats=False):
+    def forward_nhwc(self, x, slot=None, in_relu=False, in_upsample=False, out_pool=False, res=None, link=None, stats=False, x_plane=None, out_plane=None):
         rt = self._sg_rt
         slot = slot if slot is not None else rt.bank().current
         kh, kw = self.kernel_size
         cfg = F.ConvCfg(kh, kw, self.stride[0], self.padding[0], self.padding[1], in_relu, in_upsample, out_pool, stats and self.training)
-        return F.ConvFn.apply(x, self.master_weight, self.bias, res, rt, slot, cfg, link)
+        return F.ConvFn.apply(x, self.master_weight, self.bias, res, rt, slot, cfg, link, x_plane, out_plane)
 
     def forward(self, x):
         slot = _standalone_slot(self, x)
@@ -114,12 +114,13 @@
         return to_nchw(y)
 
 
-def conv_skip_nhwc(conv_main, conv_skip, h, x, slot=None, in_relu=False, out_pool=False, skip_upsample=False, link=None, stats=False, skip_relu=None):
+def conv_skip_nhwc(conv_main, conv_skip, h, x, slot=None, in_relu=False, out_pool=False, skip_upsample=False, link=None, stats=False, skip_relu=None,
+                   h_plane=None, x_plane=None, out_plane=None):
     rt2, rt0 = conv_main._sg_rt, conv_skip._sg_rt
     slot = slot if slot is not None else rt2.bank().current
     cfg2 = F.ConvCfg(3, 3, 1, 1, 1, in_relu, False, out_pool, stats)
     cfg0 = F.ConvCfg(1, 1, 1, 0, 0, in_relu if skip_relu is None else skip_relu, skip_upsample, out_pool)
-    return F.ConvSkipFn.apply(h, x, conv_main.master_weight, conv_main.bias, conv_skip.master_weight, conv_skip.bias, rt2, rt0, slot, cfg2, cfg0, link)
+    return F.ConvSkipFn.apply(h, x, conv_main.master_weight, conv_main.bias, conv_skip.master_weight, conv_skip.bias, rt2, rt0, slot, cfg2, cfg0, link, h_plane, x_plane, out_plane)
 
 
 class ConvTranspose2d(_WeightLayerMixin, nn.ConvTranspose2d):
@@ -282,7 +283,7 @@
             m._sg_rows_pad = pad8
         self.sigma = nn.Parameter(torch.zeros(1), requires_grad=True)
 
-    def forward_nhwc(self, x, slot=None):
+    def forward_nhwc(self, x, slot=None, out_plane=None):
         link = F.GradLink(chain=True) if (F._GRAD_LINK[0] and torch.is_grad_enabled() and x.requires_grad) else None
         rt = self.conv1x1_attn._sg_rt
         slot = slot if slot is not None else rt.bank().current
@@ -296,7 +297,7 @@
             phi = self.conv1x1_phi.forward_nhwc(x, slot, link=link)
             g = self.conv1x1_g.forward_nhwc(x, slot, link=link)
             o = F.AttnCoreFn.apply(theta, phi, g)
-        return F.AttnOutFn.apply(x, o, self.conv1x1_attn.master_weight, self.sigma, rt, slot, link)
+        return F.AttnOutFn.apply(x, o, self.conv1x1_attn.master_weight, self.sigma, rt, slot, link, out_plane)
 
     def forward(self, x):
         _, bank = _root_and_bank(self.conv1x1_theta)
```

New measurement: 2096 (median of 6 runs). 1.02x the previous value.
